# PrimeIntellect-ai/protocol

Hardware: AMD Instinct MI355X
Metric: task x worker pair-evals/sec (full-swarm match) (higher is better)
Workload: dtype u64

## Files before the change

### protocol_amd/csrc/pm_device.h

```cpp
#ifndef PM_DEVICE_H
#define PM_DEVICE_H

#include <hip/hip_runtime.h>
#include <stdint.h>

#include "pm_engine.h"

namespace pm {

static constexpr double PM_RAD = 3.14159265358979323846 / 180.0;
static constexpr uint64_t PM_KEY_NOLOC = 0x7FEFFFFFFFFFFFFFull;
static constexpr double PM_A_MAX_SAFE = 1.0 - 1.0 / 1048576.0;
static constexpr double PM_A_CHORD_MIN = 1.3e-6;
static constexpr uint32_t PM_CARVE_SLOTS = 8192;
static constexpr uint32_t PM_CARVE_PART = 64;
static constexpr uint32_t PM_CARVE_SEL_CAP = 256;
static constexpr uint32_t PM_CARVE_SLOT_BITS = 13;
static constexpr uint32_t PM_CARVE_BIG_SLOTS = 262144;
static constexpr uint32_t PM_CARVE_SLOT_BITS_BIG = 18;
static constexpr uint32_t PM_CARVE_SLOT_BITS_MEM = 21;
static constexpr double PM_TIE_BAND = 1.0 / 68719476736.0;
static constexpr double PM_TIE_BAND_BIG = 1.0 / 2147483648.0;
static constexpr double PM_TIE_BAND_MEM = 1.0 / 268435456.0;
static constexpr uint32_t PM_PROP_ROW = 96;
static constexpr uint32_t PM_PROP_SLOTS = 64;
static constexpr uint32_t PM_PROP_KMAX = 63;
static constexpr uint32_t PM_ROW_SAFE = 1u << 27;
static constexpr uint32_t PM_ROW_TAIL_CLEAR = 1u << 28;
static constexpr uint32_t PM_ROW_CLEAN = 1u << 29;
static constexpr uint32_t PM_ROW_TAIL_OK = 1u << 30;
static constexpr uint32_t PM_ROW_COMPLETE = 1u << 31;
static constexpr uint32_t PM_PROP_RESERVE = 64;
static constexpr uint32_t PM_PROP_MAX_SEEDS = 16384;
static constexpr uint32_t PM_CELL_G_MAX = 64;
static constexpr uint32_t PM_CELL_TABLE = PM_CELL_G_MAX * PM_CELL_G_MAX * PM_CELL_G_MAX + 2;
static constexpr uint32_t PM_CELL_MIN_N = 6000;
static constexpr uint32_t PM_CELL_AUTO_N = 40000;
static constexpr uint32_t PM_CELL_BIG_N = 40000;
static constexpr uint32_t PM_CELL_RMAX = 14;
static constexpr size_t PM_CARVE_LDS_BYTES = size_t(16) * PM_CARVE_PART * 8 + size_t(PM_CARVE_SLOTS / 64) * 16 +
                                             size_t(PM_CARVE_SLOTS) * 16 + size_t(PM_CARVE_SEL_CAP) * 4 + 1024;
static constexpr uint32_t PM_STREAM_SQ = 8192;
static constexpr uint32_t PM_STREAM_RQ = 8192;
static constexpr uint32_t PM_STREAM_TP = 4096;
static constexpr uint32_t PM_STREAM_LA_MAX = 3072;
static constexpr uint32_t PM_STREAM_CTL_WORDS = 64;
#ifndef PM_STREAM_PROP_WAVES_N
#define PM_STREAM_PROP_WAVES_N 4
#endif
static constexpr uint32_t PM_STREAM_PROP_WAVES = PM_STREAM_PROP_WAVES_N;
static constexpr uint32_t PM_STREAM_SLW_TREQ = PM_STREAM_TP;
static constexpr uint32_t PM_STREAM_SLW_PAY = PM_STREAM_TP + 1;
static constexpr size_t PM_STREAM_LDS_BYTES = PM_CARVE_LDS_BYTES + size_t(PM_STREAM_TP) * 4 + 128;
enum { SC_CLAIM = 0,
       SC_QUIT = 16,
       SC_DROP = 32,
       SC_ROWS = 48,
       SC_LET_BE = 53,
       SC_GAVE_UP = 49,
       SC_FINISH = 50,
       SC_FINISH_TICKET = 52,
       SC_TRACE = 51,
       SC_BATCHES = 54
};
static constexpr uint32_t PM_STREAM_TRACE_CAP = 1u << 17;
enum { SROW_NONE = 0, SROW_BITMAP = 1, SROW_WALK = 2, SROW_SWEEP = 3 };

struct CompatArgs {
  uint32_t W, n_cfgs, model_words;
  const uint32_t *flags, *gpu_count, *gpu_mem, *gpu_cls, *cpu_cores, *ram, *storage;
  const pm_config_row* cfgs;
  const pm_gpu_alt_row* alts;
  const uint32_t* model_bits;
  uint64_t* compat;
};

enum : uint32_t {
  REP_WHY = 0,
  REP_IDLE = PM_WHY_N,
  REP_GROUPS,
  REP_MEMBERS,
  REP_NO_TASK,
  REP_TASKS,
  REP_STRIDE = 16
};

struct ReportArgs {
  CompatArgs c;
  const int32_t* group_of;
  const uint32_t *g_cfg, *g_n, *g_task, *live_bits;
  uint32_t G;
  const uint64_t *tmask, *tlive;
  const uint32_t* tprefix;
  uint32_t t_lo, t_cap;
  uint32_t* out;
  uint32_t *running, *workers, *allowed;
};

struct ClaimArgs {
  uint32_t R;
  const uint32_t* rows;
  const int32_t* group_of;
  const uint32_t *g_n, *g_off, *g_task;
  const uint64_t* g_id;
  uint32_t* g_task_next;
  const uint32_t* chosen;
  const uint32_t* rank_in_group;
  const uint32_t* by_rank;
  const uint64_t* t_live;
  const uint32_t* t_prefix;
  pm_assignment* table;
  uint32_t* task_col;
  pm_assignment* h_table;
  uint32_t* h_gtask;
};

struct MatchPrepArgs {
  uint32_t W, G;
  const int32_t* group_of;
  const uint32_t *g_cfg, *g_n, *g_off, *members, *addr_rank, *g_task;
  uint64_t* sel;
  uint32_t *first, *count;
  uint32_t *rank_in_group, *by_rank;
  uint32_t* g_task_next;
};

struct RowUpdateArgs {
  uint32_t n;
  const double *lat_in, *lon_in;
  const uint32_t* u32_in;
  uint32_t *flags, *gpu_count, *gpu_mem, *gpu_cls, *cpu_cores, *ram, *storage, *addr_rank, *site;
  double *lat, *lon, *coslat;
  double *ux, *uy, *uz;
};

enum { CARVE_MODE_FORM = 0, CARVE_MODE_MERGE = 1 };
enum { CARVE_STATE_RUNNING = 0, CARVE_STATE_DONE = 1, CARVE_STATE_UNCERTAIN = 2, CARVE_STATE_OVERFLOW = 3,
       CARVE_STATE_ABORTED = 4 };
enum {
  CARVE_F_INIT = 1u << 0,
  CARVE_F_RUN = 1u << 1,
  CARVE_F_ALL = 1u << 2,
  CARVE_F_PROPS = 1u << 3,
  CARVE_F_EXTPREP = 1u << 4
};
struct CarveStatus {
  uint32_t state;
  uint32_t stop_ci;
  uint32_t n_groups;
  uint32_t n_members;
  uint32_t steps_total;
  uint32_t stop_seed;
  uint32_t n_eligible;
  uint32_t cur_ci;
  unsigned long long cand_sum;
  uint32_t n_list;
  uint32_t prop_k;
  uint32_t prop_limit;
  uint32_t rows_pr;
  uint32_t n_seeds;
  uint32_t total_available;
  uint32_t fast_steps;
  uint32_t slow_steps;
  uint32_t n_solo;
  uint32_t n_props;
  uint32_t need_prep;
  uint32_t g_lo, g_hi;
  uint32_t n_batches;
  uint32_t n_void;
  uint32_t why[8];
  uint32_t stream_timeouts;
  uint32_t stream_tickets;
  uint32_t stream_switches;
  uint32_t stream_listed;
  uint32_t stream_pre_used;
  uint32_t stream_pre_lost;
  uint32_t stream_refreshes;
  uint32_t _pad_sr;
  uint32_t cell_g;
  uint32_t n_indexed;
  uint32_t pruned_batches;
  uint32_t prune_fallbacks;
#ifdef PM_BATCH_LOG
  uint32_t blog_n;
  uint32_t blog[3 * 512];
#endif
  unsigned long long prop_keys;
  unsigned long long prof[64];
};

struct BatchDesc {
  uint32_t planned;
  uint32_t ci0;
  uint32_t total_available;
  uint32_t valid;
  uint32_t none;
  uint32_t ci, n_list, prop_k, prop_limit, rows_pr, n_seeds;
  uint32_t cell_g;
};

struct CarveArgs {
  uint32_t mode;
  uint32_t _flags_unused;
  uint32_t W;
  uint32_t proximity;
  uint32_t debug_uncertain_every;
  uint32_t _pad_re;
  const uint32_t* wflags;
  const double *lat, *lon, *coslat;
  const double *ux, *uy, *uz;
  const uint32_t* site;
  const uint64_t* compat;
  int32_t* group_of;
  uint32_t* order;
  uint32_t n_order;
  uint32_t _pad2;
  double *c_lat, *c_lon, *c_cos;
  double *c_ux, *c_uy, *c_uz;
  uint32_t* c_site;
  uint64_t* c_compat;
  uint64_t *alive_g, *loc_g;
  double *cc_lat, *cc_lon, *cc_cos;
  double *cc_ux, *cc_uy, *cc_uz;
  uint32_t* cc_site;
  uint32_t* slot_pos;
  uint32_t* slot_wid;
  uint64_t* bits_scratch;
  uint64_t* keys;
  uint32_t bits_stride;
  uint32_t _pad0;
  uint64_t* prop;
  uint64_t* prop_send;
  uint64_t* seed_map;
  uint32_t* seed_prefix;
  uint32_t* seed_slots;
  uint32_t dist_rank, dist_world;
  uint32_t count_keys, _pad_ck;
  uint32_t* prep_block_counts;
  uint32_t* prep_counts;
  BatchDesc* desc;
  uint64_t* alive_snap;
  uint32_t _pad_sp;
  uint32_t debug_mem_above;
  uint32_t* cell_cnt;
  uint32_t* cell_start;
  uint32_t *pos_cell, *pos_rank;
  uint32_t* cs_of_pos;
  uint32_t* cs_slot;
  double *cs_ux, *cs_uy, *cs_uz;
  uint32_t* cs_site;
  uint32_t prune_mode;
  uint32_t prune_factor;
  uint32_t walk_cap_div, _pad_w;
  uint32_t stream, stream_tag0;
  double* c_pack;
  double* cs_pack;
  uint64_t* cfgbits;
  unsigned long long* stream_sq;
  unsigned long long* stream_row_lo;
  unsigned long long* stream_row_hi;
  uint32_t* stream_ctl;
  uint32_t stream_la, stream_row_spins;
  uint32_t stream_la_div;
  uint32_t debug_abort_after;
  unsigned long long id_state;
  uint32_t id_g0, stage_m0;
  uint32_t stage_cap_g, stage_cap_m;
  uint32_t *stage_cfg, *stage_n, *stage_off, *stage_mem;
  unsigned long long* g_id_out;
  uint32_t* g_task_out;
  CarveStatus* h_status;
  unsigned long long* stream_trace;
  uint32_t n_avail, start_ci;
  uint32_t avail_cfg[PM_MAX_CONFIGS];
  uint32_t min_size[PM_MAX_CONFIGS];
  uint32_t max_size[PM_MAX_CONFIGS];
  uint32_t *g_cfg, *g_n, *g_off, *members;
  uint32_t cap_groups, cap_members;
  CarveStatus* status;
};

void launch_compat(const CompatArgs& a, hipStream_t s);
void launch_explain(const CompatArgs& p, const uint32_t* rows, uint32_t n, uint32_t stride, uint32_t* why_out, hipStream_t s);
void launch_config_report(const ReportArgs& a, uint32_t max_blocks, hipStream_t s);
void launch_task_report(const ReportArgs& a, uint32_t max_blocks, hipStream_t s);
void launch_geo(const double* lat, const double* lon, double* coslat, double* ux, double* uy, double* uz, uint32_t W,
                hipStream_t s);
void launch_triad(const double* b, const double* c, double* a, size_t n, hipStream_t s);
#ifdef PM_ROW_BENCH
hipError_t launch_row_bench(const CarveArgs* d_args, uint32_t seed, uint32_t ci, uint32_t reps, uint32_t mode, unsigned long long* d_out, hipStream_t s);
#endif
void launch_row_network_test(const uint64_t* keys, const uint32_t* sites, uint32_t n_waves, uint32_t n_per_wave, uint32_t slot_bits,
                             uint64_t ulps, uint32_t upto, uint64_t* rows_out, uint32_t* mismatches, hipStream_t s);
static constexpr uint32_t PM_DK_WORDS = 20;
void launch_distance_key_test(const double* in, const double* geo, uint32_t n, uint32_t mode, double* out, hipStream_t s);
void launch_update_rows(const RowUpdateArgs& a, hipStream_t s);
void launch_worker_selector(const int32_t* group_of, const uint32_t* g_cfg, uint32_t R, const uint32_t* rows,
                            uint64_t* sel, hipStream_t s);
void launch_eligible_selector(const uint32_t* wflags, const int32_t* group_of, const uint64_t* compat,
                              uint64_t enabled, uint32_t W, const uint8_t* shard, uint32_t my_rank, uint64_t* sel,
                              hipStream_t s);
void launch_chooser_rank(const int32_t* group_of, const uint64_t* g_id, const uint32_t* count, uint32_t R,
                         const uint32_t* rows, uint64_t seed, uint32_t* rank, hipStream_t s);
void launch_table_scatter(const pm_assignment* x, const uint32_t* xrow, uint32_t W, pm_assignment* table,
                          uint32_t* task_col, uint32_t* g_task_next, const uint64_t* t_live, const uint32_t* t_prefix,
                          hipStream_t s);
void launch_group_rank(const int32_t* group_of, const uint32_t* g_n, const uint32_t* g_off, const uint32_t* members,
                       const uint32_t* addr_rank, uint32_t W, uint32_t* rank_in_group, uint32_t* by_rank,
                       hipStream_t s);
void launch_claim_publish(const ClaimArgs& a, hipStream_t s);
void launch_match_prep(const MatchPrepArgs& a, hipStream_t s);
void launch_build_planes(const uint64_t* col_mask, uint32_t n_cols, uint32_t c_begin, uint32_t c_end, uint32_t stride,
                         uint32_t n_planes, uint64_t* planes, hipStream_t s);
void launch_pair_sweep(int variant, const uint64_t* row_sel, uint32_t R, const uint64_t* col_mask,
                       const uint64_t* planes, uint32_t c_begin, uint32_t c_end, uint32_t stride, uint32_t n_planes,
                       uint32_t* first, uint32_t* count, hipStream_t s, bool inited = false);
void launch_pair_select(int variant, const uint64_t* row_sel, uint32_t R, const uint64_t* col_mask,
                        const uint64_t* planes, uint32_t c_begin, uint32_t c_end, uint32_t stride, uint32_t n_planes,
                        const uint32_t* rank, uint32_t* out, hipStream_t s);
void launch_task_prefix(const uint64_t* live, uint32_t w_begin, uint32_t w_end, uint32_t* prefix, hipStream_t s);
void launch_task_delete(const uint32_t* slots, uint32_t n, uint64_t* tmask, uint64_t* live, uint64_t* planes,
                        uint32_t stride, uint32_t n_planes, hipStream_t s);
void launch_task_intern(const uint64_t* tmask, const uint64_t* live, uint32_t u_begin, uint32_t u_end, uint64_t valid,
                        uint64_t* keys, uint32_t n_slots, uint32_t* vals, uint32_t* counter_and_overflow, uint64_t* umask,
                        uint32_t cap_u, hipStream_t s);
void launch_task_compact_class(const uint32_t* first_c, const uint32_t* count_c, const uint64_t* tmask, uint64_t valid,
                               const uint64_t* keys, const uint32_t* vals, uint32_t n_slots, uint32_t u_begin,
                               uint32_t u_end, const uint64_t* live, const uint32_t* prefix, uint32_t* first_out,
                               uint32_t* count_out, hipStream_t s);
void launch_task_compact(const uint32_t* first_u, const uint32_t* count_u, uint32_t u_begin, uint32_t u_end,
                         const uint64_t* live, const uint32_t* prefix, uint32_t* first_out, uint32_t* count_out,
                         hipStream_t s);
void launch_newest(const int64_t* created_at, const uint64_t* live, uint32_t t_begin, uint32_t t_end,
                   uint32_t* idx_by_block, long long* val_by_block, uint32_t n_blocks, hipStream_t s);
void launch_group_ids(uint64_t* g_id, uint32_t* g_task, uint32_t n, uint64_t rng_state, hipStream_t s);
hipError_t carve_kernels_init();
hipError_t launch_carve(const CarveArgs* d_args, uint32_t flags, uint32_t start_ci, size_t lds_bytes, hipStream_t s);
uint32_t launch_carve_prep(const CarveArgs* d_args, uint32_t W, hipStream_t s);
hipError_t launch_carve_args_put(const CarveArgs& a, CarveArgs* d_args, hipStream_t s);
uint32_t launch_carve_elig(CarveArgs* d_args, const CarveArgs* put, uint32_t W, uint32_t n_bound, uint32_t index_min, uint32_t start_ci,
                           bool fresh, uint32_t n_groups0, uint32_t n_members0, hipStream_t s);
void launch_carve_apply(const CarveArgs* d_args, uint32_t W, hipStream_t s);
void launch_carve_propose(const CarveArgs* d_args, uint32_t W, hipStream_t s);
hipError_t launch_carve_stream(const CarveArgs* d_args, uint32_t start_ci, uint32_t n_prop_wgs, hipStream_t s);
void launch_scatter_const(uint32_t* dst, const uint32_t* idx, uint32_t n, uint32_t v, hipStream_t s);
void launch_scatter_pairs(uint32_t* dst, const uint32_t* pairs, uint32_t n, hipStream_t s);
void launch_merge_place(const CarveArgs* d_args, uint32_t n_order, uint32_t n_groups0, uint32_t n_members0, uint32_t steps0,
                        hipStream_t s);

}
#endif
```

### protocol_amd/csrc/pm_engine_carve.inc

```
static int32_t ensure_compat(pm_engine* e, hipEvent_t end_ev = nullptr) {
  if (!e->have_cfgs || !e->have_workers) return set_error(PM_ESTATE, "configs and workers must be uploaded first");
  {
    int32_t rcf = sync_flags(e);
    if (rcf) return rcf;
  }
  if (!e->compat_dirty) return PM_OK;
  for (const pm_gpu_alt_row& a : e->alts)
    if ((a.flags & PM_G_MODEL) && a.model_row >= e->model_rows)
      return set_error(PM_ESTATE, "a GPU alternative names a model row but pm_set_model_table was not called");
  if (e->model_rows && e->cls_check_dirty)
    for (uint32_t w = 0; w < e->W; ++w)
      if ((e->h_flags[w] & PM_W_GPU_MODEL) && e->h_gpu_cls[w] >= e->model_classes)
        return set_error(PM_ERANGE, "worker gpu_model_class outside the model table");
  e->cls_check_dirty = false;
  HIPCHK(e->d_compat.ensure(std::max<size_t>(e->W, 1)));
  CompatArgs a{};
  a.W = e->W;
  a.n_cfgs = uint32_t(e->cfgs.size());
  a.model_words = (e->model_classes + 31u) / 32u;
  a.flags = e->d_flags.p;
  a.gpu_count = e->d_gpu_count.p;
  a.gpu_mem = e->d_gpu_mem.p;
  a.gpu_cls = e->d_gpu_cls.p;
  a.cpu_cores = e->d_cpu_cores.p;
// ... 23 lines not shown
  }
  e->h_compat_valid = true;
  return PM_OK;
}

static double host_distance(double lat1, double lon1, double lat2, double lon2) {
  const double R = 6371.0;
  const double lat1r = lat1 * PM_RAD, lat2r = lat2 * PM_RAD;
  const double dlat = (lat2 - lat1) * PM_RAD, dlon = (lon2 - lon1) * PM_RAD;
  const double s1 = std::sin(dlat / 2.0), s2 = std::sin(dlon / 2.0);
  const double a = s1 * s1 + std::cos(lat1r) * std::cos(lat2r) * (s2 * s2);
  const double c = 2.0 * std::atan2(std::sqrt(a), std::sqrt(1.0 - a));
  return R * c;
}

struct CarvePlan {
  std::vector<uint32_t> avail;
};

static size_t carve_lds_bytes(uint32_t , bool* in_lds) {
  *in_lds = true;
  return PM_CARVE_LDS_BYTES;
}

static int32_t fill_carve_args(pm_engine* e, CarveArgs* a, uint32_t mode, uint32_t n_order, bool stream = false) {
  const size_t cap = std::max<size_t>(e->W, 1);
  HIPCHK(e->d_order.ensure(cap));
  HIPCHK(e->d_c_lat.ensure(cap));
  HIPCHK(e->d_c_lon.ensure(cap));
  HIPCHK(e->d_c_cos.ensure(cap));
  HIPCHK(e->d_cc_lat.ensure(cap));
  HIPCHK(e->d_cc_lon.ensure(cap));
  HIPCHK(e->d_cc_cos.ensure(cap));
  for (int k = 0; k < 3; ++k) {
    HIPCHK(e->d_c_u[k].ensure(cap));
    HIPCHK(e->d_cc_u[k].ensure(cap));
  }
  HIPCHK(e->d_c_compat.ensure(cap));
  HIPCHK(e->d_keys.ensure(cap));
  HIPCHK(e->d_slot_pos.ensure(cap));
  HIPCHK(e->d_slot_wid.ensure(cap));
  HIPCHK(e->d_c_site.ensure(cap));
  HIPCHK(e->d_cc_site.ensure(cap));
  {
    const size_t world = e->dist_world;
    const size_t rows_pr = (size_t(PM_PROP_MAX_SEEDS) + 64 + world - 1) / world;
    HIPCHK(e->d_prop.ensure(rows_pr * world * PM_PROP_ROW));
    if (world > 1) HIPCHK(e->d_prop_send.ensure(rows_pr * PM_PROP_ROW));
    HIPCHK(e->d_seed_map.ensure((cap + 63) / 64 + 64));
    HIPCHK(e->d_seed_prefix.ensure((cap + 63) / 64 + 64));
    HIPCHK(e->d_seed_slots.ensure(size_t(PM_PROP_MAX_SEEDS) + 128));
    HIPCHK(e->d_prep_block_counts.ensure(((cap + 255) / 256 + 1) * PM_MAX_CONFIGS));
    HIPCHK(e->d_prep_counts.ensure(PM_MAX_CONFIGS + 8));
  }
  HIPCHK(e->d_status.ensure(1));
  HIPCHK(e->d_carve_args.ensure(2));
  HIPCHK(e->d_desc.ensure(2));
  const uint32_t stride = uint32_t((cap + 63) / 64);
  HIPCHK(e->d_bits.ensure(size_t(stride) * 4));
  HIPCHK(e->d_snap.ensure(size_t(stride) * 2));
  if (stream) {
    HIPCHK(e->d_c_pack.ensure(cap * 4));
    HIPCHK(e->d_cs_pack.ensure(cap * 4));
    HIPCHK(e->d_cfgbits.ensure(size_t(stride) * PM_MAX_CONFIGS));
    HIPCHK(e->d_stream_ctl.ensure(PM_STREAM_CTL_WORDS));
    if (!e->d_stream_sq.p) {
      HIPCHK(e->d_stream_sq.ensure(PM_STREAM_SQ));
      HIPCHK(e->d_stream_row_lo.ensure(size_t(PM_STREAM_RQ) * 64));
      HIPCHK(e->d_stream_row_hi.ensure(size_t(PM_STREAM_RQ) * 64));
      e->stream_seq = 0;
    }
  }
  if (mode == CARVE_MODE_FORM && e->prune_mode && e->cfg.proximity_enabled) {
    if (!e->d_cell_cnt.p) {
      HIPCHK(e->d_cell_cnt.ensure(PM_CELL_TABLE));
      HIPCHK(hipMemsetAsync(e->d_cell_cnt.p, 0, e->d_cell_cnt.cap * sizeof(uint32_t), e->stream));
    }
    if (!e->d_cell_start.p) {
      HIPCHK(e->d_cell_start.ensure(PM_CELL_TABLE + 384));
      HIPCHK(hipMemsetAsync(e->d_cell_start.p, 0, e->d_cell_start.cap * sizeof(uint32_t), e->stream));
    }
    HIPCHK(e->d_pos_cell.ensure(cap));
    HIPCHK(e->d_pos_rank.ensure(cap));
    HIPCHK(e->d_cs_of_pos.ensure(cap));
    HIPCHK(e->d_cs_slot.ensure(cap));
    HIPCHK(e->d_cs_site.ensure(cap));
    for (auto& u : e->d_cs_u) HIPCHK(u.ensure(cap));
  }
  std::memset(a, 0, sizeof(*a));
  a->mode = mode;
  a->W = e->W;
  a->proximity = e->cfg.proximity_enabled;
  a->debug_uncertain_every = e->cfg.debug_uncertain_every;
  a->wflags = e->d_flags.p;
  a->lat = e->d_lat.p;
  a->lon = e->d_lon.p;
  a->coslat = e->d_coslat.p;
  a->ux = e->d_ux.p;
  a->uy = e->d_uy.p;
  a->uz = e->d_uz.p;
  a->compat = e->d_compat.p;
  a->group_of = e->d_group_of.p;
  a->order = e->d_order.p;
  a->n_order = n_order;
  a->c_lat = e->d_c_lat.p;
  a->c_lon = e->d_c_lon.p;
  a->c_cos = e->d_c_cos.p;
  a->c_ux = e->d_c_u[0].p;
  a->c_uy = e->d_c_u[1].p;
  a->c_uz = e->d_c_u[2].p;
  a->c_compat = e->d_c_compat.p;
  a->alive_g = e->d_bits.p;
  a->loc_g = e->d_bits.p + stride;
  a->cc_lat = e->d_cc_lat.p;
  a->cc_lon = e->d_cc_lon.p;
  a->cc_cos = e->d_cc_cos.p;
  a->cc_ux = e->d_cc_u[0].p;
  a->cc_uy = e->d_cc_u[1].p;
  a->cc_uz = e->d_cc_u[2].p;
  a->keys = e->d_keys.p;
  a->slot_pos = e->d_slot_pos.p;
  a->slot_wid = e->d_slot_wid.p;
  a->site = e->d_site.p;
  a->c_site = e->d_c_site.p;
  a->cc_site = e->d_cc_site.p;
  a->prop = e->d_prop.p;
  a->prop_send = e->dist_world > 1 ? e->d_prop_send.p : e->d_prop.p;
  a->seed_map = e->d_seed_map.p;
  a->seed_prefix = e->d_seed_prefix.p;
  a->seed_slots = e->d_seed_slots.p;
  a->dist_rank = e->dist_rank;
  a->dist_world = e->dist_world;
  a->count_keys = e->cfg.time_proposer ? 1u : 0u;
  a->prep_block_counts = e->d_prep_block_counts.p;
  a->prep_counts = e->d_prep_counts.p;
  a->bits_scratch = e->d_bits.p + size_t(stride) * 2;
  a->bits_stride = stride;
  a->status = e->d_status.p;
  a->desc = e->d_desc.p;
  a->alive_snap = e->d_snap.p;
  a->debug_mem_above = e->debug_mem_above;
  if (mode == CARVE_MODE_FORM && e->prune_mode && e->cfg.proximity_enabled) {
    a->prune_mode = e->prune_mode;
    a->prune_factor = e->prune_factor;
    a->walk_cap_div = e->walk_cap_div;
    a->cell_cnt = e->d_cell_cnt.p;
    a->cell_start = e->d_cell_start.p;
    a->pos_cell = e->d_pos_cell.p;
    a->pos_rank = e->d_pos_rank.p;
    a->cs_of_pos = e->d_cs_of_pos.p;
    a->cs_slot = e->d_cs_slot.p;
    a->cs_site = e->d_cs_site.p;
    a->cs_ux = e->d_cs_u[0].p;
    a->cs_uy = e->d_cs_u[1].p;
    a->cs_uz = e->d_cs_u[2].p;
  }
  if (stream) {
    a->stream = 1;
    a->cc_lat = a->c_lat;
    a->cc_lon = a->c_lon;
    a->cc_cos = a->c_cos;
    a->cc_ux = a->c_ux;
    a->cc_uy = a->c_uy;
    a->cc_uz = a->c_uz;
    a->cc_site = a->c_site;
    a->slot_wid = a->order;
    a->bits_scratch = e->d_bits.p;
    a->loc_g = e->d_bits.p + stride;
    a->alive_g = e->d_bits.p + size_t(stride) * 2;
    a->cfgbits = e->d_cfgbits.p;
    a->c_pack = e->d_c_pack.p;
    a->cs_pack = e->d_cs_pack.p;
    a->stream_sq = (unsigned long long*)e->d_stream_sq.p;
    a->stream_row_lo = (unsigned long long*)e->d_stream_row_lo.p;
    a->stream_row_hi = (unsigned long long*)e->d_stream_row_hi.p;
    a->stream_ctl = e->d_stream_ctl.p;
#if defined(PM_CARVE_PROF) || defined(PM_ROW_REC)
    HIPCHK(e->d_stream_trace.ensure(size_t(PM_STREAM_TRACE_CAP) * 2));
    a->stream_trace = (unsigned long long*)e->d_stream_trace.p;
#endif
#ifdef PM_ROW_REC
    HIPCHK(hipMemsetAsync(e->d_stream_trace.p, 0, size_t(PM_STREAM_TRACE_CAP) * 16, e->stream));
#endif
    a->stream_la = e->stream_la_env;
    a->stream_la_div = e->stream_la_div_env;
    a->stream_row_spins = e->stream_row_spins_env;
    a->debug_abort_after = e->debug_abort_after;
  }
  return PM_OK;
}

static int32_t host_resolve_form_step(pm_engine* e, uint32_t cfg, CarveStatus* st) {
  int32_t rc = pull_compat(e);
  if (rc) return rc;
  std::vector<int32_t> group_of(e->W);
  if (e->W) {
    HIPCHK(hipMemcpyAsync(group_of.data(), e->d_group_of.p, size_t(e->W) * 4, hipMemcpyDeviceToHost, e->stream));
    HIPCHK(hipStreamSynchronize(e->stream));
  }
  const pm_config_row& c = e->cfgs[cfg];
  std::vector<uint32_t> compat;
  size_t total_available = 0;
  for (uint32_t w = 0; w < e->W; ++w) {
    const uint32_t f = e->h_flags[w];
    if (!((f & PM_W_HEALTHY) && (f & PM_W_HAS_P2P) && group_of[w] < 0)) continue;
    ++total_available;
    if ((e->h_compat[w] >> cfg) & 1ull) compat.push_back(w);
  }
  if (total_available < c.min_group_size || compat.size() < c.min_group_size || compat.empty())
    return set_error(PM_ESTATE, "host resolve: nothing to carve (state mismatch)");
  uint32_t seed = compat[0];
  bool seed_loc = false;
  for (uint32_t w : compat)
    if (e->h_flags[w] & PM_W_HAS_LOC) {
      seed = w;
      seed_loc = true;
      break;
    }
  std::vector<uint32_t> rest;
  for (uint32_t w : compat)
    if (w != seed) rest.push_back(w);
  if (seed_loc && e->cfg.proximity_enabled) {
    std::vector<double> d(e->W, 0.0);
    for (uint32_t w : rest)
      d[w] = (e->h_flags[w] & PM_W_HAS_LOC) ? host_distance(e->h_lat[seed], e->h_lon[seed], e->h_lat[w], e->h_lon[w])
                                            : 1.7976931348623157e308;
    std::stable_sort(rest.begin(), rest.end(), [&](uint32_t a, uint32_t b) { return d[a] < d[b]; });
  }
  std::vector<uint32_t> members{seed};
  for (uint32_t w : rest) {
    if (members.size() >= c.max_group_size) break;
    members.push_back(w);
  }
  if (members.size() < c.min_group_size) return set_error(PM_ESTATE, "host resolve: group below min size");
  const uint32_t g = st->n_groups, off = st->n_members, n = uint32_t(members.size());
  if (g >= e->d_g_cfg.cap || off + n > e->d_members.cap) return set_error(PM_ENOMEM, "group arrays overflow");
  HIPCHK(hipMemcpyAsync(e->d_g_cfg.p + g, &cfg, 4, hipMemcpyHostToDevice, e->stream));
  HIPCHK(hipMemcpyAsync(e->d_g_n.p + g, &n, 4, hipMemcpyHostToDevice, e->stream));
  HIPCHK(hipMemcpyAsync(e->d_g_off.p + g, &off, 4, hipMemcpyHostToDevice, e->stream));
  HIPCHK(hipMemcpyAsync(e->d_members.p + off, members.data(), size_t(n) * 4, hipMemcpyHostToDevice, e->stream));
  for (uint32_t w : members) group_of[w] = int32_t(g);
  HIPCHK(hipMemcpyAsync(e->d_group_of.p, group_of.data(), size_t(e->W) * 4, hipMemcpyHostToDevice, e->stream));
  HIPCHK(hipStreamSynchronize(e->stream));
  st->n_groups += 1;
  st->n_members += n;
  st->n_solo += n == 1 ? 1u : 0u;
  st->steps_total += 1;
  return PM_OK;
}

static int32_t absorb_groups(pm_engine* e) {
  if (!e->absorb_pending) return PM_OK;
  HIPCHK(hipEventSynchronize(e->ev_groups));
  const uint32_t g0 = e->ab_g0, ng = e->ab_g1 - e->ab_g0, m0 = e->ab_m0;
  const uint32_t *g_cfg = e->ab_cfg_p, *g_n = e->ab_n_p, *g_off = e->ab_off_p, *members = e->ab_mem_p;
  if (e->groups.capacity() < e->groups.size() + ng) e->groups.reserve(std::max(e->groups.size() + ng, e->groups.capacity() * 2));
  for (uint32_t k = 0; k < ng; ++k) {
    Group gr;
    gr.id = splitmix64_next(&e->id_rng);
    gr.cfg = g_cfg[k];
    gr.task = PM_NONE;
    gr.task_uid = 0;
    gr.members.assign(members + (g_off[k] - m0), members + (g_off[k] - m0) + g_n[k]);
    for (uint32_t w : gr.members) e->h_group_of[w] = int32_t(g0 + k);
    log_group_event(e, PM_GROUP_CREATED, gr);
    e->groups.push_back(std::move(gr));
  }
  e->absorb_pending = false;
  return PM_OK;
}

#define ABSORB_PENDING(e)                 \
  do {                                    \
    int32_t rc_abs_ = absorb_groups(e);   \
    if (rc_abs_) return rc_abs_;          \
  } while (0)

static void host_mark(const char* what) {
  static const bool on = [] { const char* v = getenv("PM_TRACE_HOST"); return v && *v == '1'; }();
  if (!on) return;
  static const auto t0 = std::chrono::steady_clock::now();
  const double us = std::chrono::duration<double, std::micro>(std::chrono::steady_clock::now() - t0).count();
  fprintf(stderr, "[pm host] %10.1f us  %s\n", us, what);
}

struct FormRun {
  CarveArgs a;
  BatchDesc desc[2] = {};
  CarveStatus st;
  std::vector<uint32_t> avail;
  uint32_t g0 = 0, m0 = 0, start_ci = 0;
  size_t lds = 0;
  bool use_props = false;
  bool nothing = false;
  uint32_t n_bound = 0;
  uint32_t n_elig_hint = 0;
  bool stream = false;
  bool single_call = true;
  uint32_t stream_wgs = 0;
  bool local_carve = false;
  bool rearmed = false;
  uint32_t stage_cap = 0;
  bool args_pending = false;
};

static int32_t launch_propose_timed(pm_engine* e, const CarveArgs* d_args, uint32_t n_bound, hipStream_t s);

static int32_t form_setup_args(pm_engine* e, FormRun* r);

static int32_t form_queue_init(pm_engine* e, FormRun* r, bool fresh = false) {
  fresh = fresh && r->use_props;
  if (!fresh) HIPCHK(hipMemcpyAsync(e->d_status.p, &r->st, sizeof(r->st), hipMemcpyHostToDevice, e->stream));
  if (r->use_props) {
    if (!r->stream) HIPCHK(hipMemsetAsync(e->d_desc.p, 0, 2 * sizeof(BatchDesc), e->stream));
    const uint32_t index_min = !r->a.prune_mode ? 0u : r->a.prune_mode >= 2u ? 1u : PM_CELL_AUTO_N;
    if (r->stream) {
      if (e->stream_seq == 0 || e->stream_seq >= 127) {
        HIPCHK(hipMemsetAsync(e->d_stream_sq.p, 0, size_t(PM_STREAM_SQ) * 8, e->stream));
        HIPCHK(hipMemsetAsync(e->d_stream_row_lo.p, 0, size_t(PM_STREAM_RQ) * 64 * 8, e->stream));
        HIPCHK(hipMemsetAsync(e->d_stream_row_hi.p, 0, size_t(PM_STREAM_RQ) * 64 * 8, e->stream));
        e->stream_seq = 0;
      }
      e->stream_seq += 1;
      const uint32_t tag0 = e->stream_seq << 25;
      if (r->a.stream_tag0 != tag0) {
        r->a.stream_tag0 = tag0;
        if (!r->args_pending)
          HIPCHK(hipMemcpyAsync(&e->d_carve_args.p->stream_tag0, &r->a.stream_tag0, sizeof(uint32_t), hipMemcpyHostToDevice, e->stream));
      }
    }
    e->tick_carve_launches += launch_carve_elig(e->d_carve_args.p, r->args_pending ? &r->a : nullptr, e->W, r->n_bound,
                                                r->n_elig_hint >= index_min ? index_min : 0u, r->start_ci, fresh, r->st.n_groups,
                                                r->st.n_members, e->stream);
    r->args_pending = false;
    host_mark("form: eligible list queued");
    if (r->stream) {
      HIPCHK(launch_carve_stream(e->d_carve_args.p, r->start_ci, r->stream_wgs, e->stream));
      e->tick_carve_launches += 2;
      return PM_OK;
    }
    e->tick_carve_launches += launch_carve_prep(e->d_carve_args.p, r->n_bound, e->stream);
    HIPCHK(hipGetLastError());
  } else
    HIPCHK(launch_carve(e->d_carve_args.p, CARVE_F_INIT | CARVE_F_RUN | CARVE_F_ALL, r->start_ci, r->lds, e->stream));
  e->tick_carve_launches++;
  return PM_OK;
}

static int32_t form_begin(pm_engine* e, FormRun* r, bool allow_pipeline, bool local_carve = false, hipEvent_t begin_ev = nullptr) {
  int32_t rc = absorb_groups(e);
  if (rc) return rc;
  rc = ensure_compat(e);
  if (rc) return rc;
  rc = push_groups(e);
  if (rc) return rc;
  available_order(e->cfgs.data(), uint32_t(e->cfgs.size()), e->enabled, &r->avail);
  r->g0 = e->d_n_groups;
  r->m0 = e->d_n_members;
  r->start_ci = 0;
  r->nothing = r->avail.empty() || e->W == 0;
  if (r->nothing) return PM_OK;
  if (e->h_group_of.size() == e->W && e->h_flags.size() == e->W) {
    const int32_t* const gof = e->h_group_of.data();
    const uint32_t* const fl = e->h_flags.data();
    const uint32_t need = PM_W_HEALTHY | PM_W_HAS_P2P;
    uint32_t nb = 0, ne = 0;
    for (uint32_t w = 0; w < e->W; ++w) {
      const uint32_t un = uint32_t(gof[w]) >> 31;
      nb += un;
      ne += un & uint32_t((fl[w] & need) == need);
    }
    r->n_bound = nb;
    r->n_elig_hint = ne;
  } else {
    r->n_bound = uint32_t(std::count_if(e->h_group_of.begin(), e->h_group_of.end(), [](int32_t g) { return g < 0; }));
    r->n_elig_hint = r->n_bound;
  }
  if (e->h_group_of.size() != e->W) r->n_bound = r->n_elig_hint = e->W;
  if (r->n_bound == 0) r->n_bound = 1;
  r->st = CarveStatus{};
  r->st.state = CARVE_STATE_RUNNING;
  r->st.n_groups = r->g0;
  r->st.n_members = r->m0;
  r->single_call = allow_pipeline;
  r->local_carve = local_carve;
  r->use_props = e->cfg.carve_variant != 1 && e->cfg.proximity_enabled;
  r->stream = r->single_call && r->use_props && e->cfg.carve_variant == 0 && (e->dist_world == 1 || r->local_carve) &&
              r->n_bound <= PM_CARVE_BIG_SLOTS &&
              !e->debug_mem_above;
  host_mark("form: begin (host mirrors counted)");
  rc = form_setup_args(e, r);
  if (rc) return rc;
  host_mark("form: arguments queued");
  if (begin_ev && r->args_pending) {
    e->k_carve_begin = begin_ev;
  } else {
    HIPCHK(hipEventRecord(e->kev[2], e->stream));
    e->k_carve_begin = e->kev[2];
  }
  return form_queue_init(e, r, true);
}

static int32_t form_setup_args(pm_engine* e, FormRun* r) {
  CarveArgs& a = r->a;
  int32_t rc = fill_carve_args(e, &a, CARVE_MODE_FORM, 0, r->stream);
  if (rc) return rc;
  if (r->stream) {
    uint32_t wgs = e->stream_wgs_env ? e->stream_wgs_env : r->n_elig_hint / 64u + 48u;
    const uint32_t max_wgs = e->n_cus > 8u ? e->n_cus - 4u : 4u;
    r->stream_wgs = std::max(1u, std::min(wgs, max_wgs));
    a.stream_tag0 = ((e->stream_seq == 0 || e->stream_seq >= 127) ? 1u : e->stream_seq + 1u) << 25;
    a.id_state = e->id_rng;
    a.id_g0 = r->g0;
    a.stage_m0 = r->m0;
    a.g_id_out = (unsigned long long*)e->d_g_id.p;
    a.g_task_out = e->d_g_task.p;
    r->stage_cap = std::max<uint32_t>(r->n_bound, 1u);
    const size_t need = size_t(4) * r->stage_cap;
    if (e->h_gstage_cap < need) {
      HIPCHK(hipStreamSynchronize(e->stream));
      if (e->h_gstage) (void)hipHostFree(e->h_gstage);
      e->h_gstage = nullptr;
      e->h_gstage_cap = 0;
      const size_t cap = std::max<size_t>(need, size_t(4) * std::max<uint32_t>(e->W, 1));
      HIPCHK(hipHostMalloc((void**)&e->h_gstage, cap * sizeof(uint32_t)));
      e->h_gstage_cap = cap;
    }
    if (!e->h_status) HIPCHK(hipHostMalloc((void**)&e->h_status, sizeof(CarveStatus)));
    a.stage_cap_g = a.stage_cap_m = r->stage_cap;
    a.stage_cfg = e->h_gstage;
    a.stage_n = e->h_gstage + r->stage_cap;
    a.stage_off = e->h_gstage + size_t(2) * r->stage_cap;
    a.stage_mem = e->h_gstage + size_t(3) * r->stage_cap;
    a.h_status = e->h_status;
    e->h_status->state = 0xFFFFFFFFu;
  }
  if (r->local_carve) {
    a.dist_rank = 0;
    a.dist_world = 1;
    a.prop_send = a.prop;
  }
  a.n_avail = uint32_t(r->avail.size());
  for (size_t i = 0; i < r->avail.size(); ++i) {
    a.avail_cfg[i] = r->avail[i];
    a.min_size[i] = e->cfgs[r->avail[i]].min_group_size;
    a.max_size[i] = e->cfgs[r->avail[i]].max_group_size;
  }
  a.g_cfg = e->d_g_cfg.p;
  a.g_n = e->d_g_n.p;
  a.g_off = e->d_g_off.p;
  a.members = e->d_members.p;
  a.cap_groups = uint32_t(std::min<size_t>(e->d_g_cfg.cap, 0xFFFFFFFFu));
  a.cap_members = uint32_t(std::min<size_t>(e->d_members.cap, 0xFFFFFFFFu));
  bool in_lds;
  r->lds = carve_lds_bytes(a.bits_stride, &in_lds);
  r->args_pending = r->use_props;
  if (!r->args_pending) HIPCHK(launch_carve_args_put(a, e->d_carve_args.p, e->stream));
  return PM_OK;
}

static int32_t launch_propose_timed(pm_engine* e, const CarveArgs* d_args, uint32_t n_bound, hipStream_t s) {
  if (!e->cfg.time_proposer) {
    launch_carve_propose(d_args, n_bound, s);
    return PM_OK;
  }
  while (e->prop_ev.size() < e->prop_ev_used + 2) {
    hipEvent_t x = nullptr;
    HIPCHK(hipEventCreate(&x));
    e->prop_ev.push_back(x);
  }
  HIPCHK(hipEventRecord(e->prop_ev[e->prop_ev_used], s));
  launch_carve_propose(d_args, n_bound, s);
  HIPCHK(hipEventRecord(e->prop_ev[e->prop_ev_used + 1], s));
  e->prop_ev_used += 2;
  return PM_OK;
}

static int32_t form_queue_pairs(pm_engine* e, FormRun* r, uint32_t count) {
  for (uint32_t k = 0; k < count; ++k) {
    int32_t rc = launch_propose_timed(e, e->d_carve_args.p, r->n_bound, e->stream);
    if (rc) return rc;
    HIPCHK(launch_carve(e->d_carve_args.p, CARVE_F_RUN | CARVE_F_PROPS | CARVE_F_EXTPREP, 0, r->lds, e->stream));
    e->tick_carve_launches += 2u + launch_carve_prep(e->d_carve_args.p, r->n_bound, e->stream);
  }
  return PM_OK;
}

static int32_t form_poll(pm_engine* e, FormRun* r) {
  for (;;) {
    HIPCHK(hipEventRecord(e->kev[3], e->stream));
    HIPCHK(hipMemcpyAsync(&r->st, e->d_status.p, sizeof(r->st), hipMemcpyDeviceToHost, e->stream));
    const bool want_desc = r->use_props && !r->stream;
    if (want_desc) HIPCHK(hipMemcpyAsync(r->desc, e->d_desc.p, sizeof(r->desc), hipMemcpyDeviceToHost, e->stream));
    HIPCHK(hipStreamSynchronize(e->stream));
    {
      float ms = 0;
      HIPCHK(hipEventElapsedTime(&ms, e->k_carve_begin ? e->k_carve_begin : e->kev[2], e->kev[3]));
      e->k_ms_carve += ms;
      HIPCHK(hipEventRecord(e->kev[2], e->stream));
      e->k_carve_begin = e->kev[2];
      for (size_t k = 0; k + 1 < e->prop_ev_used; k += 2) {
        HIPCHK(hipEventElapsedTime(&ms, e->prop_ev[k], e->prop_ev[k + 1]));
        e->k_ms_propose += ms;
      }
      e->prop_ev_used = 0;
    }
    if (r->st.state == CARVE_STATE_OVERFLOW) return set_error(PM_ENOMEM, "carve: group arrays overflow");
    if (r->st.state == CARVE_STATE_ABORTED) {
      if (!r->stream) return set_error(PM_ENODEV, "carve: a hand-shake inside the validator timed out");
      e->tick_stream_aborts++;
      r->rearmed = true;
      r->stream = false;
      int32_t rca = form_setup_args(e, r);
      if (rca) return rca;
      r->start_ci = r->st.stop_ci;
      r->st.state = CARVE_STATE_RUNNING;
      rca = form_queue_init(e, r);
      if (rca) return rca;
      return PM_OK;
    }
    if (r->st.state != CARVE_STATE_UNCERTAIN) return PM_OK;
    int32_t rc = host_resolve_form_step(e, r->avail[r->st.stop_ci], &r->st);
    if (rc) return rc;
    e->tick_host_resolved++;
    r->rearmed = true;
    r->start_ci = r->st.stop_ci;
    r->st.state = CARVE_STATE_RUNNING;
    rc = form_queue_init(e, r);
    if (rc) return rc;
  }
}

static int32_t form_finish(pm_engine* e, FormRun* r, uint32_t* n_formed, bool defer_absorb, bool have_event = false) {
  if (n_formed) *n_formed = 0;
  if (r->nothing) return PM_OK;
  const CarveStatus& st = r->st;
  e->tick_fast_steps += st.fast_steps;
  e->tick_carve_steps += st.steps_total;
  e->tick_cand_sum += st.cand_sum;
  e->tick_props += r->stream && !st.n_props ? st.stream_tickets : st.n_props;
  e->tick_prop_keys += st.prop_keys;
  e->tick_stream_timeouts += st.stream_timeouts;
  e->tick_stream_tickets += st.stream_tickets;
  std::memcpy(e->carve_prof, st.prof, sizeof(st.prof));
  for (int k = 0; k < 8; ++k) e->carve_why[k] = st.why[k];
  e->carve_why[8] = st.n_batches;
  e->carve_why[9] = st.n_void;
  e->carve_why[10] = st.pruned_batches;
  e->carve_why[11] = st.prune_fallbacks;
  e->carve_why[12] = st.cell_g;
  e->carve_why[13] = st.n_indexed;
  e->carve_why[14] = r->stream ? 1u : 0u;
  e->carve_why[15] = st.stream_tickets;
  e->carve_why[16] = st.stream_timeouts;
  e->carve_why[17] = st.stream_switches;
  e->carve_why[18] = st.stream_listed;
  e->carve_why[19] = r->stream_wgs;
  e->carve_why[20] = e->tick_stream_aborts;
  e->carve_why[21] = st.slow_steps;
  e->carve_why[22] = st.stream_pre_used;
  e->carve_why[23] = st.stream_pre_lost;
#ifdef PM_BATCH_LOG
  e->blog.assign(st.blog, st.blog + 3 * std::min<uint32_t>(st.blog_n, 512u));
#endif

  const uint32_t g0 = r->g0, m0 = r->m0, g1 = st.n_groups, m1 = st.n_members;
  if (g1 > g0) {
    const uint32_t ng = g1 - g0, nm = m1 - m0;
    const bool staged = r->stream && !r->rearmed && ng <= r->stage_cap && nm <= r->stage_cap;
    if (staged) {
      e->ab_cfg_p = e->h_gstage;
      e->ab_n_p = e->h_gstage + r->stage_cap;
      e->ab_off_p = e->h_gstage + size_t(2) * r->stage_cap;
      e->ab_mem_p = e->h_gstage + size_t(3) * r->stage_cap;
      if (!have_event) HIPCHK(hipEventRecord(e->ev_groups, e->stream));
    } else {
      const size_t need = size_t(3) * ng + nm;
      if (e->h_gstage_cap < need) {
        if (e->h_gstage) (void)hipHostFree(e->h_gstage);
        e->h_gstage = nullptr;
        e->h_gstage_cap = 0;
        const size_t cap = std::max<size_t>(need, size_t(4) * std::max<uint32_t>(e->W, 1));
        HIPCHK(hipHostMalloc((void**)&e->h_gstage, cap * sizeof(uint32_t)));
        e->h_gstage_cap = cap;
      }
      uint32_t* st_cfg = e->h_gstage;
      HIPCHK(hipMemcpyAsync(st_cfg, e->d_g_cfg.p + g0, size_t(ng) * 4, hipMemcpyDeviceToHost, e->stream));
      HIPCHK(hipMemcpyAsync(st_cfg + ng, e->d_g_n.p + g0, size_t(ng) * 4, hipMemcpyDeviceToHost, e->stream));
      HIPCHK(hipMemcpyAsync(st_cfg + 2 * size_t(ng), e->d_g_off.p + g0, size_t(ng) * 4, hipMemcpyDeviceToHost, e->stream));
      HIPCHK(hipMemcpyAsync(st_cfg + 3 * size_t(ng), e->d_members.p + m0, size_t(nm) * 4, hipMemcpyDeviceToHost, e->stream));
      e->ab_cfg_p = st_cfg;
      e->ab_n_p = st_cfg + ng;
      e->ab_off_p = st_cfg + 2 * size_t(ng);
      e->ab_mem_p = st_cfg + 3 * size_t(ng);
      HIPCHK(hipEventRecord(e->ev_groups, e->stream));
      host_mark("form: group copies queued");
      launch_group_ids(e->d_g_id.p + g0, e->d_g_task.p + g0, ng, e->id_rng, e->stream);
      HIPCHK(hipGetLastError());
    }
    e->absorb_pending = true;
    e->ab_g0 = g0;
    e->ab_g1 = g1;
    e->ab_m0 = m0;
    e->ab_m1 = m1;
    e->ab_solo = st.n_solo;
    e->d_n_groups = g1;
    e->d_n_members = m1;
    if (!defer_absorb) {
      int32_t rc = absorb_groups(e);
      if (rc) return rc;
    }
  }
  if (n_formed) *n_formed = g1 - g0;
  return PM_OK;
}

static int32_t run_form_wait(pm_engine* e, FormRun& r) {
  int32_t rc = PM_OK;
  if (!r.nothing) {
    uint32_t batch = e->form_rounds_hint ? e->form_rounds_hint + 1u : r.a.n_avail + 3u;
    for (uint32_t spins = 0;; ++spins) {
      if (spins > 4096u + e->W / 8u) return set_error(PM_ENODEV, "carve made no progress");
      if (r.use_props && !r.stream) {
        rc = form_queue_pairs(e, &r, batch);
        if (rc) return rc;
      }
      host_mark("form: carve queued");
      rc = form_poll(e, &r);
      if (rc) return rc;
      host_mark("form: status back");
      if (r.st.state == CARVE_STATE_DONE) break;
      if (r.st.state != CARVE_STATE_RUNNING || !r.use_props) return set_error(PM_ENODEV, "carve kernel did not complete");
      if (r.stream) return set_error(PM_ENODEV, "streaming carve did not complete");
      batch = 8u;
    }
  }
  if (!r.nothing && r.use_props && !r.stream) e->form_rounds_hint = r.st.n_batches + r.st.n_void;
  return PM_OK;
}
static int32_t run_form_rest(pm_engine* e, FormRun& r, uint32_t* n_formed, bool defer_absorb) {
  int32_t rc = run_form_wait(e, r);
  if (rc) return rc;
  return form_finish(e, &r, n_formed, defer_absorb);
}

static int32_t run_form(pm_engine* e, uint32_t* n_formed, bool defer_absorb = false) {
  FormRun r;
  int32_t rc = form_begin(e, &r, true);
  if (rc) return rc;
  return run_form_rest(e, r, n_formed, defer_absorb);
}
```

### protocol_amd/csrc/pm_engine_match.inc

```

static int32_t ensure_task_planes(pm_engine* e) {
  if (!e->have_tasks) return set_error(PM_ESTATE, "tasks must be uploaded first");
  const uint32_t n_planes = uint32_t(e->cfgs.size());
  const uint32_t stride = e->t_cap / 64u;
  if (e->tplanes_dirty) {
    HIPCHK(e->d_tplanes.ensure(std::max<size_t>(size_t(stride) * (n_planes + 1), 1)));
    launch_build_planes(e->d_tmask.p, e->t_cap, e->t_lo, e->t_cap, stride, n_planes, e->d_tplanes.p, e->stream);
    HIPCHK(hipGetLastError());
    e->tplanes_dirty = false;
  }
  if (e->tprefix_dirty) {
    launch_task_prefix(e->d_tlive.p, e->t_lo / 64u, stride, e->d_tprefix.p, e->stream);
    HIPCHK(hipGetLastError());
    e->tprefix_dirty = false;
  }
  return PM_OK;
}

static uint32_t task_position(pm_engine* e, uint32_t u) {
  if (u == PM_NONE || u < e->t_lo || u >= e->t_cap) return PM_NONE;
  if (!e->h_tprefix_valid) {
    const uint32_t stride = e->t_cap / 64u;
    e->h_tprefix.assign(stride, 0);
    uint32_t acc = 0;
    for (uint32_t j = e->t_lo / 64u; j < stride; ++j) {
      e->h_tprefix[j] = acc;
      acc += uint32_t(__builtin_popcountll(e->h_tlive[j]));
    }
    e->h_tprefix_valid = true;
  }
  const uint64_t w = e->h_tlive[u >> 6];
  if (!((w >> (u & 63u)) & 1ull)) return PM_NONE;
  return e->h_tprefix[u >> 6] + uint32_t(__builtin_popcountll(w & ((1ull << (u & 63u)) - 1ull)));
}

static int32_t ensure_sweep_outputs(pm_engine* e, uint32_t R) {
  HIPCHK(e->d_first.ensure(std::max<uint32_t>(R, 1)));
  HIPCHK(e->d_count.ensure(std::max<uint32_t>(R, 1)));
  HIPCHK(e->d_rank.ensure(std::max<uint32_t>(R, 1)));
  HIPCHK(e->d_chosen.ensure(std::max<uint32_t>(R, 1)));
  return PM_OK;
}

static int32_t pick_task_for_config(pm_engine* e, uint32_t cfg, uint64_t group_id, uint32_t* task_out) {
  *task_out = PM_NONE;
  if (!e->have_tasks || e->T == 0) return PM_OK;
  if (!e->cfg_app_valid) {
    std::memset(e->cfg_app_count, 0, sizeof(e->cfg_app_count));
    for (uint32_t u = e->t_lo; u < e->t_cap; ++u) {
      uint64_t m = e->h_tmask[u];
      while (m) {
        e->cfg_app_count[__builtin_ctzll(m)]++;
        m &= m - 1;
      }
    }
    e->cfg_app_valid = true;
  }
  const uint32_t n_app = e->cfg_app_count[cfg];
  if (!n_app) return PM_OK;
  const uint64_t bit = 1ull << cfg;
  uint32_t r = 0;
  if (e->cfg.chooser == PM_CHOOSE_SEEDED) r = uint32_t(splitmix64_mix(e->cfg.chooser_seed ^ group_id) % n_app);
  for (uint32_t u = e->t_lo; u < e->t_cap; ++u)
    if (e->h_tmask[u] & bit) {
      if (r == 0) {
        *task_out = u;
        return PM_OK;
      }
      --r;
    }
  return PM_OK;
}

static int32_t run_match(pm_engine* e, bool want_count, std::vector<uint32_t>* count_out, bool dist = false, size_t G_ub = 0) {
  pm_assignment* const claim_h_table = dist ? nullptr : e->claim_h_table;
  uint32_t* const claim_h_gtask = dist ? nullptr : e->claim_h_gtask;
  e->claim_h_table = nullptr;
  e->claim_h_gtask = nullptr;
  if (!e->have_cfgs || !e->have_workers || !e->have_tasks)
    return set_error(PM_ESTATE, "configs, workers and tasks must be uploaded first");
  int32_t rc = push_groups(e);
  if (rc) return rc;
  const int variant = int(e->cfg.sweep_variant);
  host_mark("match: groups pushed");
  rc = ensure_task_planes(e);
  if (rc) return rc;
  host_mark("match: task planes");
  const uint32_t R = dist ? uint32_t(e->h_own_rows.size()) : e->W;
  const uint32_t* rows = dist ? e->d_own_rows.p : nullptr;
  rc = ensure_sweep_outputs(e, R);
  if (rc) return rc;
  HIPCHK(e->d_sel.ensure(std::max<uint32_t>(e->W, 1)));
  HIPCHK(e->d_table.ensure(std::max<uint32_t>(e->W, 1)));
  HIPCHK(e->d_task_col.ensure(std::max<uint32_t>(e->W, 1)));
  if (e->W == 0) return PM_OK;
  const uint32_t n_planes = uint32_t(e->cfgs.size());

  host_mark("match: selector launch");
  const size_t G = G_ub ? G_ub : e->d_n_groups;
  if (!dist) {
    MatchPrepArgs m{};
    m.W = e->W;
    m.G = uint32_t(G);
    m.group_of = e->d_group_of.p;
    m.g_cfg = e->d_g_cfg.p;
    m.g_n = e->d_g_n.p;
    m.g_off = e->d_g_off.p;
    m.members = e->d_members.p;
    m.addr_rank = e->d_addr_rank.p;
    m.g_task = e->d_g_task.p;
    m.sel = e->d_sel.p;
    m.first = e->d_first.p;
    m.count = e->d_count.p;
    m.rank_in_group = e->d_rank_in_group.p;
    m.by_rank = e->d_by_rank.p;
    m.g_task_next = e->d_g_task_next.p;
    launch_match_prep(m, e->stream);
  } else {
    launch_worker_selector(e->d_group_of.p, e->d_g_cfg.p, R, rows, e->d_sel.p, e->stream);
  }
  const bool time_sweep = e->cfg.time_proposer != 0;
  if (time_sweep) HIPCHK(hipEventRecord(e->kev[4], e->stream));
  const uint32_t t_stride = e->t_cap / 64u;
  launch_pair_sweep(variant, e->d_sel.p, R, e->d_tmask.p, e->d_tplanes.p, e->t_lo, e->t_cap, t_stride, n_planes,
                    e->d_first.p, e->d_count.p, e->stream, !dist);
  if (time_sweep) HIPCHK(hipEventRecord(e->kev[5], e->stream));
  e->k_sweep_recorded = time_sweep;
  const uint32_t* chosen = e->d_first.p;
  if (e->cfg.chooser == PM_CHOOSE_SEEDED) {
    launch_chooser_rank(e->d_group_of.p, e->d_g_id.p, e->d_count.p, R, rows, e->cfg.chooser_seed, e->d_rank.p,
                        e->stream);
    launch_pair_select(variant, e->d_sel.p, R, e->d_tmask.p, e->d_tplanes.p, e->t_lo, e->t_cap, t_stride, n_planes,
                       e->d_rank.p, e->d_chosen.p, e->stream);
    chosen = e->d_chosen.p;
  }
  if (dist) {
    launch_group_rank(e->d_group_of.p, e->d_g_n.p, e->d_g_off.p, e->d_members.p, e->d_addr_rank.p, e->W,
                      e->d_rank_in_group.p, e->d_by_rank.p, e->stream);
    if (G) HIPCHK(hipMemcpyAsync(e->d_g_task_next.p, e->d_g_task.p, G * 4, hipMemcpyDeviceToDevice, e->stream));
  }
  ClaimArgs c{};
  c.R = R;
  c.rows = rows;
  c.group_of = e->d_group_of.p;
  c.g_n = e->d_g_n.p;
  c.g_off = e->d_g_off.p;
  c.g_task = e->d_g_task.p;
  c.g_id = e->d_g_id.p;
  c.g_task_next = e->d_g_task_next.p;
  c.chosen = chosen;
  c.rank_in_group = e->d_rank_in_group.p;
  c.by_rank = e->d_by_rank.p;
  c.t_live = e->d_tlive.p;
  c.t_prefix = e->d_tprefix.p;
  c.table = dist ? e->d_table_x.p + size_t(e->dist_rank) * e->dist_cap_t : e->d_table.p;
  c.task_col = e->d_task_col.p;
  c.h_table = claim_h_table;
  c.h_gtask = claim_h_gtask;
  launch_claim_publish(c, e->stream);
  HIPCHK(hipGetLastError());
  if (want_count && count_out) {
    count_out->resize(R);
    HIPCHK(hipMemcpyAsync(count_out->data(), e->d_count.p, size_t(R) * 4, hipMemcpyDeviceToHost, e->stream));
  }
  return PM_OK;
}

static int32_t pub_buffer(pm_engine* e, PubTable& t, uint32_t rows, uint64_t** out) {
  uint64_t* words = t.words.load(std::memory_order_relaxed);
  if (t.cap_rows < rows || !words) {
    const size_t cap = std::max<size_t>(size_t(rows) + rows / 8 + 64, 64);
    uint64_t* nw = nullptr;
    if (hipHostMalloc((void**)&nw, cap * 32) != hipSuccess || !nw)
      return set_error(PM_ENOMEM, "out of pinned host memory for the published table");
    std::memset(nw, 0, cap * 32);
    const uint64_t s0 = t.seq.load(std::memory_order_relaxed);
    t.seq.store(s0 + 1, std::memory_order_relaxed);
    std::atomic_thread_fence(std::memory_order_release);
    if (words) e->pub_retired.push_back(words);
    words = nw;
    t.cap_rows = cap;
    t.words.store(nw, std::memory_order_relaxed);
    t.seq.store(s0 + 2, std::memory_order_release);
  }
  *out = words;
  return PM_OK;
}

static void pub_patch(pm_engine* e, const std::vector<uint32_t>* only) {
  const int cur = e->pub_cur.load(std::memory_order_relaxed);
  if (cur < 0) return;
  const bool by_id = e->pub_groups_epoch != e->groups_epoch;
  std::unordered_map<uint64_t, uint32_t>& slot_of_id = e->slot_of_id;
  if (by_id && e->slot_of_id_epoch != e->groups_epoch) {
    slot_of_id.clear();
    slot_of_id.reserve(e->groups.size() * 2);
    for (size_t g = 0; g < e->groups.size(); ++g) slot_of_id.emplace(e->groups[g].id, uint32_t(g));
    e->slot_of_id_epoch = e->groups_epoch;
  }
  PubTable& t = e->pub[cur];
  if (t.cleared.load(std::memory_order_relaxed)) return;
  const uint32_t n = t.n.load(std::memory_order_relaxed);
  pm_assignment* rows = reinterpret_cast<pm_assignment*>(t.words.load(std::memory_order_relaxed));
  if (!rows || !n) return;
  auto patched = [&](pm_assignment a, uint32_t keep_shift) -> pm_assignment {
    if (a.group_slot == PM_NONE) return a;
    uint32_t slot = a.group_slot;
    if (by_id) {
      const auto it = slot_of_id.find(a.group_id);
      slot = it == slot_of_id.end() ? PM_NONE : it->second;
    }
    const bool gone = slot >= e->groups.size() || e->groups[slot].dead;
    if (gone) {
      a.task = PM_NONE;
      a.group_slot = PM_NONE;
      a.group_index = 0;
      a.group_size = 0;
      a.next_worker = PM_NONE;
      a.group_id = 0;
    } else {
      const uint32_t h = e->groups[slot].task;
      a.task = h == PM_NONE ? PM_NONE : task_position(e, h) - keep_shift;
    }
    return a;
  };
  auto store_row = [](pm_assignment* dst, const pm_assignment& a) {
    uint64_t v[4];
    std::memcpy(v, &a, sizeof(a));
    uint64_t* d = reinterpret_cast<uint64_t*>(dst);
    for (int k = 0; k < 4; ++k) __atomic_store_n(&d[k], v[k], __ATOMIC_RELAXED);
  };
  if (!only) {
    const int nx = cur ^ 1;
    PubTable& d = e->pub[nx];
    uint64_t* dw = nullptr;
    if (pub_buffer(e, d, n, &dw) == PM_OK && dw) {
      pm_assignment* drows = reinterpret_cast<pm_assignment*>(dw);
      const uint64_t d0 = d.seq.load(std::memory_order_relaxed);
      d.seq.store(d0 + 1, std::memory_order_relaxed);
      std::atomic_thread_fence(std::memory_order_release);
      for (uint32_t w = 0; w < n; ++w) store_row(&drows[w], patched(rows[w], 0u));
      d.n.store(n, std::memory_order_relaxed);
      d.task_shift.store(0, std::memory_order_relaxed);
      d.cleared.store(0, std::memory_order_relaxed);
      d.seq.store(d0 + 2, std::memory_order_release);
      e->pub_cur.store(nx, std::memory_order_release);
      e->h_table = drows;
      return;
    }
  }
  const uint64_t s0 = t.seq.load(std::memory_order_relaxed);
  t.seq.store(s0 + 1, std::memory_order_relaxed);
  std::atomic_thread_fence(std::memory_order_release);
  if (only) {
    const std::vector<uint32_t>& ws = *only;
    for (size_t i = 0; i < ws.size(); ++i) {
      if (i + 12u < ws.size() && ws[i + 12u] < n) __builtin_prefetch(&rows[ws[i + 12u]], 1);
      const uint32_t w = ws[i];
      if (w >= n) continue;
      uint64_t* d = reinterpret_cast<uint64_t*>(&rows[w]);
      if (uint32_t(__atomic_load_n(&d[0], __ATOMIC_RELAXED) >> 32) == PM_NONE) continue;
      const uint64_t w2 = __atomic_load_n(&d[2], __ATOMIC_RELAXED);
      __atomic_store_n(&d[0], (uint64_t(PM_NONE) << 32) | PM_NONE, __ATOMIC_RELAXED);
      __atomic_store_n(&d[1], 0ull, __ATOMIC_RELAXED);
      __atomic_store_n(&d[2], (w2 & 0xFFFFFFFF00000000ull) | PM_NONE, __ATOMIC_RELAXED);
      __atomic_store_n(&d[3], 0ull, __ATOMIC_RELAXED);
    }
  } else {
    for (uint32_t w = 0; w < n; ++w) store_row(&rows[w], patched(rows[w], 0u));
    t.task_shift.store(0, std::memory_order_relaxed);
  }
  t.seq.store(s0 + 2, std::memory_order_release);
}

static void pub_shift_tasks(pm_engine* e, uint32_t n_new) {
  const int cur = e->pub_cur.load(std::memory_order_relaxed);
  if (cur < 0) return;
  PubTable& t = e->pub[cur];
  const uint64_t s0 = t.seq.load(std::memory_order_relaxed);
  t.seq.store(s0 + 1, std::memory_order_relaxed);
  std::atomic_thread_fence(std::memory_order_release);
  t.task_shift.store(t.task_shift.load(std::memory_order_relaxed) + n_new, std::memory_order_relaxed);
  t.seq.store(s0 + 2, std::memory_order_release);
}

struct PubRun {
  int nx = 0;
  uint64_t s0 = 0;
  uint64_t* words = nullptr;
  size_t G = 0;
};

static void publish_abandon(pm_engine* e, const PubRun& pr) {
  (void)hipStreamSynchronize(e->stream);
  PubTable& t = e->pub[pr.nx];
  t.n.store(0, std::memory_order_relaxed);
  t.seq.store(pr.s0 + 2, std::memory_order_release);
}

static int32_t publish_begin(pm_engine* e, PubRun* pr, size_t G, bool direct = false) {
  e->claim_h_table = nullptr;
  e->claim_h_gtask = nullptr;
  if (e->h_gtask_cap < G) {
    if (e->h_gtask_pinned) (void)hipHostFree(e->h_gtask_pinned);
    e->h_gtask_pinned = nullptr;
    e->h_gtask_cap = 0;
    const size_t cap = std::max<size_t>(G, std::max<uint32_t>(e->W, 1));
    HIPCHK(hipHostMalloc((void**)&e->h_gtask_pinned, cap * sizeof(uint32_t)));
    e->h_gtask_cap = cap;
  }
  const int cur = e->pub_cur.load(std::memory_order_relaxed);
  const int nx = cur < 0 ? 0 : (cur ^ 1);
  PubTable& t = e->pub[nx];
  uint64_t* words = nullptr;
  {
    int32_t rcb = pub_buffer(e, t, e->W, &words);
    if (rcb) return rcb;
  }
  const uint64_t s0 = t.seq.load(std::memory_order_relaxed);
  t.seq.store(s0 + 1, std::memory_order_relaxed);
  std::atomic_thread_fence(std::memory_order_release);
  pr->nx = nx;
  pr->s0 = s0;
  pr->words = words;
  pr->G = G;
  if (direct) {
    e->claim_h_table = reinterpret_cast<pm_assignment*>(words);
    e->claim_h_gtask = e->h_gtask_pinned;
    return PM_OK;
  }
  hipError_t herr = hipSuccess;
  if (e->W) herr = hipMemcpyAsync(words, e->d_table.p, sizeof(pm_assignment) * e->W, hipMemcpyDeviceToHost, e->stream);
  if (herr == hipSuccess && G)
    herr = hipMemcpyAsync(e->h_gtask_pinned, e->d_g_task_next.p, G * 4, hipMemcpyDeviceToHost, e->stream);
  if (herr != hipSuccess) {
    publish_abandon(e, *pr);
    HIPCHK(herr);
  }
  return PM_OK;
}

static int32_t publish_end(pm_engine* e, const PubRun& pr) {
  PubTable& t = e->pub[pr.nx];
  const hipError_t herr = hipStreamSynchronize(e->stream);
  if (herr != hipSuccess) {
    publish_abandon(e, pr);
    HIPCHK(herr);
  }
  const size_t G = e->groups.size();
  if (G != pr.G) {
    publish_abandon(e, pr);
    return set_error(PM_ESTATE, "publish: the host group list and the device group arrays disagree");
  }
  const uint32_t* g_task = e->h_gtask_pinned;
  t.n.store(e->W, std::memory_order_relaxed);
  t.task_shift.store(0, std::memory_order_relaxed);
  t.cleared.store(0, std::memory_order_relaxed);
  t.seq.store(pr.s0 + 2, std::memory_order_release);
  e->pub_cur.store(pr.nx, std::memory_order_release);
  e->h_table = reinterpret_cast<const pm_assignment*>(pr.words);
  e->pub_groups_epoch = e->groups_epoch;
  for (size_t g = 0; g < G; ++g) {
    if (e->groups[g].dead) continue;
    e->groups[g].task = g_task[g];
    e->groups[g].task_uid = g_task[g] == PM_NONE ? 0 : (e->tasks_have_uid ? e->h_tuid[g_task[g]] : task_position(e, g_task[g]));
  }
  std::swap(e->d_g_task, e->d_g_task_next);
  return PM_OK;
}

static int32_t publish_open(pm_engine* e, PubRun* pr, size_t G) { return publish_begin(e, pr, G, true); }

static int32_t publish(pm_engine* e) {
  PubRun pr;
  int32_t rc = publish_begin(e, &pr, e->groups.size());
  if (rc) return rc;
  return publish_end(e, pr);
}
```

### protocol_amd/csrc/pm_engine_tick.inc

```
static void tick_reset(pm_engine* e) {
  e->tick_host_resolved = e->tick_carve_launches = e->tick_carve_steps = 0;
  e->tick_fast_steps = 0;
  e->tick_cand_sum = 0;
  e->tick_props = 0;
  e->tick_prop_keys = 0;
  e->tick_stream_timeouts = e->tick_stream_tickets = e->tick_stream_aborts = 0;
  e->k_ms_propose = 0;
  e->prop_ev_used = 0;
  e->k_ms_compat = e->k_ms_carve = e->k_ms_sweep = 0;
  e->k_sweep_recorded = e->k_compat_recorded = false;
  e->one_event_behind_carve = false;
  e->end_event_queued = false;
  e->tick_t0 = std::chrono::steady_clock::now();
}

static int32_t tick_stats(pm_engine* e, pm_stats* stats, uint32_t n_formed, uint32_t n_merged) {
  if (!e->end_event_queued) HIPCHK(hipEventRecord(e->ev[5], e->stream));
  HIPCHK(hipEventSynchronize(e->ev[5]));
  hipEvent_t const sweep_end = e->end_event_queued ? e->ev[5] : e->ev[4];
  pm_stats s{};
  HIPCHK(hipEventElapsedTime(&s.ms_compat, e->ev[0], e->ev[1]));
  HIPCHK(hipEventElapsedTime(&s.ms_carve, e->ev[1], e->ev[2]));
  if (e->one_event_behind_carve) {
    s.ms_merge = 0.0f;
    HIPCHK(hipEventElapsedTime(&s.ms_sweep, e->ev[2], sweep_end));
  } else {
    HIPCHK(hipEventElapsedTime(&s.ms_merge, e->ev[2], e->ev[3]));
    HIPCHK(hipEventElapsedTime(&s.ms_sweep, e->ev[3], sweep_end));
  }
  if (!e->end_event_queued) HIPCHK(hipEventElapsedTime(&s.ms_publish, e->ev[4], e->ev[5]));
  if (e->end_event_queued)
    s.ms_total = std::chrono::duration<float, std::milli>(std::chrono::steady_clock::now() - e->tick_t0).count();
  else
    HIPCHK(hipEventElapsedTime(&s.ms_total, e->ev[0], e->ev[5]));
  if (e->k_compat_recorded) HIPCHK(hipEventElapsedTime(&s.ms_compat_kernel, e->kev[0], e->k_compat_end ? e->k_compat_end : e->kev[1]));
  if (e->k_sweep_recorded) HIPCHK(hipEventElapsedTime(&s.ms_sweep_kernel, e->kev[4], e->kev[5]));
  s.ms_carve_kernel = e->k_ms_carve;
  s.carve_cand_sum = e->tick_cand_sum;
  s.ms_propose_kernel = e->k_ms_propose;
  s.proposals = e->tick_props;
  s.propose_keys = e->tick_prop_keys;
  s.n_groups = uint32_t(e->groups.size() - e->n_dead_groups);
  s.n_formed = n_formed;
  s.n_merged = n_merged;
  s.carve_steps = e->tick_carve_steps;
  s.carve_fast_steps = e->tick_fast_steps;
  s.host_resolved_steps = e->tick_host_resolved;
  s.carve_launches = e->tick_carve_launches;
  s.pair_evals = uint64_t(e->T) * uint64_t(e->W);
  e->last_stats = s;
  if (stats) *stats = s;
  return PM_OK;
}

int32_t pm_tick(pm_engine* e, pm_stats* stats) {
  if (!e) return set_error(PM_EINVAL, "null argument");
  std::lock_guard<std::mutex> lk(e->mu);
  if (e->dist_phase != 0) return set_error(PM_ESTATE, "a stepwise tick is in progress");
  HIPCHK(hipSetDevice(e->cfg.device));
  if (!e->have_cfgs || !e->have_workers || !e->have_tasks)
    return set_error(PM_ESTATE, "configs, workers and tasks must be uploaded first");
  if (e->dist_world > 1) return set_error(PM_ESTATE, "multi-GPU engine: use the stepwise tick (pm_dist_tick_begin ...)");
  if (e->dist_phase != 0) return set_error(PM_ESTATE, "a stepwise tick is in progress");
  tick_reset(e);
  host_mark("tick: begin");
  uint32_t n_formed = 0, n_merged = 0;
  HIPCHK(hipEventRecord(e->ev[0], e->stream));
  e->compat_dirty = true;
  int32_t rc = absorb_groups(e);
  if (rc) return rc;
  rc = push_groups(e);
  if (rc) return rc;
  rc = ensure_task_planes(e);
  if (rc) return rc;
  rc = ensure_compat(e, e->ev[1]);
  if (rc) return rc;
  if (!e->k_compat_recorded) HIPCHK(hipEventRecord(e->ev[1], e->stream));
  host_mark("tick: compat queued");
  FormRun r;
  rc = form_begin(e, &r, true, false, e->ev[1]);
  if (rc) return rc;
  bool done = false;
  if (r.stream && !r.nothing && !e->tick_needs_merge) {
    PubRun pr;
    HIPCHK(hipEventRecord(e->ev[2], e->stream));
    const size_t G_ub = std::min<size_t>(size_t(r.g0) + r.stage_cap, std::min(e->d_g_task.cap, e->d_g_task_next.cap));
    host_mark("tick: carve queued");
    rc = publish_open(e, &pr, G_ub);
    if (rc) return rc;
    host_mark("tick: snapshot buffer open");
    rc = run_match(e, false, nullptr, false, G_ub);
    if (rc) {
      publish_abandon(e, pr);
      return rc;
    }
    HIPCHK(hipEventRecord(e->ev[5], e->stream));
    e->end_event_queued = true;
    host_mark("tick: everything queued");
    if (hipEventSynchronize(e->ev[2]) != hipSuccess) {
      publish_abandon(e, pr);
      return set_error(PM_ENODEV, "tick: the stream failed");
    }
    host_mark("tick: carve through");
    const CarveStatus& hs = *e->h_status;
    size_t solo = hs.n_solo;
    for (const Group& g : e->groups) solo += g.members.size() == 1 && !g.dead;
    const bool fits = hs.n_groups >= r.g0 && hs.n_groups - r.g0 <= r.stage_cap && hs.n_members >= r.m0 &&
                      hs.n_members - r.m0 <= r.stage_cap && hs.n_groups <= G_ub;
    if (hs.state == CARVE_STATE_DONE && fits && solo < 2) {
      r.st = hs;
      rc = form_finish(e, &r, &n_formed, false, true);
      if (rc) {
        publish_abandon(e, pr);
        return rc;
      }
      host_mark("tick: groups absorbed");
      pr.G = e->groups.size();
      rc = publish_end(e, pr);
      host_mark("tick: published");
      if (rc) return rc;
      float ms = 0;
      HIPCHK(hipEventElapsedTime(&ms, e->k_carve_begin ? e->k_carve_begin : e->kev[2], e->ev[2]));
      e->k_ms_carve += ms;
      e->one_event_behind_carve = true;
      done = true;
    } else {
      publish_abandon(e, pr);
      e->tick_needs_merge = solo >= 2;
    }
  }
  if (!done) {
    rc = run_form_rest(e, r, &n_formed, true);
    if (rc) return rc;
    host_mark("tick: form done");
    HIPCHK(hipEventRecord(e->ev[2], e->stream));
    rc = run_merge(e, &n_merged);
    if (rc) return rc;
    host_mark("tick: merge done");
    HIPCHK(hipEventRecord(e->ev[3], e->stream));
    PubRun pr;
    rc = push_groups(e);
    if (rc) return rc;
    rc = publish_open(e, &pr, e->d_n_groups);
    if (rc) return rc;
    rc = run_match(e, false, nullptr);
    if (rc) {
      publish_abandon(e, pr);
      return rc;
    }
    host_mark("tick: match queued");
    HIPCHK(hipEventRecord(e->ev[5], e->stream));
    e->end_event_queued = true;
    rc = absorb_groups(e);
    if (rc) {
      publish_abandon(e, pr);
      return rc;
    }
    host_mark("tick: groups absorbed");
    rc = publish_end(e, pr);
    host_mark("tick: published");
    if (rc) return rc;
  }
  return tick_stats(e, stats, n_formed, n_merged);
}

int32_t pm_tick_many(pm_engine* const* engines, uint32_t n, pm_stats* stats, uint32_t flags) {
  if (!engines || n == 0) return set_error(PM_EINVAL, "null argument");
  if (n > 1024u) return set_error(PM_EINVAL, "more than 1024 engines in one call");
  if (flags & ~uint32_t(PM_TICK_MANY_THREADS)) return set_error(PM_EINVAL, "unknown flag");
  for (uint32_t i = 0; i < n; ++i) {
    if (!engines[i]) return set_error(PM_EINVAL, "null engine");
    for (uint32_t j = 0; j < i; ++j)
      if (engines[j] == engines[i]) return set_error(PM_EINVAL, "the same engine twice in one call");
  }
  if (flags & PM_TICK_MANY_THREADS) {
    std::vector<int32_t> rcs(n, PM_OK);
    std::vector<std::string> msgs(n);
    std::vector<std::thread> th;
    th.reserve(n);
    for (uint32_t i = 0; i < n; ++i)
      th.emplace_back([&, i] {
        rcs[i] = pm_tick(engines[i], stats ? &stats[i] : nullptr);
        if (rcs[i]) msgs[i] = g_last_error;
      });
    for (std::thread& t : th) t.join();
    for (uint32_t i = 0; i < n; ++i)
      if (rcs[i]) return set_error(rcs[i], msgs[i]);
    return PM_OK;
  }
  std::vector<pm_engine*> by_addr(engines, engines + n);
  std::sort(by_addr.begin(), by_addr.end(), [](const pm_engine* a, const pm_engine* b) { return std::less<const pm_engine*>()(a, b); });
  std::vector<std::unique_lock<std::mutex>> locks;
  locks.reserve(n);
  for (pm_engine* e : by_addr) locks.emplace_back(e->mu);
  for (uint32_t i = 0; i < n; ++i) {
    pm_engine* e = engines[i];
    if (!e->have_cfgs || !e->have_workers || !e->have_tasks)
      return set_error(PM_ESTATE, "configs, workers and tasks must be uploaded first");
    if (e->dist_world > 1) return set_error(PM_ESTATE, "multi-GPU engine: use the stepwise tick (pm_dist_tick_begin ...)");
    if (e->dist_phase != 0) return set_error(PM_ESTATE, "a stepwise tick is in progress");
  }
  std::vector<std::unique_ptr<FormRun>> runs(n);
  std::vector<PubRun> pubs(n);
  std::vector<uint32_t> n_formed(n, 0), n_merged(n, 0);
  std::vector<int32_t> rcs(n, PM_OK);
  std::vector<std::string> msgs(n);
  auto failed = [&](uint32_t i, int32_t rc) {
    rcs[i] = rc;
    msgs[i] = g_last_error;
  };
  const uint32_t i_lo = 0, i_hi = n;
  {
  for (uint32_t i = i_lo; i < i_hi; ++i) {
    pm_engine* e = engines[i];
    auto stage = [&]() -> int32_t {
      HIPCHK(hipSetDevice(e->cfg.device));
      tick_reset(e);
      HIPCHK(hipEventRecord(e->ev[0], e->stream));
      e->compat_dirty = true;
      int32_t rc = ensure_compat(e);
      if (rc) return rc;
      HIPCHK(hipEventRecord(e->ev[1], e->stream));
      runs[i].reset(new (std::nothrow) FormRun());
      if (!runs[i]) return set_error(PM_ENOMEM, "out of host memory");
      return form_begin(e, runs[i].get(), true);
    };
    const int32_t rc = stage();
    if (rc) failed(i, rc);
  }
  for (uint32_t i = i_lo; i < i_hi; ++i) {
    if (rcs[i]) continue;
    pm_engine* e = engines[i];
    auto stage = [&]() -> int32_t {
      HIPCHK(hipSetDevice(e->cfg.device));
      int32_t rc = run_form_rest(e, *runs[i], &n_formed[i], true);
      if (rc) return rc;
      HIPCHK(hipEventRecord(e->ev[2], e->stream));
      rc = run_merge(e, &n_merged[i]);
      if (rc) return rc;
      HIPCHK(hipEventRecord(e->ev[3], e->stream));
      rc = push_groups(e);
      if (rc) return rc;
      rc = publish_open(e, &pubs[i], e->d_n_groups);
      if (rc) return rc;
      rc = run_match(e, false, nullptr);
      if (rc) {
        publish_abandon(e, pubs[i]);
        return rc;
      }
      HIPCHK(hipEventRecord(e->ev[5], e->stream));
      e->end_event_queued = true;
      return PM_OK;
    };
    const int32_t rc = stage();
    runs[i].reset();
    if (rc) failed(i, rc);
  }
  for (uint32_t i = i_lo; i < i_hi; ++i) {
    if (rcs[i]) continue;
    pm_engine* e = engines[i];
    auto stage = [&]() -> int32_t {
      HIPCHK(hipSetDevice(e->cfg.device));
      int32_t rc = absorb_groups(e);
      if (rc) {
        publish_abandon(e, pubs[i]);
        return rc;
      }
      rc = publish_end(e, pubs[i]);
      if (rc) return rc;
      return tick_stats(e, stats ? &stats[i] : nullptr, n_formed[i], n_merged[i]);
    };
    const int32_t rc = stage();
    if (rc) failed(i, rc);
  }
  }
  for (uint32_t i = 0; i < n; ++i)
    if (rcs[i]) return set_error(rcs[i], msgs[i]);
  return PM_OK;
}
```

### protocol_amd/csrc/pm_kernels.hip

```cpp
#include <hip/hip_runtime.h>
#include <stdint.h>

#include "pm_device.h"

#if defined(__HIP_DEVICE_COMPILE__) && !defined(__gfx950__)
#error "pm_kernels.hip is written for gfx950 (MI355X): see the note on the placement kernels' fences above"
#endif

namespace pm {


template <int CTRL, int ROW_MASK>
__device__ __forceinline__ uint32_t dpp_add_step(uint32_t v) {
  return v + (uint32_t)__builtin_amdgcn_update_dpp(0, (int)v, CTRL, ROW_MASK, 0xF, false);
}
__device__ __forceinline__ uint32_t wave_incl_scan_u32(uint32_t v) {
  v = dpp_add_step<0x111, 0xF>(v);
  v = dpp_add_step<0x112, 0xF>(v);
  v = dpp_add_step<0x114, 0xF>(v);
  v = dpp_add_step<0x118, 0xF>(v);
  v = dpp_add_step<0x142, 0xA>(v);
  v = dpp_add_step<0x143, 0xC>(v);
  return v;
}
__device__ __forceinline__ uint32_t wave_sum(uint32_t v) {
#ifdef PM_WAVE_SUM_SHFL
#pragma unroll
  for (int o = 32; o > 0; o >>= 1) v += __shfl_xor(v, o, 64);
  return v;
#else
  return (uint32_t)__builtin_amdgcn_readlane((int)wave_incl_scan_u32(v), 63);
#endif
}
__device__ __forceinline__ uint32_t wave_min(uint32_t v) {
#pragma unroll
  for (int o = 32; o > 0; o >>= 1) v = min(v, (uint32_t)__shfl_xor(v, o, 64));
  return v;
}
struct KeyIdx {
  uint64_t k;
  uint32_t i;
};
__device__ __forceinline__ bool ki_less(uint64_t ka, uint32_t ia, uint64_t kb, uint32_t ib) {
  return ka < kb || (ka == kb && ia < ib);
}
__device__ __forceinline__ KeyIdx wave_min_ki(KeyIdx v) {
#pragma unroll
  for (int o = 32; o > 0; o >>= 1) {
    uint32_t lo = __shfl_xor((uint32_t)v.k, o, 64);
    uint32_t hi = __shfl_xor((uint32_t)(v.k >> 32), o, 64);
    uint32_t oi = __shfl_xor(v.i, o, 64);
    uint64_t ok = ((uint64_t)hi << 32) | lo;
    if (ki_less(ok, oi, v.k, v.i)) {
      v.k = ok;
      v.i = oi;
    }
  }
  return v;
}


__device__ __forceinline__ bool gpu_alt_meets(uint32_t wf, uint32_t wcount, uint32_t wmem, uint32_t wcls,
                                              const pm_gpu_alt_row& a, const uint32_t* __restrict__ model_bits,
                                              uint32_t words) {
  if (a.flags & PM_G_COUNT) {
    if (!(wf & PM_W_GPU_COUNT)) {
      if (a.count > 0) return false;
    } else if (wcount != a.count) {
      return false;
    }
  }
  if (a.flags & PM_G_MODEL) {
    if (!(wf & PM_W_GPU_MODEL)) return false;
    uint32_t word = model_bits[a.model_row * words + (wcls >> 5)];
    if (!((word >> (wcls & 31)) & 1u)) return false;
  }
  const bool mem_some = (wf & PM_W_GPU_MEM) != 0;
  if ((a.flags & PM_G_MEM) && (!mem_some || wmem < a.memory_mb)) return false;
  if ((a.flags & PM_G_MEM_MIN) && (!mem_some || wmem < a.memory_mb_min)) return false;
  if ((a.flags & PM_G_MEM_MAX) && (!mem_some || wmem > a.memory_mb_max)) return false;
  if ((wf & PM_W_GPU_COUNT) && mem_some) {
    const uint32_t total = wcount * wmem;
    if ((a.flags & PM_G_TOT_MIN) && total < a.total_memory_min) return false;
    if ((a.flags & PM_G_TOT_MAX) && total > a.total_memory_max) return false;
  }
  return true;
}

template <bool SLICED>
__device__ __forceinline__ void compat_body(const CompatArgs& p) {
  __shared__ uint64_t s_part[SLICED ? 256 : 1];
  const uint32_t lane = threadIdx.x & 63u, slice = (uint32_t)__builtin_amdgcn_readfirstlane((int)(threadIdx.x >> 6));
  const uint32_t w = SLICED ? blockIdx.x * 64u + lane : blockIdx.x * 256u + threadIdx.x;
  const bool in = w < p.W;
  if (!SLICED && !in) return;
  const uint32_t per = SLICED ? (p.n_cfgs + 3u) / 4u : p.n_cfgs;
  const uint32_t c_begin = SLICED ? (slice * per < p.n_cfgs ? slice * per : p.n_cfgs) : 0u;
  const uint32_t c_end = SLICED ? (c_begin + per < p.n_cfgs ? c_begin + per : p.n_cfgs) : p.n_cfgs;
  const uint32_t wr = in ? w : 0u;
  const uint32_t wf = p.flags[wr];
  const uint32_t wcount = p.gpu_count[wr], wmem = p.gpu_mem[wr], wcls = p.gpu_cls[wr];
  const uint32_t wcores = p.cpu_cores[wr], wram = p.ram[wr], wsto = p.storage[wr];
  uint64_t mask = 0;
  for (uint32_t c = c_begin; c < c_end; ++c) {
    const pm_config_row cfg = p.cfgs[c];
    bool ok;
    if (!(cfg.flags & PM_R_HAS_REQ)) {
      ok = true;
    } else if (!(wf & PM_W_HAS_SPECS)) {
      ok = false;
    } else {
      ok = true;
      if (cfg.flags & PM_R_CPU) {
        if (!(wf & PM_W_HAS_CPU)) ok = false;
        if ((cfg.flags & PM_R_CPU_CORES) && (!(wf & PM_W_CPU_CORES) || wcores < cfg.cpu_cores)) ok = false;
      }
      if ((cfg.flags & PM_R_RAM) && (!(wf & PM_W_RAM) || wram < cfg.ram_mb)) ok = false;
      if ((cfg.flags & PM_R_STORAGE) && (!(wf & PM_W_STORAGE) || wsto < cfg.storage_gb)) ok = false;
      if (cfg.alt_count) {
        bool any = false;
        if (wf & PM_W_HAS_GPU)
          for (uint32_t k = 0; k < cfg.alt_count; ++k)
            any |= gpu_alt_meets(wf, wcount, wmem, wcls, p.alts[cfg.alt_begin + k], p.model_bits, p.model_words);
        ok = ok && any;
      }
    }
    mask |= (uint64_t)ok << c;
  }
  if (!SLICED) {
    p.compat[w] = mask;
    return;
  }
  s_part[threadIdx.x] = mask;
  __syncthreads();
  if (slice == 0u && in) p.compat[w] = s_part[lane] | s_part[64u + lane] | s_part[128u + lane] | s_part[192u + lane];
}
__global__ __launch_bounds__(256) void compat_kernel(CompatArgs p) { compat_body<false>(p); }
__global__ __launch_bounds__(256) void compat_sliced_kernel(CompatArgs p) { compat_body<true>(p); }

__global__ __launch_bounds__(256) void triad_kernel(const double* __restrict__ b, const double* __restrict__ c,
                                                    double* __restrict__ a, size_t n) {
  for (size_t i = (size_t)blockIdx.x * 256u + threadIdx.x; i < n; i += (size_t)gridDim.x * 256u) a[i] = b[i] + 3.0 * c[i];
}

__device__ __forceinline__ void geo_of(double la, double lo, double* coslat, double* ux, double* uy, double* uz) {
  const double phi = la * PM_RAD, lam = lo * PM_RAD;
  const double c = cos(phi);
  *coslat = c;
  *ux = c * cos(lam);
  *uy = c * sin(lam);
  *uz = sin(phi);
}
__global__ __launch_bounds__(256) void geo_kernel(const double* __restrict__ lat, const double* __restrict__ lon,
                                                  double* __restrict__ coslat, double* __restrict__ ux,
                                                  double* __restrict__ uy, double* __restrict__ uz, uint32_t W) {
  const uint32_t w = blockIdx.x * 256u + threadIdx.x;
  if (w < W) geo_of(lat[w], lon[w], &coslat[w], &ux[w], &uy[w], &uz[w]);
}

__global__ __launch_bounds__(256) void update_rows_kernel(RowUpdateArgs p) {
  const uint32_t k = blockIdx.x * 256u + threadIdx.x;
  if (k >= p.n) return;
  const size_t n = p.n;
  const uint32_t w = p.u32_in[k];
  p.flags[w] = p.u32_in[1 * n + k];
  p.gpu_count[w] = p.u32_in[2 * n + k];
  p.gpu_mem[w] = p.u32_in[3 * n + k];
  p.gpu_cls[w] = p.u32_in[4 * n + k];
  p.cpu_cores[w] = p.u32_in[5 * n + k];
  p.ram[w] = p.u32_in[6 * n + k];
  p.storage[w] = p.u32_in[7 * n + k];
  p.addr_rank[w] = p.u32_in[8 * n + k];
  p.site[w] = p.u32_in[9 * n + k];
  const double la = p.lat_in[k], lo = p.lon_in[k];
  p.lat[w] = la;
  p.lon[w] = lo;
  geo_of(la, lo, &p.coslat[w], &p.ux[w], &p.uy[w], &p.uz[w]);
}


__global__ __launch_bounds__(256) void pair_init_kernel(uint32_t* __restrict__ first, uint32_t* __restrict__ count,
                                                        uint32_t R) {
  const uint32_t r = blockIdx.x * 256u + threadIdx.x;
  if (r < R) {
    first[r] = PM_NONE;
    count[r] = 0u;
  }
}

__device__ __forceinline__ void pair_fold(uint32_t* __restrict__ first, uint32_t* __restrict__ count, uint32_t r,
                                          uint32_t f, uint32_t cnt, bool atomic) {
  if (!atomic) {
    first[r] = f;
    count[r] = cnt;
  } else if (cnt) {
    atomicMin(&first[r], f);
    atomicAdd(&count[r], cnt);
  }
}

__global__ __launch_bounds__(256) void pair_sweep_scalar_kernel(const uint64_t* __restrict__ row_sel, uint32_t R,
                                                                const uint64_t* __restrict__ col_mask,
                                                                uint32_t c_begin, uint32_t c_end, uint32_t chunk,
                                                                uint32_t* __restrict__ first_out,
                                                                uint32_t* __restrict__ count_out, uint32_t atomic) {
  const uint32_t r = blockIdx.x * 256u + threadIdx.x;
  const uint32_t c0 = c_begin + blockIdx.y * chunk;
  const uint32_t c1 = min(c_end, c0 + chunk);
  const uint64_t sel = r < R ? row_sel[r] : 0ull;
  uint32_t first = PM_NONE, cnt = 0;
  for (uint32_t c = c0; c < c1; ++c) {
    const uint64_t m = col_mask[c];
    const bool hit = (m & sel) != 0ull;
    cnt += hit;
    first = hit ? min(first, c) : first;
  }
  if (r < R) pair_fold(first_out, count_out, r, first, cnt, atomic != 0u);
}

__global__ __launch_bounds__(256) void pair_select_scalar_kernel(const uint64_t* __restrict__ row_sel, uint32_t R,
                                                                 const uint64_t* __restrict__ col_mask,
                                                                 uint32_t c_begin, uint32_t c_end,
                                                                 const uint32_t* __restrict__ rank,
                                                                 uint32_t* __restrict__ out) {
  const uint32_t r = blockIdx.x * 256u + threadIdx.x;
  const uint64_t sel = r < R ? row_sel[r] : 0ull;
  uint32_t want = r < R ? rank[r] : PM_NONE;
  uint32_t res = PM_NONE, seen = 0;
  for (uint32_t c = c_begin; c < c_end; ++c) {
    const bool hit = (col_mask[c] & sel) != 0ull;
    res = (hit && seen == want) ? c : res;
    seen += hit;
  }
  if (r < R) out[r] = res;
}


__global__ __launch_bounds__(256) void build_planes_kernel(const uint64_t* __restrict__ col_mask, uint32_t n_cols,
                                                           uint32_t w_begin, uint32_t w_end, uint32_t stride,
                                                           uint32_t n_planes, uint64_t* __restrict__ planes) {
  const uint32_t lane = threadIdx.x & 63u;
  const uint32_t j = w_begin + ((blockIdx.x * 256u + threadIdx.x) >> 6);
  if (j >= w_end) return;
  const uint32_t c = j * 64u + lane;
  const uint64_t m = c < n_cols ? col_mask[c] : 0ull;
  for (uint32_t b = 0; b < n_planes; ++b) {
    const uint64_t word = __ballot((m >> b) & 1ull);
    if (lane == 0) planes[(size_t)b * stride + j] = word;
  }
  const uint64_t valid = n_planes >= 64u ? ~0ull : ((1ull << n_planes) - 1ull);
  const uint64_t any = __ballot((m & valid) != 0ull);
  if (lane == 0) planes[(size_t)n_planes * stride + j] = any;
}

template <uint32_t RPT>
__global__ __launch_bounds__(256) void pair_sweep_planes_kernel(const uint64_t* __restrict__ row_sel, uint32_t R,
                                                                const uint64_t* __restrict__ planes,
                                                                uint32_t stride, uint32_t w_begin, uint32_t w_end,
                                                                uint32_t n_planes, uint32_t words_per_split,
                                                                uint32_t words_per_piece,
                                                                uint32_t* __restrict__ first_out,
                                                                uint32_t* __restrict__ count_out, uint32_t atomic) {
  extern __shared__ uint64_t s_pl[];
  const uint32_t lds_stride = words_per_piece | 1u;
  const uint32_t r0 = blockIdx.x * (256u * RPT) + threadIdx.x;
  const uint32_t w0 = w_begin + blockIdx.y * words_per_split;
  const uint32_t w1 = min(w_end, w0 + words_per_split);
  const uint64_t valid = n_planes >= 64u ? ~0ull : ((1ull << n_planes) - 1ull);
  uint64_t sel[RPT], keep[RPT];
  uint32_t first[RPT], cnt[RPT], my_plane[RPT];
  bool single[RPT];
#pragma unroll
  for (uint32_t k = 0; k < RPT; ++k) {
    const uint32_t r = r0 + k * 256u;
    sel[k] = r < R ? (row_sel[r] & valid) : 0ull;
    if (sel[k] == valid && n_planes > 1u && n_planes < 64u) sel[k] = 1ull << n_planes;
    first[k] = PM_NONE;
    cnt[k] = 0;
    single[k] = __ballot((sel[k] & (sel[k] - 1ull)) != 0ull) == 0ull;
    my_plane[k] = sel[k] ? (uint32_t)__builtin_ctzll(sel[k]) : 0u;
    keep[k] = sel[k] ? ~0ull : 0ull;
  }
  for (uint32_t j0 = w0; j0 < w1; j0 += words_per_piece) {
    const uint32_t nj = min(words_per_piece, w1 - j0);
    __syncthreads();
    for (uint32_t b = 0; b <= n_planes; ++b)
      for (uint32_t j = threadIdx.x; j < nj; j += 256u) s_pl[b * lds_stride + j] = planes[(size_t)b * stride + j0 + j];
    __syncthreads();
#pragma unroll
    for (uint32_t k = 0; k < RPT; ++k) {
      if (single[k]) {
        const uint64_t* pl = s_pl + my_plane[k] * lds_stride;
        uint32_t j = 0;
        for (; j + 4u <= nj; j += 4u) {
          const uint64_t h0 = pl[j], h1 = pl[j + 1u], h2 = pl[j + 2u], h3 = pl[j + 3u];
          const uint32_t before = cnt[k];
          cnt[k] += __popcll(h0) + __popcll(h1) + __popcll(h2) + __popcll(h3);
          if (before == 0u && cnt[k] != 0u) {
            const uint32_t u = h0 ? 0u : (h1 ? 1u : (h2 ? 2u : 3u));
            const uint64_t h = h0 ? h0 : (h1 ? h1 : (h2 ? h2 : h3));
            first[k] = (j0 + j + u) * 64u + __builtin_ctzll(h);
          }
        }
        for (; j < nj; ++j) {
          const uint64_t h = pl[j];
          if (h && cnt[k] == 0u) first[k] = (j0 + j) * 64u + __builtin_ctzll(h);
          cnt[k] += __popcll(h);
        }
      } else {
        for (uint32_t j = 0; j < nj; ++j) {
          uint64_t hits = 0;
          uint64_t s = sel[k];
          while (s) {
            const uint32_t b = __builtin_ctzll(s);
            s &= s - 1;
            hits |= s_pl[b * lds_stride + j];
          }
          cnt[k] += __popcll(hits);
          if (hits && first[k] == PM_NONE) first[k] = (j0 + j) * 64u + __builtin_ctzll(hits);
        }
      }
    }
  }
#pragma unroll
  for (uint32_t k = 0; k < RPT; ++k) {
    const uint32_t r = r0 + k * 256u;
    if (!keep[k]) {
      first[k] = PM_NONE;
      cnt[k] = 0u;
    }
    if (r < R) pair_fold(first_out, count_out, r, first[k], cnt[k], atomic != 0u);
  }
}

__global__ __launch_bounds__(256) void pair_select_planes_kernel(const uint64_t* __restrict__ row_sel, uint32_t R,
                                                                 const uint64_t* __restrict__ planes,
                                                                 uint32_t stride, uint32_t w_begin, uint32_t w_end,
                                                                 uint32_t n_planes, const uint32_t* __restrict__ rank,
                                                                 uint32_t* __restrict__ out) {
  const uint32_t r = blockIdx.x * 256u + threadIdx.x;
  if (r >= R) return;
  const uint64_t valid = n_planes >= 64u ? ~0ull : ((1ull << n_planes) - 1ull);
  const uint64_t sel = row_sel[r] & valid;
  uint32_t want = rank[r];
  uint32_t res = PM_NONE;
  if (want != PM_NONE) {
    for (uint32_t j = w_begin; j < w_end; ++j) {
      uint64_t hits = 0, s = sel;
      while (s) {
        const uint32_t b = __builtin_ctzll(s);
        s &= s - 1;
        hits |= planes[(size_t)b * stride + j];
      }
      const uint32_t pc = __popcll(hits);
      if (want < pc) {
        for (uint32_t k = 0; k < want; ++k) hits &= hits - 1;
        res = j * 64u + __builtin_ctzll(hits);
        break;
      }
      want -= pc;
    }
  }
  out[r] = res;
}

__global__ __launch_bounds__(64) void task_prefix_kernel(const uint64_t* __restrict__ live, uint32_t w_begin,
                                                         uint32_t w_end, uint32_t* __restrict__ prefix) {
  const uint32_t lane = threadIdx.x;
  uint32_t acc = 0;
  for (uint32_t j0 = w_begin; j0 < w_end; j0 += 64u) {
    const uint32_t j = j0 + lane;
    const uint32_t cnt = j < w_end ? (uint32_t)__popcll(live[j]) : 0u;
    const uint32_t incl = wave_incl_scan_u32(cnt);
    if (j < w_end) prefix[j] = acc + incl - cnt;
    acc += __shfl(incl, 63, 64);
  }
}
__global__ __launch_bounds__(256) void task_delete_kernel(const uint32_t* __restrict__ slots, uint32_t n,
                                                          uint64_t* __restrict__ tmask,
                                                          uint64_t* __restrict__ live, uint64_t* __restrict__ planes,
                                                          uint32_t stride, uint32_t n_planes) {
  const uint32_t k = blockIdx.x * 256u + threadIdx.x;
  if (k >= n) return;
  const uint32_t u = slots[k];
  const uint64_t bit = 1ull << (u & 63u);
  tmask[u] = 0ull;
  atomicAnd((unsigned long long*)&live[u >> 6], ~bit);
  for (uint32_t b = 0; b <= n_planes; ++b)
    atomicAnd((unsigned long long*)&planes[(size_t)b * stride + (u >> 6)], ~bit);
}
__global__ __launch_bounds__(256) void task_compact_kernel(const uint32_t* __restrict__ first_u,
                                                           const uint32_t* __restrict__ count_u, uint32_t u_begin,
                                                           uint32_t u_end, const uint64_t* __restrict__ live,
                                                           const uint32_t* __restrict__ prefix,
                                                           uint32_t* __restrict__ first_out,
                                                           uint32_t* __restrict__ count_out) {
  const uint32_t u = u_begin + blockIdx.x * 256u + threadIdx.x;
  if (u >= u_end) return;
  const uint64_t w = live[u >> 6];
  if (!((w >> (u & 63u)) & 1ull)) return;
  const uint32_t pos = prefix[u >> 6] + (uint32_t)__popcll(w & ((1ull << (u & 63u)) - 1ull));
  first_out[pos] = first_u[u - u_begin];
  count_out[pos] = count_u[u - u_begin];
}


__device__ __forceinline__ uint64_t splitmix64_mix(uint64_t x) {
  uint64_t z = x + 0x9E3779B97F4A7C15ull;
  z = (z ^ (z >> 30)) * 0xBF58476D1CE4E5B9ull;
  z = (z ^ (z >> 27)) * 0x94D049BB133111EBull;
  return z ^ (z >> 31);
}

#define PM_INTERN_EMPTY (~0ull)
__global__ __launch_bounds__(256) void task_intern_insert_kernel(const uint64_t* __restrict__ tmask,
                                                                 const uint64_t* __restrict__ live, uint32_t u_begin,
                                                                 uint32_t u_end, uint64_t valid,
                                                                 unsigned long long* __restrict__ keys, uint32_t h_mask,
                                                                 uint32_t* __restrict__ overflow) {
  const uint32_t u = u_begin + blockIdx.x * 256u + threadIdx.x;
  if (u >= u_end || !((live[u >> 6] >> (u & 63u)) & 1ull)) return;
  const uint64_t m = tmask[u] & valid;
  if (m == 0ull) return;
  uint32_t h = (uint32_t)splitmix64_mix(m) & h_mask;
  for (uint32_t probe = 0; probe <= h_mask; ++probe, h = (h + 1u) & h_mask) {
    const unsigned long long k = keys[h];
    if (k == m) return;
    if (k == PM_INTERN_EMPTY) {
      const unsigned long long old = atomicCAS(&keys[h], PM_INTERN_EMPTY, (unsigned long long)m);
      if (old == PM_INTERN_EMPTY || old == m) return;
    }
  }
  *overflow = 1u;
}
__global__ __launch_bounds__(256) void task_intern_number_kernel(const unsigned long long* __restrict__ keys,
                                                                 uint32_t n_slots, uint32_t* __restrict__ vals,
                                                                 uint32_t* __restrict__ counter,
                                                                 uint64_t* __restrict__ umask, uint32_t cap_u) {
  const uint32_t s = blockIdx.x * 256u + threadIdx.x;
  if (s >= n_slots) return;
  const unsigned long long k = keys[s];
  if (k == PM_INTERN_EMPTY) return;
  const uint32_t id = atomicAdd(counter, 1u);
  vals[s] = id;
  if (id < cap_u) umask[id] = k;
}
__global__ __launch_bounds__(256) void task_compact_class_kernel(const uint32_t* __restrict__ first_c,
                                                                 const uint32_t* __restrict__ count_c,
                                                                 const uint64_t* __restrict__ tmask, uint64_t valid,
                                                                 const unsigned long long* __restrict__ keys,
                                                                 const uint32_t* __restrict__ vals, uint32_t h_mask,
                                                                 uint32_t u_begin, uint32_t u_end,
                                                                 const uint64_t* __restrict__ live,
                                                                 const uint32_t* __restrict__ prefix,
                                                                 uint32_t* __restrict__ first_out,
                                                                 uint32_t* __restrict__ count_out) {
  const uint32_t u = u_begin + blockIdx.x * 256u + threadIdx.x;
  if (u >= u_end) return;
  const uint64_t w = live[u >> 6];
  if (!((w >> (u & 63u)) & 1ull)) return;
  const uint32_t pos = prefix[u >> 6] + (uint32_t)__popcll(w & ((1ull << (u & 63u)) - 1ull));
  const uint64_t m = tmask[u] & valid;
  uint32_t first = PM_NONE, count = 0u;
  if (m != 0ull) {
    uint32_t h = (uint32_t)splitmix64_mix(m) & h_mask;
    while (keys[h] != m) h = (h + 1u) & h_mask;
    const uint32_t id = vals[h];
    first = first_c[id];
    count = count_c[id];
  }
  first_out[pos] = first;
  count_out[pos] = count;
}

__global__ __launch_bounds__(256) void worker_selector_kernel(const int32_t* __restrict__ group_of,
                                                              const uint32_t* __restrict__ g_cfg, uint32_t R,
                                                              const uint32_t* __restrict__ rows,
                                                              uint64_t* __restrict__ sel) {
  const uint32_t r = blockIdx.x * 256u + threadIdx.x;
  if (r >= R) return;
  const int32_t g = group_of[rows ? rows[r] : r];
  sel[r] = g >= 0 ? (1ull << g_cfg[g]) : 0ull;
}

__global__ __launch_bounds__(256) void chooser_rank_kernel(const int32_t* __restrict__ group_of,
                                                           const uint64_t* __restrict__ g_id,
                                                           const uint32_t* __restrict__ count, uint32_t R,
                                                           const uint32_t* __restrict__ rows, uint64_t seed,
                                                           uint32_t* __restrict__ rank) {
  const uint32_t r = blockIdx.x * 256u + threadIdx.x;
  if (r >= R) return;
  const int32_t g = group_of[rows ? rows[r] : r];
  const uint32_t n = count[r];
  rank[r] = (g >= 0 && n) ? (uint32_t)(splitmix64_mix(seed ^ g_id[g]) % n) : PM_NONE;
}

__global__ __launch_bounds__(256) void eligible_selector_kernel(const uint32_t* __restrict__ wflags,
                                                                const int32_t* __restrict__ group_of,
                                                                const uint64_t* __restrict__ compat, uint64_t enabled,
                                                                uint32_t W, const uint8_t* __restrict__ shard,
                                                                uint32_t my_rank, uint64_t* __restrict__ sel) {
  const uint32_t w = blockIdx.x * 256u + threadIdx.x;
  if (w >= W) return;
  const uint32_t f = wflags[w];
  const bool e = (f & PM_W_HEALTHY) && (f & PM_W_HAS_P2P) && group_of[w] < 0 && (!shard || shard[w] == my_rank);
  sel[w] = e ? (compat[w] & enabled) : 0ull;
}

__global__ __launch_bounds__(256) void group_rank_kernel(const int32_t* __restrict__ group_of,
                                                         const uint32_t* __restrict__ g_n,
                                                         const uint32_t* __restrict__ g_off,
                                                         const uint32_t* __restrict__ members,
                                                         const uint32_t* __restrict__ addr_rank, uint32_t W,
                                                         uint32_t* __restrict__ rank_in_group,
                                                         uint32_t* __restrict__ by_rank) {
  const uint32_t w = blockIdx.x * 256u + threadIdx.x;
  if (w >= W) return;
  const int32_t g = group_of[w];
  if (g < 0) {
    rank_in_group[w] = 0;
    return;
  }
  const uint32_t n = g_n[g], off = g_off[g], my = addr_rank[w];
  uint32_t idx = 0;
  for (uint32_t k = 0; k < n; ++k) idx += addr_rank[members[off + k]] < my;
  rank_in_group[w] = idx;
  by_rank[off + idx] = w;
}

__global__ __launch_bounds__(256) void match_prep_kernel(MatchPrepArgs p) {
  const uint32_t w = blockIdx.x * 256u + threadIdx.x;
  if (w < p.G) p.g_task_next[w] = p.g_task[w];
  if (w >= p.W) return;
  const int32_t g = p.group_of[w];
  p.first[w] = PM_NONE;
  p.count[w] = 0u;
  if (g < 0) {
    p.sel[w] = 0ull;
    p.rank_in_group[w] = 0;
    return;
  }
  p.sel[w] = 1ull << p.g_cfg[g];
  const uint32_t n = p.g_n[g], off = p.g_off[g], my = p.addr_rank[w];
  uint32_t idx = 0;
  for (uint32_t k = 0; k < n; ++k) idx += p.addr_rank[p.members[off + k]] < my;
  p.rank_in_group[w] = idx;
  p.by_rank[off + idx] = w;
}

__device__ __forceinline__ uint32_t task_position(const uint64_t* __restrict__ live, const uint32_t* __restrict__ prefix,
                                                  uint32_t u) {
  return prefix[u >> 6] + (uint32_t)__popcll(live[u >> 6] & ((1ull << (u & 63u)) - 1ull));
}

__global__ __launch_bounds__(256) void claim_publish_kernel(ClaimArgs p) {
  const uint32_t r = blockIdx.x * 256u + threadIdx.x;
  const bool in = r < p.R;
  if (!in && !p.h_table) return;
  const uint32_t w = !in ? 0u : p.rows ? p.rows[r] : r;
  const int32_t g = in ? p.group_of[w] : -1;
  pm_assignment a;
  a.task = PM_NONE;
  a.group_slot = PM_NONE;
  a.group_index = 0;
  a.group_size = 0;
  a.next_worker = PM_NONE;
  a.group_id = 0;
  uint32_t t = PM_NONE;
  if (g >= 0) {
    t = p.g_task[g];
    if (t == PM_NONE) {
      t = p.chosen[r];
      if (t != PM_NONE) p.g_task_next[g] = t;
    }
    const uint32_t n = p.g_n[g], off = p.g_off[g];
    const uint32_t idx = p.rank_in_group[w];
    a.task = (t == PM_NONE || p.rows) ? t : task_position(p.t_live, p.t_prefix, t);
    a.group_slot = (uint32_t)g;
    a.group_index = idx;
    a.group_size = n;
    a.next_worker = p.by_rank[off + ((idx + 1u == n) ? 0u : idx + 1u)];
    a.group_id = p.g_id[g];
  }
  if (p.rows) {
    p.table[r] = a;
    return;
  }
  if (in) {
    p.table[w] = a;
    p.task_col[w] = a.task;
  }
  if (p.h_table) {
    static_assert(sizeof(pm_assignment) == 32, "a row is two 16-byte pieces");
    __shared__ uint4 s_rows[512];
    s_rows[2u * threadIdx.x] = make_uint4(a.task, a.group_slot, a.group_index, a.group_size);
    s_rows[2u * threadIdx.x + 1u] = make_uint4(a.next_worker, 0u, (uint32_t)a.group_id, (uint32_t)(a.group_id >> 32));
    if (g >= 0 && a.group_index == 0u) p.h_gtask[g] = t;
    __syncthreads();
    const uint32_t row0 = blockIdx.x * 256u;
    const uint32_t n16 = 2u * (p.R - row0 < 256u ? p.R - row0 : 256u);
    uint4* const dst = reinterpret_cast<uint4*>(p.h_table + row0);
    for (uint32_t k = threadIdx.x; k < n16; k += 256u) dst[k] = s_rows[k];
  }
}

__global__ __launch_bounds__(256) void table_scatter_kernel(const pm_assignment* __restrict__ x,
                                                            const uint32_t* __restrict__ xrow, uint32_t W,
                                                            pm_assignment* __restrict__ table,
                                                            uint32_t* __restrict__ task_col,
                                                            uint32_t* __restrict__ g_task_next,
                                                            const uint64_t* __restrict__ t_live,
                                                            const uint32_t* __restrict__ t_prefix) {
  const uint32_t w = blockIdx.x * 256u + threadIdx.x;
  if (w >= W) return;
  pm_assignment a = x[xrow[w]];
  if (a.group_slot != PM_NONE && a.task != PM_NONE) g_task_next[a.group_slot] = a.task;
  if (a.task != PM_NONE) a.task = task_position(t_live, t_prefix, a.task);
  table[w] = a;
  task_col[w] = a.task;
}


__global__ __launch_bounds__(256) void newest_kernel(const int64_t* __restrict__ created_at,
                                                     const uint64_t* __restrict__ live, uint32_t t_begin, uint32_t T,
                                                     unsigned long long* __restrict__ best_key,
                                                     uint32_t* __restrict__ best_idx_by_block,
                                                     long long* __restrict__ best_val_by_block) {
  __shared__ long long s_v[4];
  __shared__ uint32_t s_i[4];
  long long bv = INT64_MIN;
  uint32_t bi = PM_NONE;
  for (uint32_t t = t_begin + blockIdx.x * 256u + threadIdx.x; t < T; t += gridDim.x * 256u) {
    if (!((live[t >> 6] >> (t & 63u)) & 1ull)) continue;
    const long long v = created_at[t];
    if (bi == PM_NONE || v >= bv) {
      bv = v;
      bi = t;
    }
  }
#pragma unroll
  for (int o = 32; o > 0; o >>= 1) {
    const uint32_t lo = __shfl_xor((uint32_t)bv, o, 64), hi = __shfl_xor((uint32_t)((uint64_t)bv >> 32), o, 64);
    const long long ov = (long long)(((uint64_t)hi << 32) | lo);
    const uint32_t oi = __shfl_xor(bi, o, 64);
    if (oi != PM_NONE && (bi == PM_NONE || ov > bv || (ov == bv && oi > bi))) {
      bv = ov;
      bi = oi;
    }
  }
  const uint32_t wave = threadIdx.x >> 6;
  if ((threadIdx.x & 63u) == 0) {
    s_v[wave] = bv;
    s_i[wave] = bi;
  }
  __syncthreads();
  if (threadIdx.x == 0) {
    for (int k = 1; k < 4; ++k)
      if (s_i[k] != PM_NONE && (bi == PM_NONE || s_v[k] > bv || (s_v[k] == bv && s_i[k] > bi))) {
        bv = s_v[k];
        bi = s_i[k];
      }
    best_idx_by_block[blockIdx.x] = bi;
    best_val_by_block[blockIdx.x] = bv;
  }
  (void)best_key;
}

#include "pm_validate.inc"
#include "pm_propose.inc"
#include "pm_prep.inc"
#include "pm_carve_kernel.inc"
#include "pm_stream.inc"

#include "pm_report.inc"
#include "pm_launch.inc"
}
```

### protocol_amd/csrc/pm_launch.inc

```

void launch_compat(const CompatArgs& a, hipStream_t s) {
  if (a.W == 0) return;
  if (a.W < 65536u)
    hipLaunchKernelGGL(compat_sliced_kernel, dim3((a.W + 63u) / 64u), dim3(256), 0, s, a);
  else
    hipLaunchKernelGGL(compat_kernel, dim3((a.W + 255u) / 256u), dim3(256), 0, s, a);
}
void launch_triad(const double* b, const double* c, double* a, size_t n, hipStream_t s) {
  hipLaunchKernelGGL(triad_kernel, dim3(256 * 32), dim3(256), 0, s, b, c, a, n);
}
void launch_row_network_test(const uint64_t* keys, const uint32_t* sites, uint32_t n_waves, uint32_t n_per_wave, uint32_t slot_bits,
                             uint64_t ulps, uint32_t upto, uint64_t* rows_out, uint32_t* mismatches, hipStream_t s) {
  hipLaunchKernelGGL(row_network_test_kernel, dim3(n_waves / 4u), dim3(256), 0, s, keys, sites, n_per_wave, slot_bits, ulps, upto, rows_out,
                     mismatches);
}
void launch_distance_key_test(const double* in, const double* geo, uint32_t n, uint32_t mode, double* out, hipStream_t s) {
  if (n == 0) return;
  hipLaunchKernelGGL(distance_key_test_kernel, dim3((n + 255u) / 256u), dim3(256), 0, s, in, geo, n, mode, out);
}
void launch_geo(const double* lat, const double* lon, double* coslat, double* ux, double* uy, double* uz, uint32_t W,
                hipStream_t s) {
  if (W == 0) return;
  hipLaunchKernelGGL(geo_kernel, dim3((W + 255u) / 256u), dim3(256), 0, s, lat, lon, coslat, ux, uy, uz, W);
}
void launch_update_rows(const RowUpdateArgs& a, hipStream_t s) {
  if (a.n == 0) return;
  hipLaunchKernelGGL(update_rows_kernel, dim3((a.n + 255u) / 256u), dim3(256), 0, s, a);
}
void launch_worker_selector(const int32_t* group_of, const uint32_t* g_cfg, uint32_t R, const uint32_t* rows,
                            uint64_t* sel, hipStream_t s) {
  if (R == 0) return;
  hipLaunchKernelGGL(worker_selector_kernel, dim3((R + 255u) / 256u), dim3(256), 0, s, group_of, g_cfg, R, rows, sel);
}
void launch_chooser_rank(const int32_t* group_of, const uint64_t* g_id, const uint32_t* count, uint32_t R,
                         const uint32_t* rows, uint64_t seed, uint32_t* rank, hipStream_t s) {
  if (R == 0) return;
  hipLaunchKernelGGL(chooser_rank_kernel, dim3((R + 255u) / 256u), dim3(256), 0, s, group_of, g_id, count, R, rows,
                     seed, rank);
}
void launch_eligible_selector(const uint32_t* wflags, const int32_t* group_of, const uint64_t* compat,
                              uint64_t enabled, uint32_t W, const uint8_t* shard, uint32_t my_rank, uint64_t* sel,
                              hipStream_t s) {
  if (W == 0) return;
  hipLaunchKernelGGL(eligible_selector_kernel, dim3((W + 255u) / 256u), dim3(256), 0, s, wflags, group_of, compat,
                     enabled, W, shard, my_rank, sel);
}
void launch_table_scatter(const pm_assignment* x, const uint32_t* xrow, uint32_t W, pm_assignment* table,
                          uint32_t* task_col, uint32_t* g_task_next, const uint64_t* t_live, const uint32_t* t_prefix,
                          hipStream_t s) {
  if (W == 0) return;
  hipLaunchKernelGGL(table_scatter_kernel, dim3((W + 255u) / 256u), dim3(256), 0, s, x, xrow, W, table, task_col,
                     g_task_next, t_live, t_prefix);
}
void launch_group_rank(const int32_t* group_of, const uint32_t* g_n, const uint32_t* g_off, const uint32_t* members,
                       const uint32_t* addr_rank, uint32_t W, uint32_t* rank_in_group, uint32_t* by_rank,
                       hipStream_t s) {
  if (W == 0) return;
  hipLaunchKernelGGL(group_rank_kernel, dim3((W + 255u) / 256u), dim3(256), 0, s, group_of, g_n, g_off, members,
                     addr_rank, W, rank_in_group, by_rank);
}
void launch_match_prep(const MatchPrepArgs& a, hipStream_t s) {
  const uint32_t n = a.W > a.G ? a.W : a.G;
  if (n == 0) return;
  hipLaunchKernelGGL(match_prep_kernel, dim3((n + 255u) / 256u), dim3(256), 0, s, a);
}
void launch_claim_publish(const ClaimArgs& a, hipStream_t s) {
  if (a.R == 0) return;
  hipLaunchKernelGGL(claim_publish_kernel, dim3((a.R + 255u) / 256u), dim3(256), 0, s, a);
}

void launch_build_planes(const uint64_t* col_mask, uint32_t n_cols, uint32_t c_begin, uint32_t c_end, uint32_t stride,
                         uint32_t n_planes, uint64_t* planes, hipStream_t s) {
  const uint32_t w0 = c_begin / 64u, w1 = (c_end + 63u) / 64u;
  if (w1 <= w0) return;
  hipLaunchKernelGGL(build_planes_kernel, dim3(((w1 - w0) * 64u + 255u) / 256u), dim3(256), 0, s, col_mask, n_cols, w0,
                     w1, stride, n_planes, planes);
}

void launch_pair_sweep(int variant, const uint64_t* row_sel, uint32_t R, const uint64_t* col_mask,
                       const uint64_t* planes, uint32_t c_begin, uint32_t c_end, uint32_t stride, uint32_t n_planes,
                       uint32_t* first, uint32_t* count, hipStream_t s, bool inited) {
  if (R == 0) return;
  const uint32_t rb = (R + 255u) / 256u;
#ifndef PM_SWEEP_RPT4_MIN_RB
#define PM_SWEEP_RPT4_MIN_RB 256u
#endif
  const bool rpt4 = rb >= PM_SWEEP_RPT4_MIN_RB;
#ifndef PM_SWEEP_RPT_N
#define PM_SWEEP_RPT_N 4u
#endif
  const uint32_t rbe = (rpt4 && rb < 1024u) ? (rb + PM_SWEEP_RPT_N - 1u) / PM_SWEEP_RPT_N : rb;
  const uint32_t want_split = ((R <= 16384u ? 512u : (rpt4 && rb < 1024u) ? 1400u : 2048u) + rbe - 1u) / rbe;
  const uint32_t n_cols = c_end > c_begin ? c_end - c_begin : 0u;
  if (n_cols == 0) {
    if (!inited) hipLaunchKernelGGL(pair_init_kernel, dim3(rb), dim3(256), 0, s, first, count, R);
    return;
  }
  if (variant == 1) {
    uint32_t n_split = want_split < n_cols ? want_split : n_cols;
    const uint32_t chunk = (n_cols + n_split - 1u) / n_split;
    n_split = (n_cols + chunk - 1u) / chunk;
    if (n_split > 1u && !inited) hipLaunchKernelGGL(pair_init_kernel, dim3(rb), dim3(256), 0, s, first, count, R);
    hipLaunchKernelGGL(pair_sweep_scalar_kernel, dim3(rb, n_split), dim3(256), 0, s, row_sel, R, col_mask, c_begin,
                       c_end, chunk, first, count, n_split > 1u ? 1u : 0u);
    return;
  }
  const uint32_t w0 = c_begin / 64u, w1 = (c_end + 63u) / 64u, n_words = w1 - w0;
  uint32_t n_split = want_split < n_words ? want_split : n_words;
  const uint32_t wps = (n_words + n_split - 1u) / n_split;
  n_split = (n_words + wps - 1u) / wps;
  const uint32_t lds_cap_words = ((48u * 1024u / 8u) / (n_planes + 1u)) - 1u;
  const uint32_t wpp = wps < lds_cap_words ? wps : lds_cap_words;
  const size_t lds = (size_t)(n_planes + 1u) * (wpp | 1u) * sizeof(uint64_t);
  if (n_split > 1u && !inited) hipLaunchKernelGGL(pair_init_kernel, dim3(rb), dim3(256), 0, s, first, count, R);
  if (rpt4)
    hipLaunchKernelGGL(pair_sweep_planes_kernel<PM_SWEEP_RPT_N>, dim3((rb + PM_SWEEP_RPT_N - 1u) / PM_SWEEP_RPT_N, n_split), dim3(256), lds, s,
                       row_sel, R, planes, stride, w0, w1, n_planes, wps, wpp, first, count, n_split > 1u ? 1u : 0u);
  else
    hipLaunchKernelGGL(pair_sweep_planes_kernel<1u>, dim3(rb, n_split), dim3(256), lds, s, row_sel, R, planes, stride, w0,
                       w1, n_planes, wps, wpp, first, count, n_split > 1u ? 1u : 0u);
}

void launch_pair_select(int variant, const uint64_t* row_sel, uint32_t R, const uint64_t* col_mask,
                        const uint64_t* planes, uint32_t c_begin, uint32_t c_end, uint32_t stride, uint32_t n_planes,
                        const uint32_t* rank, uint32_t* out, hipStream_t s) {
  if (R == 0) return;
  const uint32_t rb = (R + 255u) / 256u;
  if (variant == 1) {
    hipLaunchKernelGGL(pair_select_scalar_kernel, dim3(rb), dim3(256), 0, s, row_sel, R, col_mask, c_begin, c_end,
                       rank, out);
  } else {
    hipLaunchKernelGGL(pair_select_planes_kernel, dim3(rb), dim3(256), 0, s, row_sel, R, planes, stride,
                       c_begin / 64u, (c_end + 63u) / 64u, n_planes, rank, out);
  }
}

void launch_task_prefix(const uint64_t* live, uint32_t w_begin, uint32_t w_end, uint32_t* prefix, hipStream_t s) {
  if (w_end <= w_begin) return;
  hipLaunchKernelGGL(task_prefix_kernel, dim3(1), dim3(64), 0, s, live, w_begin, w_end, prefix);
}
void launch_task_delete(const uint32_t* slots, uint32_t n, uint64_t* tmask, uint64_t* live, uint64_t* planes,
                        uint32_t stride, uint32_t n_planes, hipStream_t s) {
  if (!n) return;
  hipLaunchKernelGGL(task_delete_kernel, dim3((n + 255u) / 256u), dim3(256), 0, s, slots, n, tmask, live, planes,
                     stride, n_planes);
}
void launch_task_intern(const uint64_t* tmask, const uint64_t* live, uint32_t u_begin, uint32_t u_end, uint64_t valid,
                        uint64_t* keys, uint32_t n_slots, uint32_t* vals, uint32_t* counter_and_overflow, uint64_t* umask,
                        uint32_t cap_u, hipStream_t s) {
  (void)hipMemsetAsync(keys, 0xFF, size_t(n_slots) * 8, s);
  (void)hipMemsetAsync(counter_and_overflow, 0, 8, s);
  if (u_end > u_begin)
    hipLaunchKernelGGL(task_intern_insert_kernel, dim3((u_end - u_begin + 255u) / 256u), dim3(256), 0, s, tmask, live, u_begin,
                       u_end, valid, (unsigned long long*)keys, n_slots - 1u, counter_and_overflow + 1);
  hipLaunchKernelGGL(task_intern_number_kernel, dim3((n_slots + 255u) / 256u), dim3(256), 0, s,
                     (const unsigned long long*)keys, n_slots, vals, counter_and_overflow, umask, cap_u);
}
void launch_task_compact_class(const uint32_t* first_c, const uint32_t* count_c, const uint64_t* tmask, uint64_t valid,
                               const uint64_t* keys, const uint32_t* vals, uint32_t n_slots, uint32_t u_begin,
                               uint32_t u_end, const uint64_t* live, const uint32_t* prefix, uint32_t* first_out,
                               uint32_t* count_out, hipStream_t s) {
  if (u_end <= u_begin) return;
  hipLaunchKernelGGL(task_compact_class_kernel, dim3((u_end - u_begin + 255u) / 256u), dim3(256), 0, s, first_c, count_c,
                     tmask, valid, (const unsigned long long*)keys, vals, n_slots - 1u, u_begin, u_end, live, prefix,
                     first_out, count_out);
}
void launch_task_compact(const uint32_t* first_u, const uint32_t* count_u, uint32_t u_begin, uint32_t u_end,
                         const uint64_t* live, const uint32_t* prefix, uint32_t* first_out, uint32_t* count_out,
                         hipStream_t s) {
  if (u_end <= u_begin) return;
  hipLaunchKernelGGL(task_compact_kernel, dim3((u_end - u_begin + 255u) / 256u), dim3(256), 0, s, first_u, count_u,
                     u_begin, u_end, live, prefix, first_out, count_out);
}

void launch_newest(const int64_t* created_at, const uint64_t* live, uint32_t t_begin, uint32_t t_end,
                   uint32_t* idx_by_block, long long* val_by_block, uint32_t n_blocks, hipStream_t s) {
  hipLaunchKernelGGL(newest_kernel, dim3(n_blocks), dim3(256), 0, s, created_at, live, t_begin, t_end,
                     (unsigned long long*)nullptr, idx_by_block, val_by_block);
}

void launch_carve_propose(const CarveArgs* d_args, uint32_t W, hipStream_t s) {
  uint32_t blocks = (W + 3u) / 4u;
  if (blocks > 2048u) blocks = 2048u;
  if (blocks == 0) blocks = 1;
  hipLaunchKernelGGL(carve_propose_kernel, dim3(blocks), dim3(256), 0, s, d_args);
}

__global__ __launch_bounds__(256) void group_ids_kernel(uint64_t* __restrict__ g_id, uint32_t* __restrict__ g_task,
                                                        uint32_t n, uint64_t state) {
  const uint32_t k = blockIdx.x * 256u + threadIdx.x;
  if (k >= n) return;
  uint64_t z = state + (uint64_t)(k + 1u) * 0x9E3779B97F4A7C15ull;
  z = (z ^ (z >> 30)) * 0xBF58476D1CE4E5B9ull;
  z = (z ^ (z >> 27)) * 0x94D049BB133111EBull;
  g_id[k] = z ^ (z >> 31);
  g_task[k] = PM_NONE;
}
void launch_group_ids(uint64_t* g_id, uint32_t* g_task, uint32_t n, uint64_t rng_state, hipStream_t s) {
  if (!n) return;
  hipLaunchKernelGGL(group_ids_kernel, dim3((n + 255u) / 256u), dim3(256), 0, s, g_id, g_task, n, rng_state);
}

uint32_t launch_carve_prep(const CarveArgs* d_args, uint32_t W, hipStream_t s) {
  uint32_t blocks = ((W + 63u) / 64u + PREP_WAVES - 1u) / PREP_WAVES;
  if (blocks == 0) blocks = 1;
  hipLaunchKernelGGL(carve_prep_count_kernel, dim3(blocks), dim3(256), 0, s, d_args);
  hipLaunchKernelGGL(carve_prep_place_kernel, dim3(blocks), dim3(256), 0, s, d_args);
  return 2u;
}
uint32_t launch_carve_elig(CarveArgs* d_args, const CarveArgs* put, uint32_t W, uint32_t n_bound, uint32_t index_min, uint32_t start_ci,
                           bool fresh, uint32_t n_groups0, uint32_t n_members0, hipStream_t s) {
  uint32_t blocks = ((W + 63u) / 64u + PREP_WAVES - 1u) / PREP_WAVES;
  if (blocks == 0) blocks = 1;
  if (put) {
    CarveArgWords w{};
    __builtin_memcpy(w.w, put, sizeof(CarveArgs));
    hipLaunchKernelGGL(carve_elig_count_put_kernel, dim3(blocks), dim3(256), 0, s, w, reinterpret_cast<uint32_t*>(d_args),
                       fresh ? 1u : 0u, n_groups0, n_members0);
  } else {
    hipLaunchKernelGGL(carve_elig_count_kernel, dim3(blocks), dim3(256), 0, s, d_args, fresh ? 1u : 0u, n_groups0, n_members0);
  }
  hipLaunchKernelGGL(carve_elig_place_kernel, dim3(blocks), dim3(256), 0, s, d_args, start_ci);
  if (!index_min || n_bound < index_min) return 2u;
  const uint32_t pb = (n_bound + 255u) / 256u;
  hipLaunchKernelGGL(cell_count_kernel, dim3(pb), dim3(256), 0, s, d_args);
  const uint32_t sb = (PM_CELL_TABLE + CELL_SCAN_PER_BLOCK - 1u) / CELL_SCAN_PER_BLOCK;
  hipLaunchKernelGGL(cell_scan_sums_kernel, dim3(sb), dim3(256), 0, s, d_args);
  hipLaunchKernelGGL(cell_scan_apply_kernel, dim3(sb), dim3(256), 0, s, d_args);
  hipLaunchKernelGGL(cell_place_kernel, dim3(pb), dim3(256), 0, s, d_args);
  return 6u;
}
__global__ __launch_bounds__(256) void carve_args_put_kernel(CarveArgWords a, uint32_t* __restrict__ dst) {
  for (uint32_t i = threadIdx.x; i < sizeof(CarveArgWords) / 4u; i += 256u) dst[i] = a.w[i];
}
hipError_t launch_carve_args_put(const CarveArgs& a, CarveArgs* d_args, hipStream_t s) {
  CarveArgWords w{};
  __builtin_memcpy(w.w, &a, sizeof(CarveArgs));
  hipLaunchKernelGGL(carve_args_put_kernel, dim3(1), dim3(256), 0, s, w, reinterpret_cast<uint32_t*>(d_args));
  return hipGetLastError();
}
void launch_carve_apply(const CarveArgs* d_args, uint32_t W, hipStream_t s) {
  uint32_t blocks = ((W + 63u) / 64u + PREP_WAVES - 1u) / PREP_WAVES;
  if (blocks == 0) blocks = 1;
  hipLaunchKernelGGL(carve_prep_count_kernel, dim3(blocks), dim3(256), 0, s, d_args);
}

hipError_t carve_kernels_init() {
  hipError_t e = hipFuncSetAttribute((const void*)carve_kernel, hipFuncAttributeMaxDynamicSharedMemorySize, (int)PM_CARVE_LDS_BYTES);
  if (e != hipSuccess) return e;
  return hipFuncSetAttribute((const void*)carve_stream_kernel, hipFuncAttributeMaxDynamicSharedMemorySize, (int)PM_STREAM_LDS_BYTES);
}

#ifdef PM_ROW_BENCH
hipError_t launch_row_bench(const CarveArgs* d_args, uint32_t seed, uint32_t ci, uint32_t reps, uint32_t mode, unsigned long long* d_out, hipStream_t s) {
  hipError_t e = hipMemcpyToSymbolAsync(HIP_SYMBOL(g_rowb_mode), &mode, 4, 0, hipMemcpyHostToDevice, s);
  if (e != hipSuccess) return e;
  e = hipFuncSetAttribute((const void*)carve_row_bench_kernel, hipFuncAttributeMaxDynamicSharedMemorySize, (int)PM_STREAM_LDS_BYTES);
  if (e != hipSuccess) return e;
  hipLaunchKernelGGL(carve_row_bench_kernel, dim3(1), dim3(CARVE_THREADS), PM_STREAM_LDS_BYTES, s, d_args, seed, ci, reps, d_out);
  static const uint32_t zero = 0u;
  (void)hipMemcpyToSymbolAsync(HIP_SYMBOL(g_rowb_mode), &zero, 4, 0, hipMemcpyHostToDevice, s);
  return hipGetLastError();
}
#endif
hipError_t launch_carve(const CarveArgs* d_args, uint32_t flags, uint32_t start_ci, size_t lds_bytes, hipStream_t s) {
  hipLaunchKernelGGL(carve_kernel, dim3(1), dim3(CARVE_THREADS), lds_bytes, s, d_args, flags, start_ci);
  return hipGetLastError();
}


void launch_merge_place(const CarveArgs* d_args, uint32_t n_order, uint32_t n_groups0, uint32_t n_members0, uint32_t steps0,
                        hipStream_t s) {
  const uint32_t blocks = ((n_order ? n_order : 1u) + 255u) / 256u;
  hipLaunchKernelGGL(merge_place_kernel, dim3(blocks), dim3(256), 0, s, d_args, n_groups0, n_members0, steps0);
}

__global__ __launch_bounds__(256) void scatter_const_kernel(uint32_t* __restrict__ dst, const uint32_t* __restrict__ idx, uint32_t n,
                                                            uint32_t v) {
  const uint32_t k = blockIdx.x * 256u + threadIdx.x;
  if (k < n) dst[idx[k]] = v;
}
__global__ __launch_bounds__(256) void scatter_pairs_kernel(uint32_t* __restrict__ dst, const uint32_t* __restrict__ pairs, uint32_t n) {
  const uint32_t k = blockIdx.x * 256u + threadIdx.x;
  if (k < n) dst[pairs[2u * k]] = pairs[2u * k + 1u];
}
void launch_scatter_const(uint32_t* dst, const uint32_t* idx, uint32_t n, uint32_t v, hipStream_t s) {
  if (n) hipLaunchKernelGGL(scatter_const_kernel, dim3((n + 255u) / 256u), dim3(256), 0, s, dst, idx, n, v);
}
void launch_scatter_pairs(uint32_t* dst, const uint32_t* pairs, uint32_t n, hipStream_t s) {
  if (n) hipLaunchKernelGGL(scatter_pairs_kernel, dim3((n + 255u) / 256u), dim3(256), 0, s, dst, pairs, n);
}
```

### protocol_amd/csrc/pm_prep.inc

```

#define PREP_WAVES 4

__device__ __forceinline__ void plan_batch(const CarveArgs& p) {
  BatchDesc d = {};
  d.planned = 1u;
  d.ci0 = p.status->cur_ci;
  d.total_available = p.status->total_available;
  *p.desc = d;
}

__global__ __launch_bounds__(256) void carve_prep_count_kernel(const CarveArgs* __restrict__ pa) {
  const CarveArgs& p = *pa;
  const auto st = G(p.status);
  const uint32_t tid = threadIdx.x, lane = tid & 63u, wave = tid >> 6;
  const uint32_t wave_g = blockIdx.x * PREP_WAVES + wave;
  {
    const uint32_t g_lo = st->g_lo, g_hi = st->g_hi, n_waves = gridDim.x * PREP_WAVES;
    for (uint32_t g = g_lo + wave_g; g < g_hi; g += n_waves) {
      const uint32_t off = G(p.g_off)[g], gn = G(p.g_n)[g];
      for (uint32_t k = lane; k < gn; k += 64u) G(p.group_of)[G(p.members)[off + k]] = (int32_t)g;
    }
  }
  if (st->state != CARVE_STATE_RUNNING) {
    if (blockIdx.x == 0 && tid == 0) p.desc->planned = 0u;
    return;
  }
#ifdef PM_BATCH_LOG
  if (blockIdx.x == 0 && tid == 0) p.status->prof[5] = ~0ull;
#endif
  const uint32_t ci0 = st->cur_ci;
  if (blockIdx.x == 0 && tid == 0) plan_batch(p);
  if (ci0 >= p.n_avail) return;
  __shared__ uint32_t s_cnt[PREP_WAVES][PM_MAX_CONFIGS];
  const uint32_t n = st->n_eligible, n_words = (n + 63u) >> 6;
  const uint32_t j = wave_g;
  uint64_t m = 0;
  if (j < n_words) {
    const uint32_t i = j * 64u + lane;
    const uint64_t aw = G(p.alive_g)[j];
    const bool alive = i < n && ((aw >> lane) & 1ull);
    m = alive ? G((const uint64_t*)p.c_compat)[i] : 0ull;
    if (lane == 0) {
      G(p.alive_snap)[j] = aw;
      G(p.bits_scratch)[p.bits_stride + j] = 0ull;
    }
  }
  for (uint32_t ci = ci0; ci < p.n_avail; ++ci) {
    const uint32_t cnt = (uint32_t)__popcll(__ballot((m >> p.avail_cfg[ci]) & 1ull));
    if (lane == 0) s_cnt[wave][ci] = cnt;
  }
  __syncthreads();
  if (tid >= ci0 && tid < p.n_avail) {
    uint32_t sum = 0;
#pragma unroll
    for (uint32_t w = 0; w < PREP_WAVES; ++w) sum += s_cnt[w][tid];
    G(p.prep_block_counts)[(size_t)blockIdx.x * PM_MAX_CONFIGS + tid] = sum;
    if (sum) atomicAdd(&p.prep_counts[tid], sum);
  }
}

__global__ __launch_bounds__(256) void carve_prep_place_kernel(const CarveArgs* __restrict__ pa) {
  const CarveArgs& p = *pa;
  const auto st = G(p.status);
  const auto D = G((const BatchDesc*)p.desc);
  if (st->state != CARVE_STATE_RUNNING || !D->planned) return;
  const uint32_t tid = threadIdx.x, lane = tid & 63u, wave = tid >> 6;
  __shared__ uint32_t s_red[PREP_WAVES + 4];
  __shared__ uint32_t s_bits[PREP_WAVES][64];
#ifdef PM_BATCH_LOG
  const uint64_t pl_t0 = __builtin_amdgcn_s_memtime();
  if (tid == 0) atomicMin((unsigned long long*)&p.status->prof[5], (unsigned long long)pl_t0);
#endif
  const uint32_t n = st->n_eligible, n_words = (n + 63u) >> 6;
  const uint32_t total_available = D->total_available;
  uint32_t ci = D->ci0, n_list = 0;
  for (; ci < p.n_avail; ++ci) {
    const uint32_t min_s = p.min_size[ci];
    if (total_available < min_s) continue;
    n_list = G((const uint32_t*)p.prep_counts)[ci];
    if (n_list < min_s || n_list == 0) continue;
    break;
  }
  const bool none = ci >= p.n_avail;
  const bool props = !none && p.proximity && n_list <= PM_CARVE_BIG_SLOTS && p.max_size[ci] - 1u < PM_PROP_KMAX &&
                     !(p.debug_mem_above && n_list > p.debug_mem_above);
  uint32_t cell_g = props ? st->cell_g : 0u;
  if (cell_g && p.prune_mode == 1u && (uint64_t)n_list * n_list < (uint64_t)p.prune_factor * st->n_indexed) cell_g = 0u;
  if (!none) {
    const uint64_t cbit = 1ull << p.avail_cfg[ci];
    uint32_t part = 0;
    for (uint32_t b = tid; b < blockIdx.x; b += 256u) part += G((const uint32_t*)p.prep_block_counts)[(size_t)b * PM_MAX_CONFIGS + ci];
    part = wave_sum(part);
    if (lane == 0) s_red[wave] = part;
    const uint32_t j = blockIdx.x * PREP_WAVES + wave;
    const uint32_t i = j * 64u + lane;
    const uint32_t ic = i < n ? i : (n ? n - 1u : 0u);
    const uint64_t aw = j < n_words ? G((const uint64_t*)p.alive_snap)[j] : 0ull;
    const uint64_t lg = j < n_words ? G(p.loc_g)[j] : 0ull;
    const uint64_t cm = n ? G((const uint64_t*)p.c_compat)[ic] : 0ull;
    const uint32_t ow = n ? G(p.order)[ic] : 0u;
    const uint32_t os = n ? G(p.c_site)[ic] : 0u;
    const double la = n ? G(p.c_lat)[ic] : 0.0, lo = n ? G(p.c_lon)[ic] : 0.0, co = n ? G(p.c_cos)[ic] : 0.0;
    const double vx = n ? G(p.c_ux)[ic] : 0.0, vy = n ? G(p.c_uy)[ic] : 0.0, vz = n ? G(p.c_uz)[ic] : 0.0;
    const bool c = i < n && ((aw >> lane) & 1ull) && (cm & cbit) != 0ull;
    const uint64_t bal = __ballot(c);
    const uint32_t cnt = (uint32_t)__popcll(bal);
    if (lane == 0) s_red[PREP_WAVES + wave] = cnt;
    __syncthreads();
#ifdef PM_BATCH_LOG
    if (tid == 0) atomicAdd((unsigned long long*)&p.status->prof[14], (unsigned long long)(__builtin_amdgcn_s_memtime() - pl_t0));
#endif
    uint32_t off = 0;
#pragma unroll
    for (uint32_t w = 0; w < PREP_WAVES; ++w) off += s_red[w];
    for (uint32_t w = 0; w < wave; ++w) off += s_red[PREP_WAVES + w];
    const uint32_t rank = (uint32_t)__popcll(bal & ((1ull << lane) - 1ull));
    const uint32_t has_loc = (uint32_t)(lg >> lane) & 1u;
    if (c) {
      const uint32_t s = off + rank;
      G(p.slot_pos)[s] = i | (has_loc << 31);
      G(p.slot_wid)[s] = ow;
      G(p.cc_lat)[s] = la;
      G(p.cc_lon)[s] = lo;
      G(p.cc_cos)[s] = co;
      G(p.cc_ux)[s] = vx;
      G(p.cc_uy)[s] = vy;
      G(p.cc_uz)[s] = vz;
      G(p.cc_site)[s] = os;
      s_bits[wave][rank] = has_loc;
    }
    if (cell_g && i < n && has_loc) G(p.cs_slot)[G((const uint32_t*)p.cs_of_pos)[i]] = c ? off + rank : 0xFFFFFFFFu;
    __syncthreads();
    const uint64_t locm = __ballot(lane < cnt && s_bits[wave][lane] != 0u);
    if (lane == 0 && locm) {
      const auto loc = (unsigned long long*)(p.bits_scratch + p.bits_stride);
      const uint32_t sh = off & 63u;
      atomicOr(&loc[off >> 6], (unsigned long long)(locm << sh));
      if (sh && (locm >> (64u - sh))) atomicOr(&loc[(off >> 6) + 1u], (unsigned long long)(locm >> (64u - sh)));
    }
  }
#ifdef PM_BATCH_LOG
  if (tid == 0) atomicAdd((unsigned long long*)&p.status->prof[15], (unsigned long long)(__builtin_amdgcn_s_memtime() - pl_t0));
#endif
  __builtin_amdgcn_fence(__ATOMIC_RELEASE, "workgroup");
  __syncthreads();
#ifdef PM_BATCH_LOG
  if (tid == 0) {
    const uint64_t dt = __builtin_amdgcn_s_memtime() - pl_t0;
    atomicAdd((unsigned long long*)&p.status->prof[8], (unsigned long long)dt);
    atomicMax((unsigned long long*)&p.status->prof[9], (unsigned long long)dt);
    atomicAdd((unsigned long long*)&p.status->prof[10], 1ull);
  }
#endif
  if (tid == 0) s_red[0] = atomicAdd(&p.prep_counts[PM_MAX_CONFIGS], 1u);
  __syncthreads();
  if (s_red[0] != gridDim.x - 1u) return;
  __builtin_amdgcn_fence(__ATOMIC_ACQUIRE, "agent");
#ifdef PM_BATCH_LOG
  const uint64_t pl_t1 = __builtin_amdgcn_s_memtime();
#endif
  if (none) {
    if (tid == 0) {
      p.desc->ci = p.n_avail;
      p.desc->none = 1u;
#ifdef PM_BATCH_LOG
      const uint32_t k = p.status->blog_n++;
      if (k < 512u) p.status->blog[3u * k] = p.status->blog[3u * k + 1u] = p.status->blog[3u * k + 2u] = 0u;
#endif
    }
    return;
  }
  const uint32_t lw = (n_list + 63u) >> 6;
  const auto alive = G(p.bits_scratch);
  for (uint32_t w = tid; w < lw; w += 256u)
    alive[w] = (w + 1u < lw || (n_list & 63u) == 0u) ? ~0ull : ((1ull << (n_list & 63u)) - 1ull);
  __syncthreads();
  uint32_t prop_k = 0, limit = 0, n_seeds = 0;
  const uint32_t max_s = p.max_size[ci];
  if (props) {
    const uint32_t k = max_s - 1u + PM_PROP_RESERVE;
    prop_k = k < PM_PROP_KMAX ? k : PM_PROP_KMAX;
    if (wave == 0) {
      prop_limit_scan(p, n_list, lane, &limit, &n_seeds, cell_g != 0u);
      if (lane == 0) {
        s_red[1] = limit;
        s_red[2] = n_seeds;
      }
    }
    __syncthreads();
    limit = s_red[1];
    n_seeds = s_red[2];
    prop_seed_slots(p, limit, tid, 256u);
  }
  if (tid == 0) {
    BatchDesc* d = p.desc;
    d->ci = ci;
    d->n_list = n_list;
    d->prop_k = prop_k;
    d->prop_limit = limit;
    d->rows_pr = (n_seeds + p.dist_world - 1u) / p.dist_world;
    d->n_seeds = n_seeds;
    d->cell_g = cell_g;
    d->valid = 1u;
    if (cell_g) p.status->pruned_batches += 1u;
#ifdef PM_BATCH_LOG
    {
      const uint64_t pl_t2 = __builtin_amdgcn_s_memtime();
      p.status->prof[11] += pl_t1 - p.status->prof[5];
      p.status->prof[12] += pl_t2 - pl_t1;
      p.status->prof[13] += 1ull;
    }
    const uint32_t k = p.status->blog_n++;
    if (k < 512u) {
      p.status->blog[3u * k] = n_list;
      p.status->blog[3u * k + 1u] = n_seeds;
      p.status->blog[3u * k + 2u] = cell_g;
    }
#endif
  }
}


__device__ __forceinline__ bool row_eligible(const CarveArgs& p, uint32_t w) {
  if (w >= p.W) return false;
  const uint32_t f = G(p.wflags)[w];
  return (f & PM_W_HEALTHY) && (f & PM_W_HAS_P2P) && G(p.group_of)[w] < 0;
}

__device__ __forceinline__ void carve_elig_count_body(const CarveArgs& p, uint32_t fresh, uint32_t n_groups0, uint32_t n_members0) {
  const uint32_t tid = threadIdx.x, lane = tid & 63u, wave = tid >> 6;
  if (blockIdx.x == 0) {
    if (fresh) {
      uint32_t* w = (uint32_t*)p.status;
      for (uint32_t k = tid; k < (uint32_t)(sizeof(CarveStatus) / 4u); k += 256u) w[k] = 0u;
    }
    if (p.stream && tid < PM_STREAM_CTL_WORDS) p.stream_ctl[tid] = 0u;
    __syncthreads();
    if (fresh && tid == 0) {
      p.status->state = CARVE_STATE_RUNNING;
      p.status->n_groups = n_groups0;
      p.status->n_members = n_members0;
    }
  }
  if (!fresh && G(p.status)->state != CARVE_STATE_RUNNING) return;
  __shared__ uint32_t s_c[PREP_WAVES];
  const uint32_t j = blockIdx.x * PREP_WAVES + wave;
  const uint64_t bal = __ballot(row_eligible(p, j * 64u + lane));
  if (lane == 0) {
    s_c[wave] = (uint32_t)__popcll(bal);
    if (j < ((p.W + 63u) >> 6)) G(p.loc_g)[j] = 0ull;
  }
  if (p.stream && lane < p.n_avail && j < ((p.W + 63u) >> 6)) G(p.cfgbits)[(size_t)lane * p.bits_stride + j] = 0ull;
  if (blockIdx.x == 0 && tid <= PM_MAX_CONFIGS + 1u) p.prep_counts[tid] = 0u;
  __syncthreads();
  if (tid == 0) {
    uint32_t sum = 0;
#pragma unroll
    for (uint32_t w = 0; w < PREP_WAVES; ++w) sum += s_c[w];
    G(p.prep_block_counts)[(size_t)blockIdx.x * PM_MAX_CONFIGS] = sum;
  }
}
__global__ __launch_bounds__(256) void carve_elig_count_kernel(const CarveArgs* __restrict__ pa, uint32_t fresh, uint32_t n_groups0,
                                                               uint32_t n_members0) {
  carve_elig_count_body(*pa, fresh, n_groups0, n_members0);
}
struct CarveArgWords {
  uint32_t w[(sizeof(CarveArgs) + 3u) / 4u];
};
static_assert(sizeof(CarveArgWords) + 32u <= 4096u, "the argument block fits a kernarg segment");
static_assert(sizeof(CarveArgWords) == sizeof(CarveArgs), "the block is whole words");
__global__ __launch_bounds__(256) void carve_elig_count_put_kernel(CarveArgWords a, uint32_t* __restrict__ dst, uint32_t fresh,
                                                                   uint32_t n_groups0, uint32_t n_members0) {
  if (blockIdx.x == 0)
    for (uint32_t i = threadIdx.x; i < sizeof(CarveArgWords) / 4u; i += 256u) dst[i] = a.w[i];
  carve_elig_count_body(reinterpret_cast<const CarveArgs&>(a), fresh, n_groups0, n_members0);
}

__global__ __launch_bounds__(256) void carve_elig_place_kernel(const CarveArgs* __restrict__ pa, uint32_t start_ci) {
  const CarveArgs& p = *pa;
  const auto st = G(p.status);
  if (st->state != CARVE_STATE_RUNNING) return;
  const uint32_t tid = threadIdx.x, lane = tid & 63u, wave = tid >> 6;
  __shared__ uint32_t s_red[2 * PREP_WAVES + 2];
  __shared__ uint32_t s_bits[PREP_WAVES][64];
  __shared__ uint64_t s_cm[PREP_WAVES][64];
  uint32_t part = 0;
  for (uint32_t b = tid; b < blockIdx.x; b += 256u) part += G((const uint32_t*)p.prep_block_counts)[(size_t)b * PM_MAX_CONFIGS];
  part = wave_sum(part);
  if (lane == 0) s_red[wave] = part;
  const uint32_t w = (blockIdx.x * PREP_WAVES + wave) * 64u + lane;
  const bool e = row_eligible(p, w);
  const uint64_t bal = __ballot(e);
  const uint32_t cnt = (uint32_t)__popcll(bal);
  if (lane == 0) s_red[PREP_WAVES + wave] = cnt;
  __syncthreads();
  uint32_t off = 0;
#pragma unroll
  for (uint32_t k = 0; k < PREP_WAVES; ++k) off += s_red[k];
  for (uint32_t k = 0; k < wave; ++k) off += s_red[PREP_WAVES + k];
  const uint32_t rank = (uint32_t)__popcll(bal & ((1ull << lane) - 1ull));
  if (e) {
    const uint32_t i = off + rank;
    const uint32_t has_loc = (G(p.wflags)[w] & PM_W_HAS_LOC) ? 1u : 0u;
    G(p.order)[i] = w;
    G(p.c_lat)[i] = G(p.lat)[w];
    G(p.c_lon)[i] = G(p.lon)[w];
    G(p.c_cos)[i] = G(p.coslat)[w];
    G(p.c_ux)[i] = G(p.ux)[w];
    G(p.c_uy)[i] = G(p.uy)[w];
    G(p.c_uz)[i] = G(p.uz)[w];
    G(p.c_site)[i] = G(p.site)[w];
    if (p.stream) pack_store(p.c_pack, i, G(p.ux)[w], G(p.uy)[w], G(p.uz)[w], G(p.site)[w], has_loc);
    const uint64_t cmw = G(p.compat)[w];
    G(p.c_compat)[i] = cmw;
    s_bits[wave][rank] = has_loc;
    s_cm[wave][rank] = cmw;
  }
  __syncthreads();
  const uint64_t locm = __ballot(lane < cnt && s_bits[wave][lane] != 0u);
  if (lane == 0 && locm) {
    const auto loc = (unsigned long long*)p.loc_g;
    const uint32_t sh = off & 63u;
    atomicOr(&loc[off >> 6], (unsigned long long)(locm << sh));
    if (sh && (locm >> (64u - sh))) atomicOr(&loc[(off >> 6) + 1u], (unsigned long long)(locm >> (64u - sh)));
  }
  if (p.stream) {
    const uint64_t cmr = lane < cnt ? s_cm[wave][lane] : 0ull;
    const uint32_t sh = off & 63u;
    for (uint32_t ci = 0; ci < p.n_avail; ++ci) {
      const uint64_t bits = __ballot((cmr >> p.avail_cfg[ci]) & 1ull);
      if (lane == 0 && bits) {
        const auto cb = (unsigned long long*)(p.cfgbits + (size_t)ci * p.bits_stride);
        atomicOr(&cb[off >> 6], (unsigned long long)(bits << sh));
        if (sh && (bits >> (64u - sh))) atomicOr(&cb[(off >> 6) + 1u], (unsigned long long)(bits >> (64u - sh)));
      }
    }
  }
  __builtin_amdgcn_fence(__ATOMIC_RELEASE, "workgroup");
  __syncthreads();
  if (tid == 0) s_red[0] = atomicAdd(&p.prep_counts[PM_MAX_CONFIGS + 1u], 1u);
  __syncthreads();
  if (s_red[0] != gridDim.x - 1u) return;
  __threadfence();
  uint32_t total = 0;
  for (uint32_t b = tid; b < gridDim.x; b += 256u) total += G((const uint32_t*)p.prep_block_counts)[(size_t)b * PM_MAX_CONFIGS];
  total = wave_sum(total);
  __syncthreads();
  if (lane == 0) s_red[1u + wave] = total;
  __syncthreads();
  const uint32_t n = s_red[1] + s_red[2] + s_red[3] + s_red[4];
  const uint32_t n_words = (n + 63u) >> 6;
  for (uint32_t j = tid; j < n_words; j += 256u) {
    const uint64_t all = (j + 1u < n_words || (n & 63u) == 0u) ? ~0ull : ((1ull << (n & 63u)) - 1ull);
    G(p.alive_g)[j] = all;
    if (p.stream) G(p.bits_scratch)[j] = all;
  }
  if (tid <= PM_MAX_CONFIGS + 1u) p.prep_counts[tid] = 0u;
  if (tid == 0) {
    st->n_eligible = n;
    st->total_available = n;
    st->cur_ci = start_ci;
    st->need_prep = 1u;
    st->g_lo = st->g_hi = st->n_groups;
  }
}

__global__ __launch_bounds__(256) void cell_count_kernel(const CarveArgs* __restrict__ pa) {
  const CarveArgs& p = *pa;
  const auto st = G(p.status);
  if (st->state != CARVE_STATE_RUNNING) return;
  const uint32_t n = st->n_eligible;
  const bool forced = p.prune_mode >= 2u;
  const uint32_t g = (p.prune_mode && p.proximity && (forced || n >= PM_CELL_AUTO_N))
                         ? cell_g_for(forced && n >= 64u && n < PM_CELL_MIN_N ? PM_CELL_MIN_N : n) : 0u;
  if (blockIdx.x == 0 && threadIdx.x == 0) {
    st->cell_g = g;
    st->n_indexed = 0u;
  }
  if (!g) return;
  const uint32_t i = blockIdx.x * 256u + threadIdx.x;
  if (i >= n) return;
  if (!bit_at(G((const uint64_t*)p.loc_g), i)) {
    G(p.pos_cell)[i] = 0xFFFFFFFFu;
    return;
  }
  const uint32_t c = (cell_coord(G(p.c_uz)[i], g) * g + cell_coord(G(p.c_uy)[i], g)) * g + cell_coord(G(p.c_ux)[i], g);
  G(p.pos_cell)[i] = c;
  G(p.pos_rank)[i] = atomicAdd(&p.cell_cnt[c], 1u);
}

#define CELL_SCAN_PER_BLOCK 1024u
static_assert((PM_CELL_TABLE + CELL_SCAN_PER_BLOCK - 1u) / CELL_SCAN_PER_BLOCK <= 320u, "block sums fit one look of 256 + 64 threads");
__global__ __launch_bounds__(256) void cell_scan_sums_kernel(const CarveArgs* __restrict__ pa) {
  const CarveArgs& p = *pa;
  const auto st = G(p.status);
  if (st->state != CARVE_STATE_RUNNING) return;
  const uint32_t g = st->cell_g;
  if (!g) return;
  const uint32_t total = g * g * g, n_blocks = (total + CELL_SCAN_PER_BLOCK - 1u) / CELL_SCAN_PER_BLOCK;
  if (blockIdx.x >= n_blocks) return;
  const uint32_t tid = threadIdx.x, lane = tid & 63u, wave = tid >> 6;
  __shared__ uint32_t s_w[4];
  __shared__ uint32_t s_last;
  const auto cnt = G((const uint32_t*)p.cell_cnt);
  const uint32_t i0 = blockIdx.x * CELL_SCAN_PER_BLOCK + tid * 4u;
  uint32_t v = 0;
#pragma unroll
  for (uint32_t k = 0; k < 4u; ++k) v += i0 + k < total ? cnt[i0 + k] : 0u;
  v = wave_sum(v);
  if (lane == 0) s_w[wave] = v;
  __syncthreads();
  const auto blk = p.cell_start + PM_CELL_TABLE;
  if (tid == 0) {
    blk[blockIdx.x] = s_w[0] + s_w[1] + s_w[2] + s_w[3];
    __threadfence();
    s_last = atomicAdd(&blk[320], 1u) == n_blocks - 1u ? 1u : 0u;
  }
  __syncthreads();
  if (!s_last) return;
  __threadfence();
  if (wave == 0) {
    uint32_t carry = 0;
    for (uint32_t c0 = 0; c0 < n_blocks; c0 += 64u) {
      const uint32_t c = c0 + lane;
      const uint32_t x = c < n_blocks ? G((const uint32_t*)blk)[c] : 0u;
      const uint32_t incl = wave_incl_scan_u32(x);
      if (c < n_blocks) blk[c] = carry + incl - x;
      carry += (uint32_t)__builtin_amdgcn_readlane((int)incl, 63);
    }
    if (lane == 0) {
      blk[320] = 0u;
      p.cell_start[total] = carry;
      st->n_indexed = carry;
    }
  }
}
__global__ __launch_bounds__(256) void cell_scan_apply_kernel(const CarveArgs* __restrict__ pa) {
  const CarveArgs& p = *pa;
  const auto st = G((const CarveStatus*)p.status);
  if (st->state != CARVE_STATE_RUNNING) return;
  const uint32_t g = st->cell_g;
  if (!g) return;
  const uint32_t total = g * g * g, n_blocks = (total + CELL_SCAN_PER_BLOCK - 1u) / CELL_SCAN_PER_BLOCK;
  if (blockIdx.x >= n_blocks) return;
  const uint32_t tid = threadIdx.x, lane = tid & 63u, wave = tid >> 6;
  __shared__ uint32_t s_w[4];
  const auto cnt = G(p.cell_cnt);
  const auto start = G(p.cell_start);
  const uint32_t i0 = blockIdx.x * CELL_SCAN_PER_BLOCK + tid * 4u;
  uint32_t v[4];
#pragma unroll
  for (uint32_t k = 0; k < 4u; ++k) v[k] = i0 + k < total ? cnt[i0 + k] : 0u;
  const uint32_t mine = v[0] + v[1] + v[2] + v[3];
  const uint32_t incl = wave_incl_scan_u32(mine);
  if (lane == 63u) s_w[wave] = incl;
  __syncthreads();
  uint32_t run = G((const uint32_t*)(p.cell_start + PM_CELL_TABLE))[blockIdx.x] + incl - mine;
  for (uint32_t w = 0; w < wave; ++w) run += s_w[w];
#pragma unroll
  for (uint32_t k = 0; k < 4u; ++k) {
    if (i0 + k < total) {
      start[i0 + k] = run;
      cnt[i0 + k] = 0u;
    }
    run += v[k];
  }
}

__global__ __launch_bounds__(256) void cell_place_kernel(const CarveArgs* __restrict__ pa) {
  const CarveArgs& p = *pa;
  const auto st = G((const CarveStatus*)p.status);
  if (st->state != CARVE_STATE_RUNNING || !st->cell_g) return;
  const uint32_t i = blockIdx.x * 256u + threadIdx.x;
  if (i >= st->n_eligible) return;
  const uint32_t c = G((const uint32_t*)p.pos_cell)[i];
  if (c == 0xFFFFFFFFu) {
    G(p.cs_of_pos)[i] = 0xFFFFFFFFu;
    return;
  }
  const uint32_t e = G((const uint32_t*)p.cell_start)[c] + G((const uint32_t*)p.pos_rank)[i];
  G(p.cs_of_pos)[i] = e;
  if (p.stream) {
    G(p.cs_slot)[e] = i;
    pack_store(p.cs_pack, e, G((const double*)p.c_ux)[i], G((const double*)p.c_uy)[i], G((const double*)p.c_uz)[i],
               G((const uint32_t*)p.c_site)[i], 1u);
  }
  G(p.cs_ux)[e] = G((const double*)p.c_ux)[i];
  G(p.cs_uy)[e] = G((const double*)p.c_uy)[i];
  G(p.cs_uz)[e] = G((const double*)p.c_uz)[i];
  G(p.cs_site)[e] = G((const uint32_t*)p.c_site)[i];
}


__global__ __launch_bounds__(256) void merge_place_kernel(const CarveArgs* __restrict__ pa, uint32_t n_groups0, uint32_t n_members0,
                                                          uint32_t steps0) {
  const CarveArgs& p = *pa;
  const uint32_t tid = threadIdx.x, lane = tid & 63u;
  const uint32_t n = p.n_order, n_words = (n + 63u) >> 6;
  if (blockIdx.x == 0) {
    uint32_t* w = (uint32_t*)p.status;
    for (uint32_t k = tid; k < (uint32_t)(sizeof(CarveStatus) / 4u); k += 256u) w[k] = 0u;
    if (tid < PM_STREAM_CTL_WORDS) p.stream_ctl[tid] = 0u;
    __syncthreads();
    if (tid == 0) {
      p.status->state = CARVE_STATE_RUNNING;
      p.status->n_groups = n_groups0;
      p.status->n_members = n_members0;
      p.status->steps_total = steps0;
      p.status->n_eligible = n;
      p.status->total_available = n;
      p.status->g_lo = p.status->g_hi = n_groups0;
    }
  }
  const uint32_t i = blockIdx.x * 256u + tid;
  bool has_loc = false;
  if (i < n) {
    const uint32_t w = G(p.order)[i];
    has_loc = (G(p.wflags)[w] & PM_W_HAS_LOC) != 0u;
    G(p.c_lat)[i] = G(p.lat)[w];
    G(p.c_lon)[i] = G(p.lon)[w];
    G(p.c_cos)[i] = G(p.coslat)[w];
    G(p.c_ux)[i] = G(p.ux)[w];
    G(p.c_uy)[i] = G(p.uy)[w];
    G(p.c_uz)[i] = G(p.uz)[w];
    G(p.c_site)[i] = G(p.site)[w];
    G(p.c_compat)[i] = G(p.compat)[w];
    pack_store(p.c_pack, i, G(p.ux)[w], G(p.uy)[w], G(p.uz)[w], G(p.site)[w], has_loc ? 1u : 0u);
  }
  const uint64_t bl = __ballot(has_loc), ba = __ballot(i < n);
  const uint32_t j = i >> 6;
  if (lane == 0 && j < n_words) {
    G(p.loc_g)[j] = bl;
    G(p.cfgbits)[j] = ba;
    G(p.alive_g)[j] = ba;
    G(p.bits_scratch)[j] = ba;
  }
}
```

### protocol_amd/csrc/pm_stream.inc

```

enum { SLW_TREQ = PM_STREAM_TP,
       SLW_PAY,
       SLW_TISSUED,
       SLW_SCANW, SLW_SCANLO, SLW_SCANHI,
       SLW_TIMEOUTS,
       SLW_LA,
       SLW_TEND,
       SLW_ACKT, SLW_ACKP0, SLW_ACKP1, SLW_ACKP2, SLW_ACKP3, SLW_ACKP4,
       SLW_NCAND,
       SLW_P_CI, SLW_P_CI1, SLW_P_PAY, SLW_P_PAY1, SLW_P_MAX, SLW_P_MAX1, SLW_P_T0, SLW_P_T01, SLW_P_CNT, SLW_P_CNT1,
       SLW_P_SCANW, SLW_P_SCANW1, SLW_P_SCANLO, SLW_P_SCANLO1, SLW_P_SCANHI, SLW_P_SCANHI1,
       SLW_WORDS };
static_assert(SLW_TREQ == PM_STREAM_SLW_TREQ && SLW_PAY == PM_STREAM_SLW_PAY, "the words carve_fast_steps reads");
static_assert(SLW_WORDS <= PM_STREAM_TP + 32u, "ticket state fits its LDS region");
#ifndef STREAM_NPARK
#define STREAM_NPARK 5u
#endif
#ifndef STREAM_PARK_NB
#define STREAM_PARK_NB 16u
#endif
#ifndef STREAM_NAP_TICKETER
#define STREAM_NAP_TICKETER 4
#endif
#ifndef STREAM_NAP_PARK
// ... 2170 lines not shown
__global__ __launch_bounds__(CARVE_THREADS) void carve_row_bench_kernel(const CarveArgs* __restrict__ pa, uint32_t s, uint32_t ci, uint32_t reps,
                                                                        unsigned long long* __restrict__ out) {
  const CarveArgs& p = *pa;
  extern __shared__ __attribute__((aligned(16))) unsigned char s_raw[];
  const uint32_t lane = threadIdx.x & 63u, wave = threadIdx.x >> 6;
  if (wave != 0u) return;
  const auto st = G((const CarveStatus*)p.status);
  const uint32_t n = st->n_eligible;
  if (n == 0u || n > PM_CARVE_BIG_SLOTS || s >= n) return;
  const uint32_t SB = n > PM_CARVE_SLOTS ? PM_CARVE_SLOT_BITS_BIG : PM_CARVE_SLOT_BITS;
  const double TIE_BAND = n > PM_CARVE_SLOTS ? PM_TIE_BAND_BIG : PM_TIE_BAND;
  const uint64_t WINDOW_ULPS = n > PM_CARVE_SLOTS ? (1ull << 25) : (1ull << 20);
  uint32_t* wl = reinterpret_cast<uint32_t*>(s_raw);
  BulkCtx bulk = {0u, lane_net(lane, reinterpret_cast<uint64_t*>(s_raw + size_t(CARVE_WAVES) * STREAM_WL_WORDS * 4u))};
  const uint64_t* cfg64 = p.cfgbits + (size_t)ci * p.bits_stride;
  unsigned long long t_all = 0, t_geo = 0, t_sweep = 0, t_fin = 0, check = 0;
  uint32_t swept = 0;
  for (uint32_t rep = 0; rep < reps; ++rep) {
    const uint64_t t0 = __builtin_amdgcn_s_memtime();
    const uint32_t ssite = G(p.cc_site)[s];
    const SeedGeo sg = {G(p.cc_lat)[s], G(p.cc_lon)[s], G(p.cc_cos)[s], G(p.cc_ux)[s], G(p.cc_uy)[s], G(p.cc_uz)[s]};
    const bool shared = (ssite & 0x80000000u) != 0u;
    NearRow q = {~0ull, ~0ull, ~0ull, ~0ull, ~0ull, 0xFFFFFFFFu};
    uint32_t n_mine = 0;
    bulk.seen = 0u;
    asm volatile("s_waitcnt vmcnt(0)" ::: "memory");
    const uint64_t t1 = __builtin_amdgcn_s_memtime();
    (void)stream_bitmap_sweep(p, cfg64, n, wl, lane, s, shared, ssite, sg, SB, WINDOW_ULPS, q, n_mine, bulk, ci, 0x01FFFFF0u);
    const uint64_t t2 = __builtin_amdgcn_s_memtime();
    uint64_t mine = q.m1;
    const uint32_t meta = (g_rowb_mode & 1u) ? 0u : near_row_finish(p, q, true, PM_PROP_KMAX, SB, TIE_BAND, lane, &mine);
    const uint64_t t3 = __builtin_amdgcn_s_memtime() + (meta & 0u);
    t_all += t3 - t0;
    t_geo += t1 - t0;
    t_sweep += t2 - t1;
    t_fin += t3 - t2;
    swept = wave_sum(n_mine);
    check = mine * (lane + 1u) + meta;
  }
  unsigned long long cs = check;
  for (uint32_t o = 32u; o; o >>= 1) cs += __shfl_xor(cs, o, 64);
  if (lane == 0u) {
    out[0] = t_all;
    out[1] = reps;
    out[2] = swept;
    out[3] = cs;
    out[4] = t_geo;
    out[5] = t_sweep;
    out[6] = t_fin;
  }
}
#endif

__global__ __launch_bounds__(CARVE_THREADS) void carve_stream_kernel(const CarveArgs* __restrict__ pa, uint32_t start_ci) {
  const CarveArgs& p = *pa;
  extern __shared__ __attribute__((aligned(16))) unsigned char s_raw[];
  if (blockIdx.x != 0u) {
    stream_proposer(p, s_raw);
    return;
  }
  uint64_t* part = reinterpret_cast<uint64_t*>(s_raw);
  uint64_t* lds_alive = part + CARVE_WAVES * PM_CARVE_PART;
  uint64_t* lds_loc = lds_alive + PM_CARVE_SLOTS / 64;
  uint32_t* lds_wid = reinterpret_cast<uint32_t*>(lds_loc + PM_CARVE_SLOTS / 64);
  uint32_t* lds_site = lds_wid + PM_CARVE_SLOTS;
  uint64_t* lds_key = reinterpret_cast<uint64_t*>(lds_site + PM_CARVE_SLOTS);
  uint32_t* sel_out = reinterpret_cast<uint32_t*>(lds_key + PM_CARVE_SLOTS);
  BlockRed& red = *reinterpret_cast<BlockRed*>(sel_out + PM_CARVE_SEL_CAP);
  uint32_t* sl_words = reinterpret_cast<uint32_t*>(s_raw + PM_CARVE_LDS_BYTES);

  const uint32_t tid = threadIdx.x, lane = tid & 63u, wave = tid >> 6;
  const auto st = G(p.status);
  const auto ctl = G(p.stream_ctl);
  if (st->state != CARVE_STATE_RUNNING) {
    if (tid == 0) st_ag32(&ctl[SC_QUIT], 1u);
    return;
  }
  const uint32_t n = st->n_eligible;
  const uint32_t lw = (n + 63u) >> 6;
  uint32_t exit_state = CARVE_STATE_DONE, stop_ci = p.n_avail;
  StepCtx c;
  c.mode = p.mode;
  c.proximity = p.proximity;
  c.use_props = true;
  c.steps = 0;
  c.fast_steps = 0;
  c.cand_sum = 0;
  c.total_available = st->total_available;
  c.n_groups = st->n_groups;
  c.mem_off = st->n_members;
  c.n_list = n;
  c.n_cand = 0;
  c.min_s = c.max_s = 1;
  c.cfg = 0;
  ctx_set_geometry(c);
  const uint32_t groups_at_entry = c.n_groups;
  const uint32_t steps_before = st->steps_total;
  const bool big = c.big;
  uint64_t* r_alive = big ? reinterpret_cast<uint64_t*>(lds_wid) : lds_alive;
  uint64_t* r_loc = big ? reinterpret_cast<uint64_t*>(lds_site) : lds_loc;
  uint32_t ci = start_ci;
  if (n > PM_CARVE_BIG_SLOTS) {
    exit_state = CARVE_STATE_ABORTED;
    stop_ci = ci;
  } else if (n > 0u) {
    for (uint32_t j = tid; j < lw; j += CARVE_THREADS) r_loc[j] = G(p.loc_g)[j];
    if (!big)
      for (uint32_t sl = tid; sl < n; sl += CARVE_THREADS) lds_site[sl] = G(p.cc_site)[sl];
    for (uint32_t k = tid; k < (uint32_t)SLW_WORDS; k += CARVE_THREADS) sl_words[k] = (k == SLW_P_CI || k == SLW_P_CI1 || k == SLW_TEND) ? PM_NONE : 0u;
    __syncthreads();
    const auto master = G(p.alive_g);
    const auto cfgbits = G((const uint64_t*)p.cfgbits);
    const uint32_t cell_g = st->cell_g, n_indexed = st->n_indexed;
    auto count_candidates = [&](uint32_t cx) -> uint32_t {
      uint32_t cnt = 0;
      for (uint32_t j = tid; j < lw; j += CARVE_THREADS) cnt += (uint32_t)__popcll(master[j] & cfgbits[(size_t)cx * p.bits_stride + j]);
      cnt = wave_sum(cnt);
      __syncthreads();
      if (lane == 0) red.a[wave] = cnt;
      __syncthreads();
      uint32_t tot = 0;
#pragma unroll
      for (uint32_t k = 0; k < CARVE_WAVES; ++k) tot += red.a[k];
      __syncthreads();
      return tot;
    };
    auto row_mode = [&](uint32_t n_cand, uint32_t* switch_at) -> uint32_t {
      *switch_at = 0u;
      if (!cell_g || !p.prune_mode) return SROW_BITMAP;
      if (p.prune_mode >= 2u) return SROW_WALK;
      if ((uint64_t)n_cand * n_cand < (uint64_t)p.prune_factor * n_indexed) return SROW_BITMAP;
      *switch_at = (uint32_t)sqrt((double)p.prune_factor * (double)n_indexed);
      return SROW_WALK;
    };
    auto look_ahead = [&](uint32_t n_cand, uint32_t max_s) -> uint32_t {
      const uint32_t la_max = p.stream_la ? p.stream_la : 896u;
      const uint32_t small = p.stream_la_div ? p.stream_la_div * 256u : 1536u;
      uint32_t la = n_cand <= small ? STREAM_LA_SMALL(n_cand) : n_cand / 4u;
      (void)max_s;
      la = la < 24u ? 24u : la;
      return la > la_max ? la_max : la;
    };
    uint32_t prev_ci = PM_NONE;
    uint32_t acc_pre_used = 0u, acc_pre_lost = 0u, acc_listed = 0u, acc_pruned = 0u, acc_done = 0u;
    for (; ci < p.n_avail; ++ci) {
      c.min_s = p.min_size[ci];
      c.max_s = p.max_size[ci];
      if (tid == 0) STREAM_TRACE(11, ci, c.total_available);
      if (c.total_available < c.min_s) continue;
      uint32_t cnt = 0;
      PROF_DECL;
      for (uint32_t j = tid; j < lw; j += CARVE_THREADS) {
        uint64_t m = master[j];
        if (prev_ci != PM_NONE) m = (m & ~cfgbits[(size_t)prev_ci * p.bits_stride + j]) | r_alive[j];
        const uint64_t nc = m & cfgbits[(size_t)ci * p.bits_stride + j];
        master[j] = m;
        r_alive[j] = nc;
        cnt += (uint32_t)__popcll(nc);
      }
      prev_ci = ci;
      cnt = wave_sum(cnt);
      __syncthreads();
      if (lane == 0) red.a[wave] = cnt;
      __syncthreads();
      uint32_t n_cand = 0;
#pragma unroll
      for (uint32_t k = 0; k < CARVE_WAVES; ++k) n_cand += red.a[k];
      __syncthreads();
      PROF_MARK(32);
      if (n_cand < c.min_s || n_cand == 0u) continue;
      c.cfg = p.avail_cfg[ci];
      c.n_cand = n_cand;
      c.prop_k = (p.proximity && c.max_s - 1u < PM_PROP_KMAX) ? PM_PROP_KMAX : 0u;
      c.prop_limit = n;
      c.rows_pr = 0;
      c.n_seeds = PM_NONE;
      uint32_t switch_at = 0u;
      const uint32_t mode = c.prop_k ? row_mode(n_cand, &switch_at) : SROW_BITMAP;
      c.n_start = switch_at > 256u / PM_THIN_DIV ? switch_at * PM_THIN_DIV : 0u;
      uint32_t seed_cur0 = PM_NONE;
      if (tid == 0) {
        red._spare2 = PM_NONE;
        sl_words[SLW_SCANW] = 0u;
        sl_words[SLW_SCANLO] = sl_words[SLW_SCANHI] = 0xFFFFFFFFu;
        for (uint32_t k = 0; k < 2u; ++k) {
          const uint32_t pc = sl_words[SLW_P_CI + k];
          if (pc == PM_NONE) continue;
          const bool in_reach = sl_words[SLW_TISSUED] - sl_words[SLW_P_T0 + k] + 1280u < PM_STREAM_TP;
          STREAM_TRACE(19, ci | pc << 8 | (in_reach ? 1u : 0u) << 16, sl_words[SLW_P_CNT + k]);
          if (pc == ci && sl_words[SLW_P_CNT + k] > 0u && c.prop_k && c.max_s > 1u && in_reach) {
            red._spare2 = sl_words[SLW_P_T0 + k];
            sl_words[SLW_SCANW] = sl_words[SLW_P_SCANW + k];
            sl_words[SLW_SCANLO] = sl_words[SLW_P_SCANLO + k];
            sl_words[SLW_SCANHI] = sl_words[SLW_P_SCANHI + k];
            acc_pre_used += 1u;
          } else if (pc <= ci) {
            acc_pre_lost += sl_words[SLW_P_CNT + k];
          }
          if (pc <= ci) sl_words[SLW_P_CI + k] = PM_NONE;
        }
        sl_words[SLW_TEND] = PM_NONE;
        sl_words[SLW_NCAND] = n_cand;
        sl_words[SLW_TREQ] = sl_words[SLW_TISSUED];
        sl_words[SLW_LA] = look_ahead(n_cand, c.max_s);
        sl_words[SLW_PAY] = (ci << 18) | (mode << 24);
        if (mode == SROW_BITMAP) acc_listed += 1u;
        else acc_pruned += 1u;
      }
      __syncthreads();
      if (c.prop_k && c.max_s > 1u) {
        uint32_t have = 0u;
        for (uint32_t cx = ci + 1u; cx < p.n_avail && have < 2u; ++cx) {
          if (c.total_available < p.min_size[cx]) continue;
          const bool slotted = sl_words[SLW_P_CI] == cx || sl_words[SLW_P_CI1] == cx;
          uint32_t nx = 0u;
          if (!slotted) {
            nx = count_candidates(cx);
            if (nx < p.min_size[cx] || nx == 0u) continue;
          }
          ++have;
          if (slotted || !(p.max_size[cx] > 1u && p.max_size[cx] - 1u < PM_PROP_KMAX)) continue;
          if (tid == 0) {
            const uint32_t k = sl_words[SLW_P_CI] == PM_NONE ? 0u : sl_words[SLW_P_CI1] == PM_NONE ? 1u : 2u;
            if (k < 2u) {
              uint32_t sw_next = 0u;
              sl_words[SLW_P_CI + k] = cx;
              sl_words[SLW_P_PAY + k] = (cx << 18) | (row_mode(nx, &sw_next) << 24);
              sl_words[SLW_P_MAX + k] = look_ahead(nx, p.max_size[cx]);
              sl_words[SLW_P_CNT + k] = 0u;
              sl_words[SLW_P_T0 + k] = 0u;
              sl_words[SLW_P_SCANW + k] = 0u;
              sl_words[SLW_P_SCANLO + k] = sl_words[SLW_P_SCANHI + k] = 0xFFFFFFFFu;
            }
          }
          __syncthreads();
        }
      }
      __syncthreads();
      seed_cur0 = red._spare2;
      __syncthreads();
      if (tid == 0) STREAM_TRACE(1, ci, n_cand);
      PROF_MARK(33);
      int rc;
      if (!big)
        rc = stream_run_config<false>(p, red, c, lds_site, lds_key, r_alive, r_loc, part, sel_out,
                                      reinterpret_cast<uint32_t*>(lds_key), sl_words, steps_before, seed_cur0);
      else
        rc = stream_run_config<true>(p, red, c, p.cc_site, p.keys, r_alive, r_loc, part, sel_out,
                                     reinterpret_cast<uint32_t*>(lds_key), sl_words, steps_before, seed_cur0);
      __syncthreads();
      if (tid == 0) st_ag32(&ctl[SC_DROP], STREAM_DROP_WORD(ci, sl_words[SLW_TISSUED]));
      PROF_MARK(34);
      if (rc == STEP_UNCERTAIN || rc == STEP_OVERFLOW || rc == STEP_ABORT) {
        exit_state = rc == STEP_UNCERTAIN ? CARVE_STATE_UNCERTAIN : rc == STEP_ABORT ? CARVE_STATE_ABORTED : CARVE_STATE_OVERFLOW;
        stop_ci = ci;
        break;
      }
      if (tid == 0) acc_done += 1u;
    }
    if (tid == 0) {
      st->why[3] += acc_done;
      st->stream_pre_used += acc_pre_used;
      st->stream_pre_lost += acc_pre_lost;
      st->stream_listed += acc_listed;
      st->pruned_batches += acc_pruned;
    }
  }
  if (tid == 0) {
    st_ag32(&ctl[SC_QUIT], 1u);
    ctl[SC_FINISH] = 1u;
  }
  if (n > 0u && n <= PM_CARVE_BIG_SLOTS) {
    const uint32_t q_lo = sl_words[SLW_TISSUED];
    const uint32_t q_hi = ld_ag32(&ctl[SC_CLAIM]) + (gridDim.x - 1u) * PM_STREAM_PROP_WAVES + 64u;
    const auto sq = G(p.stream_sq);
    const uint32_t tag0 = p.stream_tag0;
    for (uint32_t t = q_lo + tid; t < q_hi && t - q_lo < PM_STREAM_SQ; t += CARVE_THREADS)
      st_ag(&sq[t & (PM_STREAM_SQ - 1u)], ((unsigned long long)(tag0 + t) << 32) | 0xFFFFFFFFull);
  }
  __syncthreads();
  if (tid == 0) {
    st->state = exit_state;
    st->n_groups = c.n_groups;
    st->n_members = c.mem_off;
    st->steps_total = steps_before + c.steps;
    st->stop_ci = stop_ci;
    st->cand_sum += c.cand_sum;
    st->cur_ci = exit_state == CARVE_STATE_DONE ? p.n_avail : ci;
    st->n_list = n;
    st->total_available = c.total_available;
    st->need_prep = 0u;
    st->g_lo = groups_at_entry;
    st->g_hi = c.n_groups;
    st->fast_steps += c.fast_steps;
    st->slow_steps += c.steps - c.fast_steps;
    st->n_batches += 1u;
    if (n > 0u && n <= PM_CARVE_BIG_SLOTS) {
      st->stream_timeouts += sl_words[SLW_TIMEOUTS];
      st->stream_tickets += sl_words[SLW_TISSUED];
    }
  }
}

__global__ __launch_bounds__(256) void carve_finish_kernel(const CarveArgs* __restrict__ pa) {
  const CarveArgs& p = *pa;
  const auto st = G(p.status);
  const auto ctl = G(p.stream_ctl);
  __shared__ uint32_t s_last;
  if (ctl[SC_FINISH]) {
    const uint32_t g_lo = st->g_lo, g_hi = st->g_hi;
    const uint32_t total = gridDim.x * 256u;
    const uint32_t id_g0 = p.id_g0, m0 = p.stage_m0, cap_g = p.stage_cap_g, cap_m = p.stage_cap_m;
    const bool stage = p.stage_cfg != nullptr;
    uint32_t solo = 0;
    for (uint32_t g = g_lo + blockIdx.x * 256u + threadIdx.x; g < g_hi; g += total) {
      const uint32_t off = G(p.g_off)[g], gn = G(p.g_n)[g];
      const uint32_t k = g - id_g0;
      for (uint32_t j = 0; j < gn; ++j) {
        const uint32_t w = G(p.order)[G(p.members)[off + j]];
        G(p.members)[off + j] = w;
        if (p.mode == CARVE_MODE_FORM) G(p.group_of)[w] = (int32_t)g;
        if (stage && off + j - m0 < cap_m) p.stage_mem[off + j - m0] = w;
      }
      if (p.g_id_out) {
        unsigned long long z = p.id_state + (unsigned long long)(k + 1u) * 0x9E3779B97F4A7C15ull;
        z = (z ^ (z >> 30)) * 0xBF58476D1CE4E5B9ull;
        z = (z ^ (z >> 27)) * 0x94D049BB133111EBull;
        p.g_id_out[g] = z ^ (z >> 31);
        p.g_task_out[g] = PM_NONE;
      }
      if (stage && k < cap_g) {
        p.stage_cfg[k] = G(p.g_cfg)[g];
        p.stage_n[k] = gn;
        p.stage_off[k] = off;
      }
      solo += gn == 1u ? 1u : 0u;
    }
    solo = wave_sum(solo);
    if ((threadIdx.x & 63u) == 0u && solo) atomicAdd(&p.status->n_solo, solo);
  }
  if (!p.h_status) return;
  __syncthreads();
  if (threadIdx.x == 0) {
    __threadfence();
    s_last = atomicAdd(&p.stream_ctl[SC_FINISH_TICKET], 1u);
  }
  __syncthreads();
  if (s_last != gridDim.x - 1u) return;
  const auto src = G((const uint32_t*)p.status);
  uint32_t* dst = (uint32_t*)p.h_status;
  for (uint32_t k = threadIdx.x; k < (uint32_t)(sizeof(CarveStatus) / 4u); k += 256u) dst[k] = ld_ag32((const stream_gu32*)(src + k));
}

hipError_t launch_carve_stream(const CarveArgs* d_args, uint32_t start_ci, uint32_t n_prop_wgs, hipStream_t s) {
  hipLaunchKernelGGL(carve_stream_kernel, dim3(1u + n_prop_wgs), dim3(CARVE_THREADS), PM_STREAM_LDS_BYTES, s, d_args, start_ci);
  hipLaunchKernelGGL(carve_finish_kernel, dim3(128), dim3(256), 0, s, d_args);
  return hipGetLastError();
}
```

Measured before the change: 1054 billion.

## Sweep task matches per group and fuse carve finish into the sweep kernel

Adds a group-row match path in which the pair sweep runs once per group (selector built from the group's config) instead of once per worker. The carve finish work is folded into extra blocks of that same kernel, so the separate finish launch and the match-prep/selector kernels are skipped. Claim-publish then computes each worker's in-group index and next worker by scanning the group's members directly, replacing the precomputed rank tables. This cuts sweep rows and kernel launches, but adds an O(group size) loop per worker in claim and more coupling between carve and match state.

```diff
diff --git a/protocol_amd/csrc/pm_device.h b/protocol_amd/csrc/pm_device.h
--- a/protocol_amd/csrc/pm_device.h
+++ b/protocol_amd/csrc/pm_device.h
@@ -105,6 +105,8 @@
   const uint64_t* g_id;
   uint32_t* g_task_next;
   const uint32_t* chosen;
+  uint32_t chosen_by_group;
+  const uint32_t *members, *addr_rank;
   const uint32_t* rank_in_group;
   const uint32_t* by_rank;
   const uint64_t* t_live;
@@ -123,6 +125,18 @@
   uint32_t *first, *count;
   uint32_t *rank_in_group, *by_rank;
   uint32_t* g_task_next;
+};
+
+struct CarveArgs;
+struct GroupRowArgs {
+  uint32_t G;
+  const CarveArgs* carve;
+  const uint32_t *g_cfg, *g_task;
+  uint32_t* g_task_next;
+  uint32_t n_split;
+  const uint64_t* planes;
+  uint32_t stride, w_begin, w_end, n_planes, words_per_split, words_per_piece, atomic;
+  uint32_t *first, *count;
 };
 
 struct RowUpdateArgs {
@@ -270,6 +284,8 @@
   unsigned long long* g_id_out;
   uint32_t* g_task_out;
   CarveStatus* h_status;
+  uint32_t *gr_first, *gr_count;
+  uint32_t gr_n, _pad_gr;
   unsigned long long* stream_trace;
   uint32_t n_avail, start_ci;
   uint32_t avail_cfg[PM_MAX_CONFIGS];
@@ -310,6 +326,7 @@
                        hipStream_t s);
 void launch_claim_publish(const ClaimArgs& a, hipStream_t s);
 void launch_match_prep(const MatchPrepArgs& a, hipStream_t s);
+hipError_t launch_group_rows(GroupRowArgs a, uint32_t c_begin, uint32_t c_end, hipStream_t s, bool inited);
 void launch_build_planes(const uint64_t* col_mask, uint32_t n_cols, uint32_t c_begin, uint32_t c_end, uint32_t stride,
                          uint32_t n_planes, uint64_t* planes, hipStream_t s);
 void launch_pair_sweep(int variant, const uint64_t* row_sel, uint32_t R, const uint64_t* col_mask,
@@ -342,7 +359,7 @@
                            bool fresh, uint32_t n_groups0, uint32_t n_members0, hipStream_t s);
 void launch_carve_apply(const CarveArgs* d_args, uint32_t W, hipStream_t s);
 void launch_carve_propose(const CarveArgs* d_args, uint32_t W, hipStream_t s);
-hipError_t launch_carve_stream(const CarveArgs* d_args, uint32_t start_ci, uint32_t n_prop_wgs, hipStream_t s);
+hipError_t launch_carve_stream(const CarveArgs* d_args, uint32_t start_ci, uint32_t n_prop_wgs, hipStream_t s, bool finish = true);
 void launch_scatter_const(uint32_t* dst, const uint32_t* idx, uint32_t n, uint32_t v, hipStream_t s);
 void launch_scatter_pairs(uint32_t* dst, const uint32_t* pairs, uint32_t n, hipStream_t s);
 void launch_merge_place(const CarveArgs* d_args, uint32_t n_order, uint32_t n_groups0, uint32_t n_members0, uint32_t steps0,
diff --git a/protocol_amd/csrc/pm_engine_carve.inc b/protocol_amd/csrc/pm_engine_carve.inc
--- a/protocol_amd/csrc/pm_engine_carve.inc
+++ b/protocol_amd/csrc/pm_engine_carve.inc
@@ -349,11 +349,14 @@
   bool rearmed = false;
   uint32_t stage_cap = 0;
   bool args_pending = false;
+  bool defer_finish = false, finish_owed = false;
+  size_t G_ub = 0;
 };
 
 static int32_t launch_propose_timed(pm_engine* e, const CarveArgs* d_args, uint32_t n_bound, hipStream_t s);
 
 static int32_t form_setup_args(pm_engine* e, FormRun* r);
+static int32_t ensure_sweep_outputs(pm_engine* e, uint32_t R);
 
 static int32_t form_queue_init(pm_engine* e, FormRun* r, bool fresh = false) {
   fresh = fresh && r->use_props;
@@ -382,7 +385,9 @@
     r->args_pending = false;
     host_mark("form: eligible list queued");
     if (r->stream) {
-      HIPCHK(launch_carve_stream(e->d_carve_args.p, r->start_ci, r->stream_wgs, e->stream));
+      r->finish_owed = r->defer_finish;
+      r->defer_finish = false;
+      HIPCHK(launch_carve_stream(e->d_carve_args.p, r->start_ci, r->stream_wgs, e->stream, !r->finish_owed));
       e->tick_carve_launches += 2;
       return PM_OK;
     }
@@ -481,6 +486,14 @@
     a.stage_mem = e->h_gstage + size_t(3) * r->stage_cap;
     a.h_status = e->h_status;
     e->h_status->state = 0xFFFFFFFFu;
+    if (r->defer_finish) {
+      r->G_ub = std::min<size_t>(size_t(r->g0) + r->stage_cap, std::min(e->d_g_task.cap, e->d_g_task_next.cap));
+      int32_t rcs = ensure_sweep_outputs(e, uint32_t(std::max<size_t>(e->W, r->G_ub)));
+      if (rcs) return rcs;
+      a.gr_first = e->d_first.p;
+      a.gr_count = e->d_count.p;
+      a.gr_n = uint32_t(r->G_ub);
+    }
   }
   if (r->local_carve) {
     a.dist_rank = 0;
diff --git a/protocol_amd/csrc/pm_engine_match.inc b/protocol_amd/csrc/pm_engine_match.inc
--- a/protocol_amd/csrc/pm_engine_match.inc
+++ b/protocol_amd/csrc/pm_engine_match.inc
@@ -72,7 +72,12 @@
   return PM_OK;
 }
 
-static int32_t run_match(pm_engine* e, bool want_count, std::vector<uint32_t>* count_out, bool dist = false, size_t G_ub = 0) {
+static bool match_by_group_rows(const pm_engine* e, bool want_count, bool dist) {
+  return !dist && !want_count && e->cfg.chooser == PM_CHOOSE_FIRST && e->cfg.sweep_variant != 1;
+}
+
+static int32_t run_match(pm_engine* e, bool want_count, std::vector<uint32_t>* count_out, bool dist = false, size_t G_ub = 0,
+                         bool behind_carve = false, hipEvent_t after_rows = nullptr) {
   pm_assignment* const claim_h_table = dist ? nullptr : e->claim_h_table;
   uint32_t* const claim_h_gtask = dist ? nullptr : e->claim_h_gtask;
   e->claim_h_table = nullptr;
@@ -88,7 +93,10 @@
   host_mark("match: task planes");
   const uint32_t R = dist ? uint32_t(e->h_own_rows.size()) : e->W;
   const uint32_t* rows = dist ? e->d_own_rows.p : nullptr;
-  rc = ensure_sweep_outputs(e, R);
+  const size_t G = G_ub ? G_ub : e->d_n_groups;
+  const bool by_group = match_by_group_rows(e, want_count, dist);
+  if (behind_carve && !by_group) return set_error(PM_ESTATE, "match: a carve without its finish needs the group-row match");
+  rc = ensure_sweep_outputs(e, by_group ? uint32_t(std::max<size_t>(R, G)) : R);
   if (rc) return rc;
   HIPCHK(e->d_sel.ensure(std::max<uint32_t>(e->W, 1)));
   HIPCHK(e->d_table.ensure(std::max<uint32_t>(e->W, 1)));
@@ -97,8 +105,26 @@
   const uint32_t n_planes = uint32_t(e->cfgs.size());
 
   host_mark("match: selector launch");
-  const size_t G = G_ub ? G_ub : e->d_n_groups;
-  if (!dist) {
+  const uint32_t t_stride = e->t_cap / 64u;
+  if (by_group) {
+    GroupRowArgs m{};
+    m.G = uint32_t(G);
+    m.carve = behind_carve ? e->d_carve_args.p : nullptr;
+    m.g_cfg = e->d_g_cfg.p;
+    m.g_task = e->d_g_task.p;
+    m.g_task_next = e->d_g_task_next.p;
+    m.planes = e->d_tplanes.p;
+    m.stride = t_stride;
+    m.n_planes = n_planes;
+    m.first = e->d_first.p;
+    m.count = e->d_count.p;
+    const bool time_sweep = e->cfg.time_proposer != 0;
+    if (time_sweep) HIPCHK(hipEventRecord(e->kev[4], e->stream));
+    HIPCHK(launch_group_rows(m, e->t_lo, e->t_cap, e->stream, behind_carve));
+    if (time_sweep) HIPCHK(hipEventRecord(e->kev[5], e->stream));
+    e->k_sweep_recorded = time_sweep;
+    if (after_rows) HIPCHK(hipEventRecord(after_rows, e->stream));
+  } else if (!dist) {
     MatchPrepArgs m{};
     m.W = e->W;
     m.G = uint32_t(G);
@@ -119,13 +145,12 @@
   } else {
     launch_worker_selector(e->d_group_of.p, e->d_g_cfg.p, R, rows, e->d_sel.p, e->stream);
   }
-  const bool time_sweep = e->cfg.time_proposer != 0;
+  const bool time_sweep = e->cfg.time_proposer != 0 && !by_group;
   if (time_sweep) HIPCHK(hipEventRecord(e->kev[4], e->stream));
-  const uint32_t t_stride = e->t_cap / 64u;
-  launch_pair_sweep(variant, e->d_sel.p, R, e->d_tmask.p, e->d_tplanes.p, e->t_lo, e->t_cap, t_stride, n_planes,
+  if (!by_group) launch_pair_sweep(variant, e->d_sel.p, R, e->d_tmask.p, e->d_tplanes.p, e->t_lo, e->t_cap, t_stride, n_planes,
                     e->d_first.p, e->d_count.p, e->stream, !dist);
   if (time_sweep) HIPCHK(hipEventRecord(e->kev[5], e->stream));
-  e->k_sweep_recorded = time_sweep;
+  if (!by_group) e->k_sweep_recorded = time_sweep;
   const uint32_t* chosen = e->d_first.p;
   if (e->cfg.chooser == PM_CHOOSE_SEEDED) {
     launch_chooser_rank(e->d_group_of.p, e->d_g_id.p, e->d_count.p, R, rows, e->cfg.chooser_seed, e->d_rank.p,
@@ -149,6 +174,9 @@
   c.g_id = e->d_g_id.p;
   c.g_task_next = e->d_g_task_next.p;
   c.chosen = chosen;
+  c.chosen_by_group = by_group ? 1u : 0u;
+  c.members = e->d_members.p;
+  c.addr_rank = e->d_addr_rank.p;
   c.rank_in_group = e->d_rank_in_group.p;
   c.by_rank = e->d_by_rank.p;
   c.t_live = e->d_tlive.p;
diff --git a/protocol_amd/csrc/pm_engine_tick.inc b/protocol_amd/csrc/pm_engine_tick.inc
--- a/protocol_amd/csrc/pm_engine_tick.inc
+++ b/protocol_amd/csrc/pm_engine_tick.inc
@@ -78,18 +78,20 @@
   if (!e->k_compat_recorded) HIPCHK(hipEventRecord(e->ev[1], e->stream));
   host_mark("tick: compat queued");
   FormRun r;
+  r.defer_finish = !e->tick_needs_merge && match_by_group_rows(e, false, false);
   rc = form_begin(e, &r, true, false, e->ev[1]);
   if (rc) return rc;
+  if (r.finish_owed && !(r.stream && !r.nothing && !e->tick_needs_merge)) return set_error(PM_ESTATE, "tick: a carve was queued without its finish");
   bool done = false;
   if (r.stream && !r.nothing && !e->tick_needs_merge) {
     PubRun pr;
-    HIPCHK(hipEventRecord(e->ev[2], e->stream));
-    const size_t G_ub = std::min<size_t>(size_t(r.g0) + r.stage_cap, std::min(e->d_g_task.cap, e->d_g_task_next.cap));
+    if (!r.finish_owed) HIPCHK(hipEventRecord(e->ev[2], e->stream));
+    const size_t G_ub = r.finish_owed ? r.G_ub : std::min<size_t>(size_t(r.g0) + r.stage_cap, std::min(e->d_g_task.cap, e->d_g_task_next.cap));
     host_mark("tick: carve queued");
     rc = publish_open(e, &pr, G_ub);
     if (rc) return rc;
     host_mark("tick: snapshot buffer open");
-    rc = run_match(e, false, nullptr, false, G_ub);
+    rc = run_match(e, false, nullptr, false, G_ub, r.finish_owed, r.finish_owed ? e->ev[2] : nullptr);
     if (rc) {
       publish_abandon(e, pr);
       return rc;
diff --git a/protocol_amd/csrc/pm_kernels.hip b/protocol_amd/csrc/pm_kernels.hip
--- a/protocol_amd/csrc/pm_kernels.hip
+++ b/protocol_amd/csrc/pm_kernels.hip
@@ -254,13 +254,12 @@
 }
 
 template <uint32_t RPT>
-__global__ __launch_bounds__(256) void pair_sweep_planes_kernel(const uint64_t* __restrict__ row_sel, uint32_t R,
-                                                                const uint64_t* __restrict__ planes,
-                                                                uint32_t stride, uint32_t w_begin, uint32_t w_end,
-                                                                uint32_t n_planes, uint32_t words_per_split,
-                                                                uint32_t words_per_piece,
-                                                                uint32_t* __restrict__ first_out,
-                                                                uint32_t* __restrict__ count_out, uint32_t atomic) {
+__device__ __forceinline__ void pair_sweep_planes_rows(const uint64_t (&sel_in)[RPT], uint32_t R,
+                                                       const uint64_t* __restrict__ planes, uint32_t stride,
+                                                       uint32_t w_begin, uint32_t w_end, uint32_t n_planes,
+                                                       uint32_t words_per_split, uint32_t words_per_piece,
+                                                       uint32_t* __restrict__ first_out,
+                                                       uint32_t* __restrict__ count_out, uint32_t atomic) {
   extern __shared__ uint64_t s_pl[];
   const uint32_t lds_stride = words_per_piece | 1u;
   const uint32_t r0 = blockIdx.x * (256u * RPT) + threadIdx.x;
@@ -273,7 +272,7 @@
 #pragma unroll
   for (uint32_t k = 0; k < RPT; ++k) {
     const uint32_t r = r0 + k * 256u;
-    sel[k] = r < R ? (row_sel[r] & valid) : 0ull;
+    sel[k] = r < R ? (sel_in[k] & valid) : 0ull;
     if (sel[k] == valid && n_planes > 1u && n_planes < 64u) sel[k] = 1ull << n_planes;
     first[k] = PM_NONE;
     cnt[k] = 0;
@@ -332,6 +331,23 @@
     if (r < R) pair_fold(first_out, count_out, r, first[k], cnt[k], atomic != 0u);
   }
 }
+template <uint32_t RPT>
+__global__ __launch_bounds__(256) void pair_sweep_planes_kernel(const uint64_t* __restrict__ row_sel, uint32_t R,
+                                                                const uint64_t* __restrict__ planes,
+                                                                uint32_t stride, uint32_t w_begin, uint32_t w_end,
+                                                                uint32_t n_planes, uint32_t words_per_split,
+                                                                uint32_t words_per_piece,
+                                                                uint32_t* __restrict__ first_out,
+                                                                uint32_t* __restrict__ count_out, uint32_t atomic) {
+  uint64_t sel[RPT];
+#pragma unroll
+  for (uint32_t k = 0; k < RPT; ++k) {
+    const uint32_t r = blockIdx.x * (256u * RPT) + threadIdx.x + k * 256u;
+    sel[k] = r < R ? row_sel[r] : 0ull;
+  }
+  pair_sweep_planes_rows<RPT>(sel, R, planes, stride, w_begin, w_end, n_planes, words_per_split, words_per_piece, first_out,
+                              count_out, atomic);
+}
 
 __global__ __launch_bounds__(256) void pair_select_planes_kernel(const uint64_t* __restrict__ row_sel, uint32_t R,
                                                                  const uint64_t* __restrict__ planes,
@@ -570,16 +586,31 @@
   if (g >= 0) {
     t = p.g_task[g];
     if (t == PM_NONE) {
-      t = p.chosen[r];
+      t = p.chosen[p.chosen_by_group ? (uint32_t)g : r];
       if (t != PM_NONE) p.g_task_next[g] = t;
     }
     const uint32_t n = p.g_n[g], off = p.g_off[g];
-    const uint32_t idx = p.rank_in_group[w];
+    uint32_t idx, next;
+    if (p.chosen_by_group) {
+      const uint32_t my = p.addr_rank[w];
+      uint32_t lo_r = 0xFFFFFFFFu, lo_w = w, up_r = 0xFFFFFFFFu, up_w = PM_NONE;
+      idx = 0;
+      for (uint32_t k = 0; k < n; ++k) {
+        const uint32_t m = p.members[off + k], r = p.addr_rank[m];
+        idx += r < my;
+        if (r < lo_r) lo_r = r, lo_w = m;
+        if (r > my && r < up_r) up_r = r, up_w = m;
+      }
+      next = up_w != PM_NONE ? up_w : lo_w;
+    } else {
+      idx = p.rank_in_group[w];
+      next = p.by_rank[off + ((idx + 1u == n) ? 0u : idx + 1u)];
+    }
     a.task = (t == PM_NONE || p.rows) ? t : task_position(p.t_live, p.t_prefix, t);
     a.group_slot = (uint32_t)g;
     a.group_index = idx;
     a.group_size = n;
-    a.next_worker = p.by_rank[off + ((idx + 1u == n) ? 0u : idx + 1u)];
+    a.next_worker = next;
     a.group_id = p.g_id[g];
   }
   if (p.rows) {
diff --git a/protocol_amd/csrc/pm_launch.inc b/protocol_amd/csrc/pm_launch.inc
--- a/protocol_amd/csrc/pm_launch.inc
+++ b/protocol_amd/csrc/pm_launch.inc
@@ -75,6 +75,19 @@
   if (w1 <= w0) return;
   hipLaunchKernelGGL(build_planes_kernel, dim3(((w1 - w0) * 64u + 255u) / 256u), dim3(256), 0, s, col_mask, n_cols, w0,
                      w1, stride, n_planes, planes);
+}
+
+static size_t plane_sweep_geometry(uint32_t want_split, uint32_t n_words, uint32_t n_planes, uint32_t* n_split_out, uint32_t* wps_out,
+                                   uint32_t* wpp_out) {
+  uint32_t n_split = want_split < n_words ? want_split : n_words;
+  const uint32_t wps = (n_words + n_split - 1u) / n_split;
+  n_split = (n_words + wps - 1u) / wps;
+  const uint32_t lds_cap_words = ((48u * 1024u / 8u) / (n_planes + 1u)) - 1u;
+  const uint32_t wpp = wps < lds_cap_words ? wps : lds_cap_words;
+  *n_split_out = n_split;
+  *wps_out = wps;
+  *wpp_out = wpp;
+  return (size_t)(n_planes + 1u) * (wpp | 1u) * sizeof(uint64_t);
 }
 
 void launch_pair_sweep(int variant, const uint64_t* row_sel, uint32_t R, const uint64_t* col_mask,
@@ -105,13 +118,9 @@
                        c_end, chunk, first, count, n_split > 1u ? 1u : 0u);
     return;
   }
-  const uint32_t w0 = c_begin / 64u, w1 = (c_end + 63u) / 64u, n_words = w1 - w0;
-  uint32_t n_split = want_split < n_words ? want_split : n_words;
-  const uint32_t wps = (n_words + n_split - 1u) / n_split;
-  n_split = (n_words + wps - 1u) / wps;
-  const uint32_t lds_cap_words = ((48u * 1024u / 8u) / (n_planes + 1u)) - 1u;
-  const uint32_t wpp = wps < lds_cap_words ? wps : lds_cap_words;
-  const size_t lds = (size_t)(n_planes + 1u) * (wpp | 1u) * sizeof(uint64_t);
+  const uint32_t w0 = c_begin / 64u, w1 = (c_end + 63u) / 64u;
+  uint32_t n_split, wps, wpp;
+  const size_t lds = plane_sweep_geometry(want_split, w1 - w0, n_planes, &n_split, &wps, &wpp);
   if (n_split > 1u && !inited) hipLaunchKernelGGL(pair_init_kernel, dim3(rb), dim3(256), 0, s, first, count, R);
   if (rpt4)
     hipLaunchKernelGGL(pair_sweep_planes_kernel<PM_SWEEP_RPT_N>, dim3((rb + PM_SWEEP_RPT_N - 1u) / PM_SWEEP_RPT_N, n_split), dim3(256), lds, s,
@@ -119,6 +128,23 @@
   else
     hipLaunchKernelGGL(pair_sweep_planes_kernel<1u>, dim3(rb, n_split), dim3(256), lds, s, row_sel, R, planes, stride, w0,
                        w1, n_planes, wps, wpp, first, count, n_split > 1u ? 1u : 0u);
+}
+
+hipError_t launch_group_rows(GroupRowArgs a, uint32_t c_begin, uint32_t c_end, hipStream_t s, bool inited) {
+  if (a.G == 0 && !a.carve) return hipSuccess;
+  const uint32_t rb = a.G ? (a.G + 255u) / 256u : 1u;
+  const uint32_t want_split = ((a.G <= 16384u ? 512u : 2048u) + rb - 1u) / rb;
+  a.w_begin = c_begin / 64u;
+  a.w_end = c_end > c_begin ? (c_end + 63u) / 64u : a.w_begin;
+  uint32_t n_split = 1u;
+  size_t lds = 0;
+  a.words_per_split = a.words_per_piece = 1u;
+  if (a.w_end > a.w_begin) lds = plane_sweep_geometry(want_split, a.w_end - a.w_begin, a.n_planes, &n_split, &a.words_per_split, &a.words_per_piece);
+  a.n_split = n_split;
+  a.atomic = n_split > 1u ? 1u : 0u;
+  if (a.atomic && !inited) hipLaunchKernelGGL(pair_init_kernel, dim3(rb), dim3(256), 0, s, a.first, a.count, a.G);
+  hipLaunchKernelGGL(group_rows_kernel, dim3(rb, n_split + (a.carve ? 1u : 0u)), dim3(256), lds, s, a);
+  return hipGetLastError();
 }
 
 void launch_pair_select(int variant, const uint64_t* row_sel, uint32_t R, const uint64_t* col_mask,
diff --git a/protocol_amd/csrc/pm_prep.inc b/protocol_amd/csrc/pm_prep.inc
--- a/protocol_amd/csrc/pm_prep.inc
+++ b/protocol_amd/csrc/pm_prep.inc
@@ -242,6 +242,11 @@
       p.status->n_members = n_members0;
     }
   }
+  if (p.gr_first)
+    for (uint32_t k = blockIdx.x * 256u + tid; k < p.gr_n; k += gridDim.x * 256u) {
+      p.gr_first[k] = PM_NONE;
+      p.gr_count[k] = 0u;
+    }
   if (!fresh && G(p.status)->state != CARVE_STATE_RUNNING) return;
   __shared__ uint32_t s_c[PREP_WAVES];
   const uint32_t j = blockIdx.x * PREP_WAVES + wave;
diff --git a/protocol_amd/csrc/pm_stream.inc b/protocol_amd/csrc/pm_stream.inc
--- a/protocol_amd/csrc/pm_stream.inc
+++ b/protocol_amd/csrc/pm_stream.inc
@@ -2496,58 +2496,96 @@
   }
 }
 
+__device__ __forceinline__ uint32_t carve_finish_group(const CarveArgs& p, uint32_t g) {
+  const uint32_t id_g0 = p.id_g0, m0 = p.stage_m0, cap_g = p.stage_cap_g, cap_m = p.stage_cap_m;
+  const bool stage = p.stage_cfg != nullptr;
+  const uint32_t off = G(p.g_off)[g], gn = G(p.g_n)[g];
+  const uint32_t k = g - id_g0;
+  for (uint32_t j = 0; j < gn; ++j) {
+    const uint32_t w = G(p.order)[G(p.members)[off + j]];
+    G(p.members)[off + j] = w;
+    if (p.mode == CARVE_MODE_FORM) G(p.group_of)[w] = (int32_t)g;
+    if (stage && off + j - m0 < cap_m) p.stage_mem[off + j - m0] = w;
+  }
+  if (p.g_id_out) {
+    unsigned long long z = p.id_state + (unsigned long long)(k + 1u) * 0x9E3779B97F4A7C15ull;
+    z = (z ^ (z >> 30)) * 0xBF58476D1CE4E5B9ull;
+    z = (z ^ (z >> 27)) * 0x94D049BB133111EBull;
+    p.g_id_out[g] = z ^ (z >> 31);
+    p.g_task_out[g] = PM_NONE;
+  }
+  if (stage && k < cap_g) {
+    p.stage_cfg[k] = G(p.g_cfg)[g];
+    p.stage_n[k] = gn;
+    p.stage_off[k] = off;
+  }
+  return gn == 1u ? 1u : 0u;
+}
+__device__ __forceinline__ void carve_finish_mirror(const CarveArgs& p, uint32_t solo, uint32_t n_blocks, uint32_t* s_last) {
+  solo = wave_sum(solo);
+  if ((threadIdx.x & 63u) == 0u && solo) atomicAdd(&p.status->n_solo, solo);
+  if (!p.h_status) return;
+  __syncthreads();
+  if (threadIdx.x == 0) {
+    __threadfence();
+    *s_last = atomicAdd(&p.stream_ctl[SC_FINISH_TICKET], 1u);
+  }
+  __syncthreads();
+  if (*s_last != n_blocks - 1u) return;
+  const auto src = G((const uint32_t*)p.status);
+  uint32_t* dst = (uint32_t*)p.h_status;
+  for (uint32_t k = threadIdx.x; k < (uint32_t)(sizeof(CarveStatus) / 4u); k += 256u) dst[k] = ld_ag32((const stream_gu32*)(src + k));
+}
 __global__ __launch_bounds__(256) void carve_finish_kernel(const CarveArgs* __restrict__ pa) {
   const CarveArgs& p = *pa;
   const auto st = G(p.status);
   const auto ctl = G(p.stream_ctl);
   __shared__ uint32_t s_last;
+  uint32_t solo = 0;
   if (ctl[SC_FINISH]) {
     const uint32_t g_lo = st->g_lo, g_hi = st->g_hi;
     const uint32_t total = gridDim.x * 256u;
-    const uint32_t id_g0 = p.id_g0, m0 = p.stage_m0, cap_g = p.stage_cap_g, cap_m = p.stage_cap_m;
-    const bool stage = p.stage_cfg != nullptr;
-    uint32_t solo = 0;
-    for (uint32_t g = g_lo + blockIdx.x * 256u + threadIdx.x; g < g_hi; g += total) {
-      const uint32_t off = G(p.g_off)[g], gn = G(p.g_n)[g];
-      const uint32_t k = g - id_g0;
-      for (uint32_t j = 0; j < gn; ++j) {
-        const uint32_t w = G(p.order)[G(p.members)[off + j]];
-        G(p.members)[off + j] = w;
-        if (p.mode == CARVE_MODE_FORM) G(p.group_of)[w] = (int32_t)g;
-        if (stage && off + j - m0 < cap_m) p.stage_mem[off + j - m0] = w;
-      }
-      if (p.g_id_out) {
-        unsigned long long z = p.id_state + (unsigned long long)(k + 1u) * 0x9E3779B97F4A7C15ull;
-        z = (z ^ (z >> 30)) * 0xBF58476D1CE4E5B9ull;
-        z = (z ^ (z >> 27)) * 0x94D049BB133111EBull;
-        p.g_id_out[g] = z ^ (z >> 31);
-        p.g_task_out[g] = PM_NONE;
-      }
-      if (stage && k < cap_g) {
-        p.stage_cfg[k] = G(p.g_cfg)[g];
-        p.stage_n[k] = gn;
-        p.stage_off[k] = off;
-      }
-      solo += gn == 1u ? 1u : 0u;
-    }
-    solo = wave_sum(solo);
-    if ((threadIdx.x & 63u) == 0u && solo) atomicAdd(&p.status->n_solo, solo);
-  }
-  if (!p.h_status) return;
-  __syncthreads();
-  if (threadIdx.x == 0) {
-    __threadfence();
-    s_last = atomicAdd(&p.stream_ctl[SC_FINISH_TICKET], 1u);
-  }
-  __syncthreads();
-  if (s_last != gridDim.x - 1u) return;
-  const auto src = G((const uint32_t*)p.status);
-  uint32_t* dst = (uint32_t*)p.h_status;
-  for (uint32_t k = threadIdx.x; k < (uint32_t)(sizeof(CarveStatus) / 4u); k += 256u) dst[k] = ld_ag32((const stream_gu32*)(src + k));
+    for (uint32_t g = g_lo + blockIdx.x * 256u + threadIdx.x; g < g_hi; g += total) solo += carve_finish_group(p, g);
+  }
+  carve_finish_mirror(p, solo, gridDim.x, &s_last);
 }
 
-hipError_t launch_carve_stream(const CarveArgs* d_args, uint32_t start_ci, uint32_t n_prop_wgs, hipStream_t s) {
+__global__ __launch_bounds__(256) void group_rows_kernel(GroupRowArgs a) {
+  __shared__ uint32_t s_last;
+  uint32_t n_groups = a.G, g_lo = 0u, g_hi = 0u;
+  if (a.carve) {
+    const CarveArgs& p = *a.carve;
+    const auto st = G(p.status);
+    n_groups = st->n_groups;
+    if (G(p.stream_ctl)[SC_FINISH]) {
+      g_lo = st->g_lo;
+      g_hi = st->g_hi;
+    }
+  }
+  if (blockIdx.y == a.n_split) {
+    uint32_t solo = 0;
+    for (uint32_t g = g_lo + blockIdx.x * 256u + threadIdx.x; g < g_hi; g += gridDim.x * 256u) solo += carve_finish_group(*a.carve, g);
+    carve_finish_mirror(*a.carve, solo, gridDim.x, &s_last);
+    return;
+  }
+  if (blockIdx.y == 0u)
+    for (uint32_t g = blockIdx.x * 256u + threadIdx.x; g < n_groups; g += gridDim.x * 256u)
+      a.g_task_next[g] = (g >= g_lo && g < g_hi) ? PM_NONE : a.g_task[g];
+  const uint32_t R = n_groups < a.G ? n_groups : a.G;
+  if (blockIdx.x * 256u >= R) return;
+  const uint32_t g = blockIdx.x * 256u + threadIdx.x;
+  uint64_t sel[1] = {0ull};
+  if (g < R) {
+    const bool fresh = g >= g_lo && g < g_hi;
+    if (fresh || a.g_task[g] == PM_NONE) sel[0] = 1ull << a.g_cfg[g];
+  }
+  if (a.atomic && !__syncthreads_or(sel[0] != 0ull)) return;
+  pair_sweep_planes_rows<1u>(sel, R, a.planes, a.stride, a.w_begin, a.w_end, a.n_planes, a.words_per_split, a.words_per_piece,
+                             a.first, a.count, a.atomic);
+}
+
+hipError_t launch_carve_stream(const CarveArgs* d_args, uint32_t start_ci, uint32_t n_prop_wgs, hipStream_t s, bool finish) {
   hipLaunchKernelGGL(carve_stream_kernel, dim3(1u + n_prop_wgs), dim3(CARVE_THREADS), PM_STREAM_LDS_BYTES, s, d_args, start_ci);
-  hipLaunchKernelGGL(carve_finish_kernel, dim3(128), dim3(256), 0, s, d_args);
+  if (finish) hipLaunchKernelGGL(carve_finish_kernel, dim3(128), dim3(256), 0, s, d_args);
   return hipGetLastError();
 }
```

Result: slower. 1035 billion (-1.7%).
